# nathanweeks/exonerate

Measured on AMD Instinct MI355X. Metric: DP cells/s (first-pass lattice cells / end-to-end time), est2genome 1kb x 100kb batch, bit-exact vulgar vs reference, higher is better.
Workload: dtype int32 (packed int16 where proven exact)

## Files before the change

exonerate_amd/csrc/c4_ckpt16_kernel.h:

```cpp
#pragma once
#include "c4_viterbi16_kernel.h"

namespace c4k {

__device__ __forceinline__ int bfi32(int mask, int a, int b) {
    return __builtin_amdgcn_bitop3_b32(mask, a, b, 0xCA);
}

template <int R>
struct Prof16 {
    static constexpr int NCODE = 8;
    static constexpr int NP = (R + 1) / 2, EB = NP == 3 ? 12 : 8;
    static constexpr int CODE = 64 * EB;
    static constexpr int INTS = NCODE * CODE / 4;
};

template <int BND>
struct Stage16 {
    static constexpr int COLS = 128, CARRY0 = 6, PLANES = 6 + BND, INTS = COLS * PLANES;
};

template <class M, int R, int ROOT = -1>
struct WaveCK16 {
    using F = Facts<M>;
    static_assert(M::MAXAQ == 1, "the packed forms exchange exactly one query row per step");
    using RT = Roots<M>;
    using W32 = WaveDP<M, R, MODE_CKPT, true, true>;
    static constexpr int NS = M::NS, NCOL = M::MAXAT + 1, W = 64 * R, MAXAT = M::MAXAT;
    static constexpr int CS = W32::CS;
    static constexpr bool live(int s) { return M::NDES > 0 && W32::slot_live(s, 0); }
    static constexpr bool inner(int s) { return RT::member(ROOT, s); }
    static constexpr bool exported(int s) { return inner(s) && F::exported(s); }
    static constexpr int n_live() { int n = 0; for (int s = 0; s < NS; s++) n += (inner(s) && live(s)); return n; }
    static constexpr int n_inner() { int n = 0; for (int s = 0; s < NS; s++) n += inner(s); return n; }
    static constexpr int word_of(int s) { int n = 0; for (int x = 0; x < s; x++) n += inner(x); return n; }
    static constexpr int live_index(int s) { int n = 0; for (int x = 0; x < s; x++) n += (inner(x) && live(x)); return n; }
    static constexpr int CKW = n_inner() + (n_live() + 1) / 2;
    static constexpr int n_exp() { int n = 0; for (int s = 0; s < NS; s++) n += exported(s); return n; }
    static constexpr int n_exp_live() { int n = 0; for (int s = 0; s < NS; s++) n += (exported(s) && live(s)); return n; }
    static constexpr int BND = n_exp() * 2 + n_exp_live();
    static_assert(!F::has_phase(), "split-codon calcs are not packed");
    static_assert(M::NDES <= 1, "one shadow designation");
    static_assert(M::START == 0 && M::END == 1, "state numbering of the closed model");
    static_assert(!F::exported(M::START), "START advances nothing");
    struct C16 { int sc[NS]; int il[NS]; int srp[NS]; };
    typedef __attribute__((address_space(3))) int lds_int;
    __device__ __forceinline__ static lds_int *lds_at(int a) { return (lds_int *)(size_t)(unsigned)a; }
    __device__ __forceinline__ static int lds_addr(const lds_int *p) { return (int)(unsigned)(size_t)p; }
    using P16 = Prof16<R>;
    using ST = Stage16<BND>;

    const KParams *kp;
    int lane;
    const uint8_t *qc[2], *tc[2];
    const uint2 *ss16[2];
    int Q[2], T[2], q0[2], t0[2], tlast[2], cp_count[2], section[2];
    int *ckp[2];
    int cp_next_j[2], cp_next_i[2];
    int cp_phase[2];
    int Qm, Tm, Tmin;
    int open_il_pk, lim_pk, fifteen, at_pk[4], cv_pk[16];
    C16 col[NCOL][R], nbr[NCOL], expo, nx_carry;
    int prof_a[2];
    const uint8_t *tdense;
    int nx_sp4[4], nx_off[2], nx_prof[2 * P16::NP];
    int stage_a, stage_base;
    int carry_a, carry_base;
    bool carry_cols;
    int corner_sc[2], corner_srp[2];
    bool corner_set[2];

    template <class Fn>
    __device__ __forceinline__ static void for_exported(Fn &&fn) {
        int slot = 0;
        static_for<NS>([&](auto S_) __attribute__((always_inline)) { constexpr int S = S_;
            if constexpr (exported(S)) { fn(S_, slot); slot += 2 + (live(S) ? 1 : 0); }
        });
    }
    __device__ __forceinline__ static void write_empty_column(int *colp) {
        for_exported([&](auto S_, int slot) __attribute__((always_inline)) { constexpr int S = S_;
            colp[slot] = NEG16; colp[slot + 1] = 0;
            if constexpr (live(S)) colp[slot + 2] = 0;
        });
    }
    __device__ __forceinline__ void prefetch_carry() {
        const lds_int *p = lds_at(carry_a);
        for_exported([&](auto S_, int slot) __attribute__((always_inline)) { constexpr int S = S_;
            nx_carry.sc[S] = p[slot * ST::COLS];
            nx_carry.srp[S] = p[(slot + 1) * ST::COLS];
            if constexpr (live(S)) nx_carry.il[S] = p[(slot + 2) * ST::COLS];
        });
        carry_a = ((carry_a + 4) & (ST::COLS * 4 - 1)) | carry_base;
    }
    __device__ __forceinline__ void fill_carry(lds_int *stage, int c0, const int *bnd_in) {
        const int c = c0 + lane;
        const int jx = c < 0 ? 0 : (c > Tm ? Tm : c);
        const int jc = carry_cols ? jx : 0;
        const int *g = bnd_in + (long long)jc * BND;
        int v[BND];
        static_for<BND>([&](auto K_) __attribute__((always_inline)) { constexpr int K = K_; v[K] = g[K]; });
        lds_int *p = stage + ST::CARRY0 * ST::COLS + (c & (ST::COLS - 1));
        static_for<BND>([&](auto K_) __attribute__((always_inline)) { constexpr int K = K_; p[K * ST::COLS] = v[K]; });
    }
    template <int H>
    __device__ __forceinline__ void build_profile(int i0) {
        using P16 = Prof16<R>;
        typedef __attribute__((address_space(3))) int lds_int;
        int qr[R];
        static_for<R>([&](auto RR_) __attribute__((always_inline)) { constexpr int RR = RR_;
            const int i = i0 + RR;
            qr[RR] = 24 * ((i >= 1 && i <= Q[H]) ? (int)qc[H][q0[H] + i - 1] : 0);
        });
        for (int d = 0; d < P16::NCODE; d++) {
            const int code = tdense[24 + d];
            int v[R];
            static_for<R>([&](auto RR_) __attribute__((always_inline)) { constexpr int RR = RR_; v[RR] = kp->submat[qr[RR] + code]; });
            lds_int *p = (lds_int *)(size_t)(unsigned)(prof_a[H] + d * P16::CODE);
            static_for<P16::NP>([&](auto K_) __attribute__((always_inline)) { constexpr int K = K_;
                p[K] = pk_pack(v[2 * K], v[2 * K + 1 < R ? 2 * K + 1 : 2 * K]);
            });
        }
    }
    __device__ __forceinline__ void prefetch_column() {
        const lds_int *p = lds_at(stage_a);
        static_for<4>([&](auto K_) __attribute__((always_inline)) { constexpr int K = K_; nx_sp4[K] = p[K * ST::COLS]; });
        nx_off[0] = p[4 * ST::COLS]; nx_off[1] = p[5 * ST::COLS];
        stage_a = ((stage_a + 4) & (ST::COLS * 4 - 1)) | stage_base;
    }
    __device__ __forceinline__ void prefetch_profile() {
        const lds_int *pa = lds_at(prof_a[0] + nx_off[0]), *pb = lds_at(prof_a[1] + nx_off[1]);
        static_for<P16::NP>([&](auto K_) __attribute__((always_inline)) { constexpr int K = K_; nx_prof[K] = pa[K]; nx_prof[P16::NP + K] = pb[K]; });
    }
    __device__ __forceinline__ void fill_stage(lds_int *stage, int c0) {
        constexpr int mat = F::match_at();
        const int c = c0 + lane;
        uint2 sv[2]; int off[2];
        static_for<2>([&](auto H_) __attribute__((always_inline)) { constexpr int H = H_;
            int ti = t0[H] + c - mat;
            ti = ti < 0 ? 0 : (ti > tlast[H] ? tlast[H] : ti);
            off[H] = (int)tc[H][(unsigned)ti] * P16::CODE;
            sv[H] = uint2{0u, 0u};
            if constexpr (F::has_splice()) {
                int tp = t0[H] + c - 2;
                tp = tp < 0 ? 0 : (tp > tlast[H] ? tlast[H] : tp);
                sv[H] = ss16[H][(unsigned)tp];
            }
        });
        lds_int *p = stage + (c & (ST::COLS - 1));
        p[0 * ST::COLS] = (int)__builtin_amdgcn_perm(sv[1].x, sv[0].x, 0x05040100u);
        p[1 * ST::COLS] = (int)__builtin_amdgcn_perm(sv[1].x, sv[0].x, 0x07060302u);
        p[2 * ST::COLS] = (int)__builtin_amdgcn_perm(sv[1].y, sv[0].y, 0x05040100u);
        p[3 * ST::COLS] = (int)__builtin_amdgcn_perm(sv[1].y, sv[0].y, 0x07060302u);
        p[4 * ST::COLS] = off[0]; p[5 * ST::COLS] = off[1];
    }

    template <int RR, int PH, bool JINT>
    __device__ __forceinline__ void eval_cell(int j, bool origin, int ms, const int (&sp)[4]) {
        C16 &c = col[PH][RR];
        static_for<M::NT>([&](auto K_) __attribute__((always_inline)) { constexpr int K = K_;
            constexpr TrDesc t = M::tr[K];
            if constexpr (!inner(t.out)) return;
            if constexpr (t.in == M::START && (RR > 0 || JINT)) return;
            static_assert(!(t.in == M::START && F::code(K) == 1), "a state's first transition is never the one out of START");
            constexpr int PD = (PH - t.at + NCOL) % NCOL;
            const C16 &src = (t.aq == 0) ? col[PD][RR] : (RR > 0 ? col[PD][RR > 0 ? RR - 1 : 0] : nbr[PD]);
            int cand, srpc = 0, ilc = 0;
            if constexpr (t.in == M::START) {
                static_assert(t.in != M::START || (t.aq == 0 && t.at == 0 && t.calc < 0), "START leaves silently");
                cand = origin ? 0 : NEG16;
            } else {
                cand = src.sc[t.in];
                srpc = src.srp[t.in];
                if constexpr (t.calc >= 0) {
                    constexpr CalcDesc cd = M::calc[t.calc];
                    if constexpr (cd.kind == CALC_CONST) cand = pk_add<1>(cand, cv_pk[t.calc]);
                    else if constexpr (cd.kind >= CALC_MATCH_DNA && cd.kind <= CALC_MATCH_P2D) cand = pk_add<1>(cand, ms);
                    else if constexpr (cd.kind == CALC_SPLICE_PRE) cand = pk_add<1>(cand, sp[cd.param]);
                    else if constexpr (cd.kind == CALC_SPLICE_POST) {
                        static_assert(live(t.in), "post-splice calc without a length");
                        const int bad = pk_neg_mask(src.il[t.in], fifteen);
                        const int sv = bfi32(bad, NEG16, sp[cd.param]);
                        cand = pk_add<1>(cand, sv);
                    }
                }
                if constexpr (!JINT && t.at > 0) cand = (j >= t.at) ? cand : NEG16;
                if constexpr (live(t.out)) {
                    if constexpr (F::owns_shadow(t.in, 0)) ilc = open_il_pk;
                    else if constexpr (live(t.in)) ilc = pk_add<1>(src.il[t.in], at_pk[t.at]);
                }
            }
            if constexpr (F::code(K) == 1) {
                c.sc[t.out] = cand;
                c.srp[t.out] = srpc;
                if constexpr (live(t.out)) c.il[t.out] = ilc;
            } else {
                const int win = pk_lt_mask<1>(c.sc[t.out], cand, 0);
                c.srp[t.out] = bfi32(win, srpc, c.srp[t.out]);
                if constexpr (live(t.out)) c.il[t.out] = bfi32(win, ilc, c.il[t.out]);
                c.sc[t.out] = pk_max<1>(c.sc[t.out], cand);
            }
        });
    }

    template <bool JINT, int PH>
    __device__ __forceinline__ void step(int s, int i0, bool first_strip, bool last_strip, const int *bnd_in, int *bnd_out) {
        const int j = s - lane;
        int ms[R];
        static_for<P16::NP>([&](auto K_) __attribute__((always_inline)) { constexpr int K = K_;
            const int ea = nx_prof[K], eb = nx_prof[P16::NP + K];
            ms[2 * K] = (int)__builtin_amdgcn_perm((unsigned)eb, (unsigned)ea, 0x05040100u);
            if constexpr (2 * K + 1 < R) ms[2 * K + 1] = (int)__builtin_amdgcn_perm((unsigned)eb, (unsigned)ea, 0x07060302u);
        });
        int sp[4];
        static_for<4>([&](auto K_) __attribute__((always_inline)) { constexpr int K = K_; sp[K] = nx_sp4[K]; });
        for_exported([&](auto S_, int) __attribute__((always_inline)) { constexpr int S = S_;
            nbr[PH].sc[S] = dpp_shr1(nx_carry.sc[S], expo.sc[S]);
            nbr[PH].srp[S] = dpp_shr1(nx_carry.srp[S], expo.srp[S]);
            if constexpr (live(S)) nbr[PH].il[S] = dpp_shr1(nx_carry.il[S], expo.il[S]);
        });
        prefetch_carry();
        prefetch_column();
        const bool origin = first_strip & (lane == 0) & (s == 0);
        static_for<R>([&](auto RR_) __attribute__((always_inline)) { constexpr int RR = RR_;
            eval_cell<RR, PH, JINT>(j, origin, ms[RR], sp);
            if constexpr (RR == (R + 1) / 2 - 1) prefetch_profile();
        });
        for_exported([&](auto S_, int) __attribute__((always_inline)) { constexpr int S = S_;
            expo.sc[S] = col[PH][R - 1].sc[S];
            expo.srp[S] = col[PH][R - 1].srp[S];
            if constexpr (live(S)) expo.il[S] = col[PH][R - 1].il[S];
        });
        if (!last_strip && lane == 63 && j >= 0 && j <= Tm) {
            for_exported([&](auto S_, int slot) __attribute__((always_inline)) { constexpr int S = S_;
                int *p = bnd_out + (long long)j * BND + slot;
                p[0] = expo.sc[S];
                p[1] = expo.srp[S];
                if constexpr (live(S)) p[2] = expo.il[S];
            });
        }
        if (s >= Tmin) {
            static_for<2>([&](auto H_) __attribute__((always_inline)) { constexpr int H = H_;
                const bool mine = (j == T[H]) & (Q[H] >= i0) & (Q[H] < i0 + R);
                if (__builtin_amdgcn_ballot_w64(mine)) {
                    static_for<R>([&](auto RR_) __attribute__((always_inline)) { constexpr int RR = RR_;
                        if (mine & (i0 + RR == Q[H])) {
                            bool set = false;
                            int e_sc = 0, e_srp = 0;
                            static_for<M::NT>([&](auto K_) __attribute__((always_inline)) { constexpr int K = K_;
                                constexpr TrDesc t = M::tr[K];
                                if constexpr (t.out == M::END && inner(t.in)) {
                                    static_assert(t.out != M::END || (t.aq == 0 && t.at == 0 && t.calc < 0 && t.in != M::START),
                                                  "END is entered silently from an inner state");
                                    const int v = pk_half(col[PH][RR].sc[t.in], H);
                                    const int p = (int)(((unsigned)col[PH][RR].srp[t.in] >> (16 * H)) & 0xffffu);
                                    const bool win = !set | (e_sc < v);
                                    e_sc = win ? v : e_sc;
                                    e_srp = win ? p : e_srp;
                                    set = true;
                                }
                            });
                            corner_sc[H] = e_sc; corner_srp[H] = e_srp; corner_set[H] = set;
                        }
                    });
                }
            });
        }
        const bool cp_near = (section[0] <= 0) | (cp_phase[0] <= 63 + MAXAT - 1) | (section[1] <= 0) | (cp_phase[1] <= 63 + MAXAT - 1);
        static_for<2>([&](auto H_) __attribute__((always_inline)) { constexpr int H = H_;
            const int nx = cp_phase[H] + 1;
            cp_phase[H] = nx >= section[H] ? nx - section[H] : nx;
        });
        if (cp_near) {
            unsigned stamp = 0;
            static_for<2>([&](auto H_) __attribute__((always_inline)) { constexpr int H = H_;
                const bool cp_live = (j >= 0) & (j <= T[H]) & (cp_next_i[H] < cp_count[H]);
                const unsigned ahead = (unsigned)(cp_next_j[H] - j);
                if (__builtin_amdgcn_ballot_w64(cp_live & (ahead < (unsigned)MAXAT))) {
                    if (cp_live & (ahead < (unsigned)MAXAT)) {
                        static_for<R>([&](auto RR_) __attribute__((always_inline)) { constexpr int RR = RR_;
                            const int i = i0 + RR;
                            if (i <= Q[H]) {
                                int *p = ckp[H] + ((((long long)cp_next_i[H] * MAXAT + ahead) * (Q[H] + 1) + i)) * CKW;
                                constexpr unsigned sel = H ? 0x07060302u : 0x05040100u;
                                int lw[(n_live() + 1) / 2 > 0 ? (n_live() + 1) / 2 : 1] = {0};
                                static_for<NS>([&](auto S_) __attribute__((always_inline)) { constexpr int S = S_;
                                    if constexpr (inner(S)) {
                                        p[word_of(S)] = (int)__builtin_amdgcn_perm((unsigned)col[PH][RR].srp[S], (unsigned)col[PH][RR].sc[S], sel);
                                        if constexpr (live(S)) {
                                            constexpr int li = live_index(S);
                                            const unsigned h = ((unsigned)pk_add<1>(col[PH][RR].il[S], lim_pk) >> (16 * H)) & 0xffffu;
                                            lw[li / 2] |= (int)(h << (16 * (li & 1)));
                                        }
                                    }
                                });
                                static_for<(n_live() + 1) / 2>([&](auto L_) __attribute__((always_inline)) { constexpr int L = L_; p[n_inner() + L] = lw[L]; });
                            }
                        });
                    }
                    stamp |= (cp_live & (ahead == 0u)) ? (H ? 0xffff0000u : 0x0000ffffu) : 0u;
                }
            });
            if (__builtin_amdgcn_ballot_w64(stamp != 0u)) {
                int i0v = i0;
                asm volatile("" : "+v"(i0v));
                static_for<MAXAT>([&](auto ROW_) __attribute__((always_inline)) { constexpr int ROW = ROW_;
                    constexpr int PR = (PH - ROW + NCOL) % NCOL;
                    static_for<R>([&](auto RR_) __attribute__((always_inline)) { constexpr int RR = RR_;
                        const int rowid = (i0v + RR) * (NS * MAXAT);
                        static_for<NS>([&](auto S_) __attribute__((always_inline)) { constexpr int S = S_;
                            if constexpr (inner(S)) {
                                const int id = (rowid + S * MAXAT + ROW) & 0xffff;
                                col[PR][RR].srp[S] = bfi32((int)stamp, id | (id << 16), col[PR][RR].srp[S]);
                            }
                        });
                    });
                    const int rowid = (i0v - 1) * (NS * MAXAT);
                    static_for<NS>([&](auto S_) __attribute__((always_inline)) { constexpr int S = S_;
                        if constexpr (exported(S)) {
                            const int id = (rowid + S * MAXAT + ROW) & 0xffff;
                            nbr[PR].srp[S] = bfi32((int)stamp, id | (id << 16), nbr[PR].srp[S]);
                        }
                    });
                });
                static_for<2>([&](auto H_) __attribute__((always_inline)) { constexpr int H = H_;
                    const bool mine = (stamp & (H ? 0xffff0000u : 0x0000ffffu)) != 0u;
                    cp_next_i[H] += mine ? 1 : 0;
                    cp_next_j[H] += mine ? section[H] : 0;
                });
            }
        }
    }

    template <int NW>
    __device__ __forceinline__ void run(const DevJob &ja, const DevJob &jb, const DevSeqs &seqs, int *bnd, int *ckpt_a, int *ckpt_b,
                                        int wid, int *prog, lds_int *stage) {
        const DevJob *jp[2] = {&ja, &jb};
        ckp[0] = ckpt_a; ckp[1] = ckpt_b;
        static_for<2>([&](auto H_) __attribute__((always_inline)) { constexpr int H = H_;
            const DevJob &jx = *jp[H];
            Q[H] = jx.Q; T[H] = jx.T; q0[H] = jx.q0; t0[H] = jx.t0;
            tlast[H] = seqs.tlen[jx.pair] > 0 ? seqs.tlen[jx.pair] - 1 : 0;
            qc[H] = seqs.qcode + seqs.qoff[jx.pair];
            tc[H] = reinterpret_cast<const uint8_t *>(seqs.sub_rows) + seqs.toff[jx.pair];
            ss16[H] = F::has_splice() ? seqs.ss16 + seqs.toff[jx.pair] : nullptr;
            cp_count[H] = jx.cp_count;
            section[H] = jx.T / (jx.cp_count + 1);
            corner_sc[H] = LOW; corner_srp[H] = 0; corner_set[H] = false;
        });
        Qm = Q[0] > Q[1] ? Q[0] : Q[1]; Tm = T[0] > T[1] ? T[0] : T[1]; Tmin = T[0] < T[1] ? T[0] : T[1];
        static_for<M::NC>([&](auto CI_) __attribute__((always_inline)) { constexpr int CI = CI_;
            const int v = clamp16(kp->calc_value[CI]);
            cv_pk[CI] = pk_pack(v, v);
        });
        static_for<4>([&](auto A_) __attribute__((always_inline)) { constexpr int A = A_; at_pk[A] = pk_pack(A, A); });
        {
            const int lim = clamp16(kp->min_intron - 4);
            lim_pk = pk_pack(lim, lim);
            open_il_pk = pk_pack(-lim, -lim);
            fifteen = 0x000f000f;
        }
        const int nstrips = (Qm + 1 + W - 1) / W;
        const int nsteps = Tm + 64;
        const int main_lo = 63 + MAXAT, main_hi = Tm;
        const int nsteps_r = (nsteps + NCOL - 1) / NCOL * NCOL;
        const int main_lo_r = (main_lo + NCOL - 1) / NCOL * NCOL;
        constexpr int CHK = (63 / NCOL) * NCOL;
        const int PS = nsteps_r + 1;
        stage_base = lds_addr(stage);
        carry_base = stage_base + ST::CARRY0 * ST::COLS * 4;
        for (int b = wid; b < nstrips; b += NW) {
            const int i0 = b * W + lane * R;
            stage_a = stage_base + ((0 - lane) & (ST::COLS - 1)) * 4;
            carry_a = carry_base;
            static_for<2>([&](auto H_) __attribute__((always_inline)) { constexpr int H = H_;
                build_profile<H>(i0);
                cp_next_j[H] = section[H] > 0 ? section[H] : 0x7fffffff; cp_next_i[H] = 0;
                cp_phase[H] = section[H] > 0 ? (MAXAT - 1) % section[H] : 0;
            });
            static_for<NS>([&](auto S_) __attribute__((always_inline)) { constexpr int S = S_;
                expo.sc[S] = NEG16; expo.il[S] = 0; expo.srp[S] = 0;
                static_for<NCOL>([&](auto D_) __attribute__((always_inline)) { constexpr int D = D_;
                    nbr[D].sc[S] = NEG16; nbr[D].il[S] = 0; nbr[D].srp[S] = 0;
                    static_for<R>([&](auto RR_) __attribute__((always_inline)) { constexpr int RR = RR_;
                        col[D][RR].sc[S] = NEG16; col[D][RR].il[S] = 0; col[D][RR].srp[S] = 0;
                    });
                });
            });
            __builtin_amdgcn_fence(__ATOMIC_ACQUIRE, "workgroup");
            const bool first = (b == 0), last = (b == nstrips - 1);
            carry_cols = !first;
            const int *bnd_in = first ? bnd : bnd + BND + (long long)((b + 1) & 1) * (Tm + 1) * BND;
            int *bnd_out = bnd + BND + (long long)(b & 1) * (Tm + 1) * BND;
            auto group = [&](auto JI_, int s0) __attribute__((always_inline)) {
                constexpr bool JI = decltype(JI_)::value != 0;
                static_for<NCOL>([&](auto P_) __attribute__((always_inline)) { constexpr int P = P_;
                    step<JI, P>(s0 + P, i0, first, last, bnd_in, bnd_out);
                });
            };
            {
                const int above = (wid + NW - 1) % NW, above_base = ((b - 1) / NW) * PS, my_base = (b / NW) * PS;
                auto wait_above = [&](int c1) __attribute__((always_inline)) {
                    if constexpr (NW == 1) return;
                    if (first) return;
                    const int need = above_base + (c1 + 64 < nsteps_r ? c1 + 64 : nsteps_r);
                    while (__hip_atomic_load(prog + above, __ATOMIC_RELAXED, __HIP_MEMORY_SCOPE_WORKGROUP) < need) __builtin_amdgcn_s_sleep(1);
                    __builtin_amdgcn_fence(__ATOMIC_ACQUIRE, "workgroup");
                };
                fill_stage(stage, -63);
                wait_above(CHK < nsteps_r ? CHK : nsteps_r);
                fill_carry(stage, -63, bnd_in);
                prefetch_column();
                prefetch_profile();
                prefetch_carry();
                for (int c0 = 0; c0 < nsteps_r; c0 += CHK) {
                    const int c1 = c0 + CHK < nsteps_r ? c0 + CHK : nsteps_r;
                    fill_stage(stage, c0 + 1);
                    if (c0) wait_above(c1);
                    fill_carry(stage, c0 + 1, bnd_in);
                    int s = c0;
                    for (; s < main_lo_r && s < c1; s += NCOL) group(IC<0>{}, s);
                    for (; s + NCOL - 1 <= main_hi && s < c1; s += NCOL) group(IC<1>{}, s);
                    for (; s < c1; s += NCOL) group(IC<0>{}, s);
                    if constexpr (NW > 1) {
                        if (!last) {
                            __builtin_amdgcn_fence(__ATOMIC_RELEASE, "workgroup");
                            if (lane == 0) __hip_atomic_store(prog + wid, my_base + c1, __ATOMIC_RELAXED, __HIP_MEMORY_SCOPE_WORKGROUP);
                        }
                    }
                }
            }
            __builtin_amdgcn_fence(__ATOMIC_RELEASE, "workgroup");
        }
    }

    struct Cell3 { int sc, shadow, srp; };
    __device__ static Cell3 cell_at(const int *ck, const DevJob &job, int section_length, int cp, int row, int qpos, int state) {
        const int *p = ck + (((long long)cp * MAXAT + row) * (job.Q + 1) + qpos) * CKW;
        Cell3 c; c.sc = 0; c.shadow = 0; c.srp = 0;
        static_for<NS>([&](auto S_) __attribute__((always_inline)) { constexpr int S = S_;
            if constexpr (inner(S)) {
                if (state == S) {
                    const unsigned w = (unsigned)p[word_of(S)];
                    c.sc = (int)(short)(w & 0xffffu);
                    c.srp = (int)(w >> 16);
                    if constexpr (live(S)) {
                        constexpr int li = live_index(S);
                        const int il = (int)(((unsigned)p[n_inner() + li / 2] >> (16 * (li & 1))) & 0xffffu);
                        c.shadow = job.t0 + (section_length * (cp + 1) - row) - il - 2;
                    }
                }
            }
        });
        return c;
    }
    __device__ __noinline__ static void checkpoint_traceback(const int *ck, const DevJob &job, DevVsa *vsa, DevResult &res) {
        const int q0 = job.q0, t0 = job.t0;
        const int cpn = job.cp_count, section_length = job.T / (cpn + 1);
        auto decode = [&](int srp, int &state, int &row, int &pos) {
            row = srp % MAXAT;
            const int rem = srp / MAXAT;
            state = rem % NS;
            pos = rem / NS;
        };
        int state, row, pos, n = 0;
        decode(res.last_srp, state, row, pos);
        int query_start = q0 + pos, target_start = t0 + section_length * cpn - row;
        DevVsa v;
        v.qs = query_start; v.ts = target_start;
        v.ql = (q0 + job.Q) - query_start; v.tl = (t0 + job.T) - target_start;
        v.first_state = state;
        for (int l = 0; l < CELL_MAX; l++) v.final_cell[l] = l < CS ? res.final_cell[l] : 0;
        vsa[n++] = v;
        for (int c = cpn - 1; c >= 1; c--) {
            const DevVsa p = v;
            const int prev_row = row;
            const Cell3 cell = cell_at(ck, job, section_length, c, prev_row, p.qs - q0, p.first_state);
            decode(cell.srp, state, row, pos);
            query_start = q0 + pos;
            target_start = p.ts - section_length - row + prev_row;
            v.qs = query_start; v.ts = target_start; v.ql = p.qs - query_start; v.tl = p.ts - target_start;
            v.first_state = state;
            for (int l = 0; l < CELL_MAX; l++) v.final_cell[l] = 0;
            v.final_cell[0] = cell.sc; v.final_cell[1] = cell.shadow; v.final_cell[CS - 1] = cell.srp;
            vsa[n++] = v;
        }
        {
            const DevVsa p = v;
            const Cell3 cell = cell_at(ck, job, section_length, 0, row, p.qs - q0, p.first_state);
            v.qs = q0; v.ts = t0; v.ql = query_start - q0; v.tl = target_start - t0;
            v.first_state = job.first_state;
            for (int l = 0; l < CELL_MAX; l++) v.final_cell[l] = 0;
            v.final_cell[0] = cell.sc; v.final_cell[1] = cell.shadow; v.final_cell[CS - 1] = cell.srp;
            vsa[n++] = v;
        }
        res.n_vsa = n;
    }
};

template <class M, int R, int ROOT, int NW>
__device__ __forceinline__ void ckpt16_pair(const KParams *kp_lds, const DevSeqs &seqs, const DevJob *jobs, int ia, int ib,
                                            DevResult *results, DevVsa *vsas, int *bnd, int *ck_a, int *ck_b, int *prog,
                                            int (*corner_lds)[4], int *prof_mem, const uint8_t *tdense, int *stage_mem) {
    using DP = WaveCK16<M, R, ROOT>;
    if (threadIdx.x == 0) DP::write_empty_column(bnd);
    if constexpr (NW > 1) {
        if (threadIdx.x < NW) prog[threadIdx.x] = 0;
        if (threadIdx.x < 2) corner_lds[threadIdx.x][3] = 0;
    }
    __builtin_amdgcn_fence(__ATOMIC_RELEASE, "workgroup");
    __syncthreads();
    DP dp{};
    dp.kp = kp_lds;
    dp.lane = threadIdx.x & 63;
    dp.tdense = tdense;
    {
        typedef __attribute__((address_space(3))) int lds_int;
        const int w = __builtin_amdgcn_readfirstlane((int)(threadIdx.x >> 6));
        for (int h = 0; h < 2; h++)
            dp.prof_a[h] = (int)(unsigned)(size_t)((lds_int *)prof_mem + (w * 2 + h) * Prof16<R>::INTS) + dp.lane * Prof16<R>::EB;
    }
    {
        const int w = __builtin_amdgcn_readfirstlane((int)(threadIdx.x >> 6));
        dp.template run<NW>(jobs[ia], jobs[ib], seqs, bnd, ck_a, ck_b, w, prog, (typename DP::lds_int *)stage_mem + w * DP::ST::INTS);
    }
    int sc[2], srp[2];
    bool set[2];
    if constexpr (NW == 1) {
        for (int h = 0; h < 2; h++) {
            const unsigned long long owners = __ballot(dp.corner_set[h]);
            const int owner = owners ? __ffsll((long long)owners) - 1 : 0;
            sc[h] = __shfl(dp.corner_sc[h], owner); srp[h] = __shfl(dp.corner_srp[h], owner);
            set[h] = owners != 0;
        }
        __builtin_amdgcn_fence(__ATOMIC_ACQ_REL, "workgroup");
        __syncthreads();
    } else {
        for (int h = 0; h < 2; h++)
            if (dp.corner_set[h]) { corner_lds[h][0] = dp.corner_sc[h]; corner_lds[h][1] = dp.corner_srp[h]; corner_lds[h][3] = 1; }
        __builtin_amdgcn_fence(__ATOMIC_ACQ_REL, "workgroup");
        __syncthreads();
        for (int h = 0; h < 2; h++) { sc[h] = corner_lds[h][0]; srp[h] = corner_lds[h][1]; set[h] = corner_lds[h][3] != 0; }
    }
    if (threadIdx.x < 2 && (threadIdx.x == 0 || ib != ia)) {
        const int h = threadIdx.x;
        const DevJob &job = jobs[h ? ib : ia];
        DevResult res;
        res.flags = set[h] ? 0 : FLAG_NO_END; res.n_ops = 0; res.n_vsa = 0; res.pad = 0; res.qs = res.ts = 0;
        res.cell_size = DP::CS; res.ops_off = 0;
        for (int l = 0; l < CELL_MAX; l++) res.final_cell[l] = 0;
        res.final_cell[0] = sc[h]; res.final_cell[DP::CS - 1] = srp[h];
        res.score = sc[h]; res.end_set = set[h]; res.qe = job.Q; res.te = job.T; res.last_srp = srp[h];
        if (set[h]) DP::checkpoint_traceback(h ? ck_b : ck_a, job, vsas + job.vsa_off, res);
        results[h ? ib : ia] = res;
    }
    __syncthreads();
}

template <class M, int R, int WPE, bool ROOTED, int NW = 1>
__global__ __launch_bounds__(64 * NW) __attribute__((amdgpu_waves_per_eu(WPE, 8)))
void ckpt16_kernel(const KParams *kparams, DevSeqs seqs, const DevJob *jobs, const int *pairs, int n_pairs, DevResult *results,
                   DevVsa *vsas, DevScratch scratch, int *queue) {
    using RT = Roots<M>;
    static_assert(!ROOTED || RT::disjoint(), "a rooted pass needs components to choose from");
    __shared__ __attribute__((aligned(512))) int stage_mem[NW * Stage16<WaveCK16<M, R, ROOTED ? Roots<M>::root(0) : -1>::BND>::INTS];
    static_assert(!ROOTED || WaveCK16<M, R, Roots<M>::root(0)>::BND == WaveCK16<M, R, Roots<M>::root(Roots<M>::count() - 1)>::BND, "one stage layout for every root");
    __shared__ int next_job;
    __shared__ int prog[NW];
    __shared__ int corner_lds[2][4];
    __shared__ __attribute__((aligned(16))) int prof_mem[NW * 2 * Prof16<R>::INTS];
    __shared__ uint8_t tdense_lds[32];
    if (threadIdx.x < 32) tdense_lds[threadIdx.x] = reinterpret_cast<const uint8_t *>(seqs.sub_colptr)[threadIdx.x];
    __syncthreads();
    const KParams *kp_lds = kparams;
    int *bnd = scratch.bnd + (long long)blockIdx.x * scratch.bnd_stride;
    int *ck_a = scratch.ckpt + (long long)blockIdx.x * 2 * scratch.ckpt_stride, *ck_b = ck_a + scratch.ckpt_stride;
    for (;;) {
        if (threadIdx.x == 0) next_job = atomicAdd(queue, 1);
        __syncthreads();
        const int pid = __builtin_amdgcn_readfirstlane(next_job);
        __syncthreads();
        if (pid >= n_pairs) break;
        const int ia = pairs[2 * pid], ib = pairs[2 * pid + 1] >= 0 ? pairs[2 * pid + 1] : ia;
        if constexpr (ROOTED) {
            const int root = jobs[ia].root;
            bool ran = false;
            static_for<RT::count()>([&](auto X_) __attribute__((always_inline)) { constexpr int X = X_;
                constexpr int ROOT = RT::root(X);
                if (!ran && root == ROOT) {
                    ckpt16_pair<M, R, ROOT, NW>(kp_lds, seqs, jobs, ia, ib, results, vsas, bnd, ck_a, ck_b, prog, corner_lds, prof_mem, tdense_lds, stage_mem);
                    ran = true;
                }
            });
            if (!ran && threadIdx.x < 2 && (threadIdx.x == 0 || ib != ia)) {
                DevResult res;
                res.flags = FLAG_NO_END; res.n_ops = 0; res.n_vsa = 0; res.pad = 0; res.qs = res.ts = res.qe = res.te = 0;
                res.cell_size = 0; res.ops_off = 0; res.score = LOW; res.end_set = 0; res.last_srp = 0;
                for (int l = 0; l < CELL_MAX; l++) res.final_cell[l] = 0;
                results[threadIdx.x ? ib : ia] = res;
            }
        } else {
            ckpt16_pair<M, R, -1, NW>(kp_lds, seqs, jobs, ia, ib, results, vsas, bnd, ck_a, ck_b, prog, corner_lds, prof_mem, tdense_lds, stage_mem);
        }
    }
}

}
```

exonerate_amd/csrc/c4_config.h:

```cpp
#pragma once
#include <cstdlib>
#include <mutex>

namespace c4cfg {

#define C4CFG_KEYS(X) \
    X(TRACE) X(PK16) X(WPE) X(WIN16) X(PACK) X(SEED_KSHIFT) X(WIN_NW) X(WINDOW_HOPS) X(WINDOWED) X(STRICT) X(SPLICE_TILE) \
    X(SDP_ARENA_MB) X(REPAIR_REJOIN) X(PK16_R6) X(PK16_NW8) X(PK16_LONG) X(PK16_IO) X(PK16_C8) X(PIN_XFER) X(NESTED_REDO) X(MW) \
    X(LOOP_SHORTCUT) X(LOCAL_EXACT) X(LANES) X(FUSED) X(FREE_NOW) X(FORCE_CORNER_MISMATCH) X(DL_SYNC_FIRST) X(CONT_FREE) \
    X(CK16_TMAX) X(CK16_ROOT) X(CK16) X(CELL_STRICT) X(BYROOT) X(SS16_CHECK) X(SCORE_FIRST) X(HOST_THREADS) X(FORCE_SEQUENTIAL) \
    X(FILL_ALLOC)

enum Key {
#define X(name) name,
    C4CFG_KEYS(X)
#undef X
    N_KEYS
};

struct Entry { bool set; int value; double real; };
struct Table { Entry e[N_KEYS]; };

inline Table &table() { static Table t{}; return t; }
inline std::once_flag &loaded_flag() { static std::once_flag f; return f; }

inline void load_from_environment() {
    static const char *const names[N_KEYS] = {
#define X(name) "C4GPU_" #name,
        C4CFG_KEYS(X)
#undef X
    };
    Table &t = table();
    for (int k = 0; k < N_KEYS; k++) {
        const char *v = getenv(names[k]);
        t.e[k].set = v != nullptr;
        t.e[k].value = v ? atoi(v) : 0;
        t.e[k].real = v ? atof(v) : 0.0;
    }
}
inline const Table &get() {
    std::call_once(loaded_flag(), load_from_environment);
    return table();
}
inline bool has(Key k) { return get().e[k].set; }
inline int num(Key k, int dflt) { const Entry &x = get().e[k]; return x.set ? x.value : dflt; }
inline double real(Key k, double dflt) { const Entry &x = get().e[k]; return x.set ? x.real : dflt; }
inline bool is(Key k, int v) { const Entry &x = get().e[k]; return x.set && x.value == v; }
inline bool nonzero(Key k) { const Entry &x = get().e[k]; return x.set && x.value != 0; }

}
```

exonerate_amd/csrc/c4_engine_find_path.inc:

```
int find_path_batch(Engine &eng, const ResidentSeqs &seqs, int dpmemory_mb, c4gpu_score threshold,
                    c4gpu_alignment *alignments, const std::vector<const c4gpu_subopt *> *subs = nullptr,
                    const uint8_t *active = nullptr, const std::vector<c4gpu_score> *pair_thresholds = nullptr,
                    const c4gpu_region *initial = nullptr, bool own_all = true) {
    const c4gpu_model *m = eng.model;
    const int n = seqs.n_pairs;
    const c4gpu_score base_threshold = threshold;
    auto thr = [&](int pair) {
        return (pair_thresholds && (*pair_thresholds)[pair] > base_threshold) ? (*pair_thresholds)[pair] : base_threshold;
    };
    struct SubScope {
        Engine &e;
        SubScope(Engine &e_, const std::vector<const c4gpu_subopt *> *s) : e(e_) { e.pair_sub = s; }
        ~SubScope() { e.pair_sub = nullptr; }
    } sub_scope(eng, subs);
    const bool trace = c4cfg::has(c4cfg::TRACE);
    const auto t_begin = std::chrono::steady_clock::now();
    auto lap = [&](const char *what) {
        if (trace) fprintf(stderr, "c4gpu trace: find_path_batch: %-28s at %.3f ms\n", what,
                           std::chrono::duration<double, std::milli>(std::chrono::steady_clock::now() - t_begin).count());
    };
    const bool strict_cells = cell_strict();
    std::vector<PairPlan> plan(n);
    std::vector<JobSpec> &specs = eng.fp_specs;
    std::vector<JobOut> &outs = eng.fp_outs;
    specs.clear();
    std::vector<int> owner;
    if (own_all) for (int i = 0; i < n; i++) memset(&alignments[i], 0, sizeof(c4gpu_alignment));
    std::vector<int> region_pairs;
    for (int i = 0; i < n; i++) {
        plan[i].ar = initial ? initial[i] : c4gpu_region{0, 0, seqs.qlen[i], seqs.tlen[i]};
        plan[i].active = !active || active[i];
        if (!plan[i].active) continue;
        if (c4h::use_reduced_space(m, &plan[i].ar, dpmemory_mb)) {
            plan[i].reduced = true;
            if (!model_is_global(m)) region_pairs.push_back(i);
        }
    }
    const size_t step1_total = region_pairs.size();
    double &hit_rate = eng.ctx->hit_rate[subs ? 1 : 0];
    std::vector<std::pair<int, DevResult>> region_done;
    {
        bool pk16_serves = eng.family == FAM_EST2GENOME && eng.pk16_params_ok && region_pairs.size() >= 2 &&
                           !(c4cfg::is(c4cfg::PK16, 0)) && get_kernel_pk16(eng.family, 1) != nullptr;
        for (size_t x = 0; x < region_pairs.size() && pk16_serves; x++)
            pk16_serves = eng.pk16_fits(plan[region_pairs[x]].ar.query_length, plan[region_pairs[x]].ar.target_length);
        int kshift_env = pk16_serves ? 12 : 13;
        for (int i : region_pairs)
            if (plan[i].ar.target_length < (4 << 13) && plan[i].ar.target_length >= (4 << 12)) kshift_env = 12;
        kshift_env = c4cfg::num(c4cfg::SEED_KSHIFT, kshift_env);
        const int kshift = std::max(2, std::min(kshift_env, 20));
        const bool off = c4cfg::is(c4cfg::WINDOWED, 0);
        const KernelInfo *k1 = get_kernel_mw(eng.family, MODE_SCORE, true, false, 4, false, 1);
        const KernelInfo *k2 = get_kernel_mw(eng.family, MODE_REGION, true, true, 4, false, 2);
        const bool pays = eng.ctx->window_rate < 0 || eng.ctx->window_rate >= 0.5 || c4cfg::has(c4cfg::SEED_KSHIFT);
        if (!off && pays && !subs && eng.local && eng.local_exact && k1 && k2 && !(c4cfg::is(c4cfg::PACK, 0))) {
            std::vector<int> win_pairs, rest;
            for (int i : region_pairs) {
                const c4gpu_region &ar = plan[i].ar;
                const bool rows_ok = ar.query_length + 1 > 2 * 64 * k2->R;
                if (rows_ok && ar.target_length >= (4 << kshift) && ar.query_length < (1 << 20)) win_pairs.push_back(i);
                else rest.push_back(i);
            }
            if (!win_pairs.empty()) {
                std::vector<DevResult> wres;
                if (windowed_region_pass(eng, seqs, win_pairs, plan, thr, kshift, wres)) return -1;
                for (size_t x = 0; x < win_pairs.size(); x++) region_done.emplace_back(win_pairs[x], wres[x]);
                region_pairs.swap(rest);
            }
        }
    }
    {
        const bool sf_env = c4cfg::has(c4cfg::SCORE_FIRST);
        const bool can = threshold > C4GPU_IMPOSSIBLY_LOW_SCORE && region_pairs.size() >= 512;
        const size_t total = region_pairs.size();
        auto score_filter = [&](size_t first, size_t count, size_t *kept) -> int {
            specs.clear();
            for (size_t x = first; x < first + count; x++) { JobSpec s; s.pair = region_pairs[x]; s.region = plan[region_pairs[x]].ar; specs.push_back(s); }
            if (eng.run(seqs, MODE_SCORE, false, specs, outs)) return -1;
            *kept = 0;
            for (size_t x = 0; x < count; x++) {
                if (outs[x].res.score < thr(region_pairs[first + x])) plan[region_pairs[first + x]].active = false;
                else (*kept)++;
            }
            return 0;
        };
        bool score_first = false;
        size_t sampled = 0, kept = 0, all_kept = 0;
        if (can && sf_env) score_first = c4cfg::num(c4cfg::SCORE_FIRST, 0) != 0;
        else if (can && hit_rate >= 0) score_first = hit_rate < 0.3;
        else if (can) {
            sampled = std::min<size_t>(8 * (size_t)eng.ctx->prop.multiProcessorCount, total);
            if (score_filter(0, sampled, &kept)) return -1;
            all_kept = kept;
            score_first = (double)kept / (double)sampled < 0.3;
        }
        if (score_first && sampled < total) {
            if (score_filter(sampled, total - sampled, &kept)) return -1;
            all_kept += kept;
        }
        if (score_first || sampled) {
            std::vector<int> survivors;
            for (int i : region_pairs) if (plan[i].active) survivors.push_back(i);
            region_pairs.swap(survivors);
        }
        (void)all_kept;
    }
    specs.clear();
    for (int i : region_pairs) { JobSpec s; s.pair = i; s.region = plan[i].ar; specs.push_back(s); }
    if (eng.run(seqs, MODE_REGION, false, specs, outs)) return -1;
    for (size_t x = 0; x < region_pairs.size(); x++) region_done.emplace_back(region_pairs[x], outs[x].res);
    for (const auto &pr : region_done) {
        PairPlan &p = plan[pr.first];
        const DevResult &r = pr.second;
        if (r.score < thr(pr.first)) { p.active = false; continue; }
        p.region_score = r.score;
        p.end_from = r.last_srp;
        if (m->start_scope != C4GPU_SCOPE_QUERY) p.ar.query_start += r.qs;
        if (m->start_scope != C4GPU_SCOPE_TARGET) p.ar.target_start += r.ts;
        p.ar.query_length = r.qe - (m->start_scope != C4GPU_SCOPE_QUERY ? r.qs : 0);
        p.ar.target_length = r.te - (m->start_scope != C4GPU_SCOPE_TARGET ? r.ts : 0);
    }
    if (step1_total >= 64 && threshold > C4GPU_IMPOSSIBLY_LOW_SCORE) {
        size_t hits = 0;
        for (const auto &pr : region_done) hits += plan[pr.first].active ? 1 : 0;
        const double rate = (double)hits / (double)step1_total;
        hit_rate = hit_rate < 0 ? rate : 0.5 * hit_rate + 0.5 * rate;
    }
    lap("region pass done");
    specs.clear(); owner.clear();
    for (int i = 0; i < n; i++) {
        PairPlan &p = plan[i];
        if (!p.active) continue;
        if (p.reduced && c4h::use_reduced_space(m, &p.ar, dpmemory_mb)) continue;
        p.reduced = false;
        JobSpec s; s.pair = i; s.region = p.ar;
        specs.push_back(s); owner.push_back(i);
    }
    if (eng.run(seqs, MODE_PATH, false, specs, outs)) return -1;
    for (size_t x = 0; x < owner.size(); x++) {
        const int i = owner[x];
        const DevResult &r = outs[x].res;
        c4gpu_alignment &a = alignments[i];
        a.score = r.score;
        a.region.query_start = plan[i].ar.query_start + r.qs;
        a.region.target_start = plan[i].ar.target_start + r.ts;
        a.region.query_length = r.qe - r.qs;
        a.region.target_length = r.te - r.ts;
        int cap = 0;
        for (uint32_t r : outs[x].runs) c4h::alignment_add(&a, &cap, (int)(r >> 24), (int)(r & 0xffffff));
        a.valid = 1;
    }
    lap("quadratic paths done");
    std::vector<int> red;
    for (int i = 0; i < n; i++)
        if (plan[i].active && plan[i].reduced) {
            Segment s;
            memset(&s, 0, sizeof s);
            s.region = plan[i].ar; s.first_state = m->start_state; s.needs_checkpoints = true;
            plan[i].segs.assign(1, s);
            red.push_back(i);
        }
    std::map<int, JobOut> ckpt_done;
    if (!red.empty() && !subs) {
        std::vector<char> done(n, 0);
        if (fused_reduced_paths(eng, seqs, red, plan, dpmemory_mb, alignments, done, ckpt_done)) return -1;
        std::vector<int> rest;
        for (int i : red) if (!done[i]) rest.push_back(i);
        red.swap(rest);
        lap("device route done");
    }
    std::vector<c4gpu_score> red_score(n, 0);
    std::vector<char> redo(n, 0), packed_pair(n, 0);
    for (const auto &kv : ckpt_done) packed_pair[kv.first] = kv.second.packed ? 1 : 0;
    bool first_round = true;
    for (;;) {
        struct Ref { int pair, seg; };
        std::vector<Ref> refs;
        specs.clear();
        for (int i : red) {
            std::vector<Segment> &sg = plan[i].segs;
            for (size_t k = 0; k < sg.size(); k++) {
                if (!sg[k].needs_checkpoints) continue;
                JobSpec s; s.pair = i; s.region = sg[k].region;
                s.first_state = sg[k].first_state;
                if (k > 0) memcpy(s.first_cell, sg[k - 1].final_cell, sizeof s.first_cell);
                s.final_state = (k + 1 < sg.size()) ? sg[k + 1].first_state : m->end_state;
                s.cp_count = c4h::checkpoint_rows(m, &s.region, dpmemory_mb);
                specs.push_back(s);
                refs.push_back(Ref{i, (int)k});
            }
        }
        if (specs.empty()) break;
        lap("checkpoint jobs listed");
        bool have_all = first_round && !ckpt_done.empty();
        for (size_t x = 0; x < refs.size() && have_all; x++) have_all = ckpt_done.count(refs[x].pair) != 0;
        if (have_all) {
            if (outs.size() < refs.size()) outs.resize(refs.size());
            for (size_t x = 0; x < refs.size(); x++) outs[x] = ckpt_done[refs[x].pair];
        } else if (eng.run(seqs, MODE_CKPT, true, specs, outs)) return -1;
        lap("checkpoint pass done");
        std::vector<int> group;
        for (size_t x = 0; x < refs.size(); x++)
            if (!x || refs[x].pair != refs[x - 1].pair) group.push_back((int)x);
        group.push_back((int)refs.size());
        parallel_for((long long)group.size() - 1, 256, [&](long long g0, long long g1) {
          for (long long g = g0; g < g1; g++)
            for (int x = group[g + 1] - 1; x >= group[g]; x--) {
            std::vector<Segment> &sg = plan[refs[x].pair].segs;
            const int k = refs[x].seg;
            if (first_round) red_score[refs[x].pair] = outs[x].res.score;
            std::vector<Segment> children;
            children.reserve(outs[x].vsa.size());
            for (int v = (int)outs[x].vsa.size() - 1; v >= 0; v--) {
                const DevVsa &dv = outs[x].vsa[v];
                Segment c;
                c.region = c4gpu_region{dv.qs, dv.ts, dv.ql, dv.tl};
                c.first_state = dv.first_state;
                memcpy(c.final_cell, dv.final_cell, sizeof c.final_cell);
                c.needs_checkpoints = c4h::use_reduced_space(m, &c.region, dpmemory_mb);
                children.push_back(c);
            }
            if (!first_round && !children.empty() &&
                !final_cell_equiv(children.back().final_cell, sg[k].final_cell, 1 + m->total_shadow_designations,
                                  sg[k].region.target_start + sg[k].region.target_length, packed_pair[refs[x].pair] != 0, strict_cells)) {
                const bool next_in_round = x + 1 < group[g + 1] && refs[x + 1].seg == k + 1;
                if (c4cfg::has(c4cfg::TRACE))
                    fprintf(stderr, "c4gpu trace: pair %d nested segment %d: final cell %d/%d after the nested pass, %d/%d predicted%s\n",
                            refs[x].pair, k, children.back().final_cell[0], children.back().final_cell[1], sg[k].final_cell[0], sg[k].final_cell[1],
                            next_in_round ? ": the next segment's nested pass used the old cell, sequential route" : "");
                if (next_in_round || c4cfg::nonzero(c4cfg::NESTED_REDO)) redo[refs[x].pair] = 1;
            }
            sg.erase(sg.begin() + k);
            sg.insert(sg.begin() + k, children.begin(), children.end());
            }
        });
        first_round = false;
    }
    lap("segments expanded");
    specs.clear();
    struct Ref2 { int pair, seg; };
    std::vector<Ref2> refs2;
    std::vector<size_t> seg_first(red.size() + 1, 0);
    for (size_t r = 0; r < red.size(); r++) seg_first[r + 1] = seg_first[r] + plan[red[r]].segs.size();
    std::vector<JobSpec> &sub_specs = eng.fp_sub_specs;
    if (sub_specs.size() != seg_first[red.size()]) sub_specs.resize(seg_first[red.size()]);
    refs2.resize(seg_first[red.size()]);
    parallel_for((long long)red.size(), 256, [&](long long r0, long long r1) {
        for (long long r = r0; r < r1; r++) {
            const int i = red[r];
            const std::vector<Segment> &sg = plan[i].segs;
            for (size_t k = 0; k < sg.size(); k++) {
                JobSpec s; s.pair = i; s.region = sg[k].region;
                s.first_state = sg[k].first_state;
                if (k > 0) memcpy(s.first_cell, sg[k - 1].final_cell, sizeof s.first_cell);
                s.final_state = (k + 1 < sg.size()) ? sg[k + 1].first_state : m->end_state;
                sub_specs[seg_first[r] + k] = s;
                refs2[seg_first[r] + k] = Ref2{i, (int)k};
            }
        }
    });
    lap("sub-alignment jobs listed");
    if (eng.run(seqs, MODE_PATH, true, sub_specs, outs)) return -1;
    lap("sub-alignment pass done");
    {
        std::vector<int> cap(n, 0);
        const int path_cs = 1 + m->total_shadow_designations;
        const bool force_seq = c4cfg::has(c4cfg::FORCE_SEQUENTIAL);
        if (force_seq) for (int i : red) redo[i] = 1;
        struct Repair { int pair, next_seg; int seed[CELL_MAX]; };
        std::vector<Repair> repairs;
        std::vector<int> repairing(n, -1);
        std::mutex repairs_lock;
        parallel_for((long long)red.size(), 256, [&](long long r0, long long r1) {
          for (long long r = r0; r < r1; r++)
            for (size_t x = seg_first[r]; x < seg_first[r + 1]; x++) {
            const int i = refs2[x].pair, k = refs2[x].seg;
            c4gpu_alignment &a = alignments[i];
            std::vector<Segment> &sg = plan[i].segs;
            if (k == 0) {
                a.score = red_score[i];
                a.region = plan[i].ar;
                a.valid = 1;
            }
            if (redo[i] || repairing[i] >= 0) continue;
            for (uint32_t r : outs[x].runs) c4h::alignment_add(&a, &cap[i], (int)(r >> 24), (int)(r & 0xffffff));
            if (!final_cell_equiv(outs[x].res.final_cell, sg[k].final_cell, path_cs,
                                  sg[k].region.target_start + sg[k].region.target_length, packed_pair[i] != 0, strict_cells)) {
                if (c4cfg::has(c4cfg::TRACE))
                    fprintf(stderr, "c4gpu trace: pair %d sub-alignment %d: final cell %d/%d computed, %d/%d predicted\n", i,
                            k, outs[x].res.final_cell[0], outs[x].res.final_cell[1], sg[k].final_cell[0], sg[k].final_cell[1]);
                if (k + 1 < (int)sg.size()) {
                    Repair rp; rp.pair = i; rp.next_seg = k + 1;
                    memcpy(rp.seed, outs[x].res.final_cell, sizeof rp.seed);
                    std::lock_guard<std::mutex> hold(repairs_lock);
                    repairs.push_back(rp);
                    repairing[i] = k + 1;
                }
            }
            }
        });
        std::sort(repairs.begin(), repairs.end(), [](const Repair &x, const Repair &y) { return x.pair < y.pair; });
        const bool rejoin = !(c4cfg::is(c4cfg::REPAIR_REJOIN, 0));
        std::vector<size_t> first_of(n, 0);
        for (size_t r = 0; r < red.size(); r++) first_of[red[r]] = seg_first[r];
        std::vector<JobOut> routs;
        long long repair_launches = 0, repaired = 0, rejoined = 0;
        while (!repairs.empty()) {
            specs.clear();
            for (const Repair &rp : repairs) {
                const std::vector<Segment> &sg = plan[rp.pair].segs;
                JobSpec s; s.pair = rp.pair; s.region = sg[rp.next_seg].region;
                s.first_state = sg[rp.next_seg].first_state;
                memcpy(s.first_cell, rp.seed, sizeof s.first_cell);
                s.final_state = (rp.next_seg + 1 < (int)sg.size()) ? sg[rp.next_seg + 1].first_state : m->end_state;
                specs.push_back(s);
            }
            if (eng.run(seqs, MODE_PATH, true, specs, routs)) return -1;
            repair_launches++; repaired += (long long)repairs.size();
            std::vector<Repair> next;
            for (size_t x = 0; x < repairs.size(); x++) {
                Repair rp = repairs[x];
                c4gpu_alignment &a = alignments[rp.pair];
                const std::vector<Segment> &sg = plan[rp.pair].segs;
                const int nseg = (int)sg.size();
                for (uint32_t r : routs[x].runs) c4h::alignment_add(&a, &cap[rp.pair], (int)(r >> 24), (int)(r & 0xffffff));
                memcpy(rp.seed, routs[x].res.final_cell, sizeof rp.seed);
                const int j = rp.next_seg;
                if (j + 1 >= nseg) continue;
                const bool joined = rejoin && final_cell_equiv(rp.seed, sg[j].final_cell, path_cs,
                                                               sg[j].region.target_start + sg[j].region.target_length, packed_pair[rp.pair] != 0, strict_cells);
                if (!joined) { rp.next_seg = j + 1; next.push_back(rp); continue; }
                rejoined++;
                for (int k = j + 1; k < nseg; k++) {
                    const JobOut &bo = outs[first_of[rp.pair] + k];
                    for (uint32_t r : bo.runs) c4h::alignment_add(&a, &cap[rp.pair], (int)(r >> 24), (int)(r & 0xffffff));
                    if (k + 1 < nseg && !final_cell_equiv(bo.res.final_cell, sg[k].final_cell, path_cs,
                                                          sg[k].region.target_start + sg[k].region.target_length, packed_pair[rp.pair] != 0, strict_cells)) {
                        rp.next_seg = k + 1;
                        memcpy(rp.seed, bo.res.final_cell, sizeof rp.seed);
                        next.push_back(rp);
                        break;
                    }
                }
            }
            repairs.swap(next);
        }
        if (repair_launches && c4cfg::has(c4cfg::TRACE))
            fprintf(stderr, "c4gpu trace: stale tails: %lld sub-alignments recomputed in %lld launches, %lld re-joined the batch\n",
                    repaired, repair_launches, rejoined);
    }
    lap("alignments assembled");
    for (int i : red)
        if (redo[i] && sequential_reduced_path(eng, seqs, i, dpmemory_mb, plan[i].ar, &alignments[i])) return -1;
    for (int i = 0; i < n; i++) {
        if (active && !active[i]) continue;
        c4gpu_alignment &a = alignments[i];
        if (a.valid && a.score < thr(i)) c4gpu_alignment_clear(&a);
    }
    return 0;
}

struct SideLane {
    c4gpu_ctx ctx;
    Engine eng;
    ~SideLane() {
        if (ctx.stream) (void)hipStreamDestroy(ctx.stream);
        if (ctx.ev0) (void)hipEventDestroy(ctx.ev0);
        if (ctx.ev1) (void)hipEventDestroy(ctx.ev1);
    }
// ... 62 lines not shown
```

exonerate_amd/csrc/c4_engine_launch.inc:

```
struct JobSpec {
    int pair;
    c4gpu_region region;
    int first_state = 0, final_state = 1, cp_count = 0;
    int root = 0;
    int first_cell[CELL_MAX] = {0};
    bool dump_checkpoints = false;
    const c4gpu_subopt *sub = nullptr;
    const int32_t *span_in = nullptr;
    int32_t *span_out = nullptr;
};
typedef std::vector<std::pair<int32_t, int32_t>> RegionPoints;
struct RunList {
    static constexpr int INLINE = 6;
    int n = 0;
    uint32_t small[INLINE];
    std::vector<uint32_t> big;
    const uint32_t *begin() const { return n <= INLINE ? small : big.data(); }
    const uint32_t *end() const { return begin() + n; }
    void assign_reversed(const uint32_t *first, int count) {
        n = count;
        uint32_t *dst = small;
        if (count > INLINE) { big.resize(count); dst = big.data(); }
        for (int k = 0; k < count; k++) dst[k] = first[count - 1 - k];
    }
};
struct JobOut {
    DevResult res;
    RunList runs;
    std::vector<DevVsa> vsa;
    std::vector<int> checkpoints;
    bool packed = false;
};

struct SeedPlan {
    int mode = 0;
    int kshift = 11;
    bool fmt16 = false;
    int seedw = 0, dc = 0;
    std::vector<long long> off;
    std::vector<int> rows;
    std::vector<long long> base;
    std::vector<int> d, t0w, t0_base;
    int hops = 0;
};

int window_waves(int family) {
    int nw = c4cfg::num(c4cfg::WIN_NW, 2);
    if (nw != 2) nw = 4;
    return get_kernel_mw(family, MODE_REGION, true, true, nw, false, 2) ? nw : 4;
}

struct Engine {
    c4gpu_ctx *ctx;
    const c4gpu_model *model;
    int family;
    bool local;
    bool local_exact = true;
    bool pk16_params_ok = false;
    double calc_bound = 0;
    int pk16_match_max = 1, pk16_max_intron = 0;
    int pk16_intron_gain = 0, pk16_intron_cols = 4;
    int loop_tr_host[16] = {-1, -1, -1, -1, -1, -1, -1, -1, -1, -1, -1, -1, -1, -1, -1, -1};
    DevBuf<KParams> kparams;
    DevBuf<DevJob> d_jobs;
    DevBuf<DevResult> d_results;
    DevBuf<DevVsa> d_vsa;
    DevBuf<uint32_t> d_runs, d_runs_out;
    DevBuf<unsigned long long> d_runs_used;
    DevBuf<uint8_t> d_ops;
    DevBuf<int> d_bnd, d_ckpt, d_ckpt_dump, d_queue;
    DevBuf<uint32_t> d_tb;
    DevBuf<int> d_sub_t, d_sub_q, d_sub_colptr, d_span, d_seed, d_pairs;
    DevBuf<DevJob> d_fjobs, d_fsub_jobs;
    DevBuf<DevResult> d_fres, d_fsub_res;
    DevBuf<DevVsa> d_fvsa;
    DevBuf<int> d_ffirst, d_fflags, d_fout;
    DevBuf<unsigned long long> d_fstats;
    DevBuf<FusePair> d_fpairs;
    std::vector<DevJob> hf_jobs;
    std::vector<DevResult> hf_res;
    std::vector<int> hf_first, hf_flags, hf_out;
    std::vector<FusePair> hf_pairs;
    std::vector<int> h_order;
    std::vector<long long> h_key;
    std::vector<DevJob> h_jobs;
    std::vector<DevResult> h_res;
    std::vector<uint32_t> h_runs;
    std::vector<DevVsa> h_vsa;
    std::vector<int> h_dump;
    std::vector<JobSpec> fp_specs;
    std::vector<JobSpec> fp_sub_specs;
    std::vector<JobOut> fp_outs;
    const std::vector<const c4gpu_subopt *> *pair_sub = nullptr;

    bool annotated = false;
    int init(c4gpu_ctx *c, const c4gpu_model *m, const c4gpu_params *params) {
        KParams kp;
        if (init_host(c, m, params, kp)) return -1;
        return kparams.upload(&kp, 1, ctx->stream);
    }
    int init_host(c4gpu_ctx *c, const c4gpu_model *m, const c4gpu_params *params, KParams &kp) {
        ctx = c; model = m;
        family = model_family(*m);
        if (family < 0) {
            c4h::set_error(std::string("model [") + m->name + "] is not one of the device-accelerated families");
            return -1;
        }
        local = m->start_scope == C4GPU_SCOPE_ANYWHERE && m->end_scope == C4GPU_SCOPE_ANYWHERE;
        memset(&kp, 0, sizeof kp);
        for (int i = 0; i < 16; i++) loop_tr_host[i] = -1;
        for (int i = 0; i < m->n_calcs; i++) kp.calc_value[i] = m->calcs[i].value;
        kp.min_intron = params->min_intron; kp.max_intron = params->max_intron;
        if (params->max_intron < params->min_intron) {
            kp.min_intron = kp.max_intron = 0x7fffffff;
        }
        kp.start_scope = m->start_scope; kp.end_scope = m->end_scope;
        bool protein = false;
        for (int i = 0; i < m->n_calcs; i++)
            if (m->calcs[i].kind == C4GPU_CALC_MATCH_PROTEIN || m->calcs[i].kind == C4GPU_CALC_MATCH_P2D ||
                m->calcs[i].kind == C4GPU_CALC_MATCH_CODON) protein = true;
        memcpy(kp.submat, protein ? &params->protein_submat[0][0] : &params->dna_submat[0][0], sizeof(int) * 24 * 24);
        bool dna_match = false;
        for (int i = 0; i < m->n_calcs; i++) dna_match |= m->calcs[i].kind == C4GPU_CALC_MATCH_DNA;
        const bool veto = annotated && dna_match && !protein;
        for (int c = 0; c < 24; c++) kp.submat[24 * 24 + c] = veto ? C4GPU_IMPOSSIBLY_LOW_SCORE : 0;
        {
            double pmax = 0;
            for (int i = 0; i < m->n_calcs; i++) pmax = std::max(pmax, std::fabs((double)m->calcs[i].value));
            for (int i = 0; i < 24 * 24; i++) pmax = std::max(pmax, std::fabs((double)kp.submat[i]));
            double smax = 0;
            if (family_has_splice(family))
                for (int k = 0; k < 4; k++) {
                    const c4gpu_splice_model &sp = params->splice[k];
                    double sum = 0;
                    for (int r = 0; r < sp.model_length && r < C4GPU_SPLICE_MAX_LEN; r++) {
                        double mx = 0;
                        for (int c = 0; c < 5; c++) mx = std::max(mx, std::fabs((double)sp.data[r][c]));
                        sum += mx;
                    }
                    smax = std::max(smax, sum + 1.0);
                }
            local_exact = (pmax + smax) * (m->n_states + 4) < 4.0e8;
            calc_bound = pmax + smax;
            double mmax = 0;
            for (int i = 0; i < 24 * 24; i++) mmax = std::max(mmax, (double)kp.submat[i]);
            pk16_match_max = (int)std::max(1.0, mmax);
            pk16_params_ok = pmax <= 16000.0 && smax <= 16000.0 && params->min_intron >= 0 && params->min_intron <= 30000 &&
                             params->max_intron >= params->min_intron;
            pk16_max_intron = params->max_intron;
            if (veto) {
                local_exact = false;
                pk16_params_ok = false;
                calc_bound = std::max(calc_bound, 987654321.0);
            }
            if (family_has_splice(family)) {
                int best[4] = {0, 0, 0, 0};
                for (int k = 0; k < 4; k++) {
                    const c4gpu_splice_model &sp = params->splice[k];
                    double sum = 0;
                    for (int r = 0; r < sp.model_length && r < C4GPU_SPLICE_MAX_LEN; r++) {
                        double mx = 0;
                        for (int c = 0; c < 5; c++) mx = std::max(mx, (double)sp.data[r][c]);
                        sum += mx;
                    }
                    best[k] = (int)std::floor(sum + 0.5) + 1;
                }
                long long gain = -0x40000000LL;
                for (int st = 0; st < m->n_states; st++) {
                    long long pre = -0x40000000LL, post = -0x40000000LL;
                    for (int k = 0; k < m->n_transitions; k++) {
                        const c4gpu_transition &t = m->transitions[k];
                        if (t.calc < 0) continue;
                        const c4gpu_calc &cc = m->calcs[t.calc];
                        const int prm = cc.param & 3;
                        if (cc.kind == C4GPU_CALC_SPLICE_PRE && t.output == st) pre = std::max<long long>(pre, (long long)cc.value + best[prm]);
                        if (cc.kind == C4GPU_CALC_SPLICE_POST && t.input == st) post = std::max<long long>(post, (long long)cc.value + best[prm]);
                    }
                    if (pre > -0x40000000LL && post > -0x40000000LL) gain = std::max(gain, pre + post);
                }
                pk16_intron_gain = (int)std::max<long long>(0, std::min<long long>(gain, 1 << 20));
                pk16_intron_cols = std::max(4, params->min_intron);
                const bool loop_on = !(c4cfg::is(c4cfg::LOOP_SHORTCUT, 0));
                bool others_cost = true;
                for (int k = 0; k < m->n_transitions; k++) {
                    const c4gpu_transition &t = m->transitions[k];
                    if (t.advance_query != 0 || t.calc < 0) continue;
                    const c4gpu_calc &cc = m->calcs[t.calc];
                    if (cc.kind == C4GPU_CALC_SPLICE_PRE || cc.kind == C4GPU_CALC_SPLICE_POST) continue;
                    if (cc.kind != C4GPU_CALC_CONST || cc.value > 0) others_cost = false;
                }
                if (loop_on && family == FAM_EST2GENOME && others_cost && m->n_states <= 16) {
                    int tight[4];
                    for (int k = 0; k < 4; k++) {
                        const c4gpu_splice_model &sp = params->splice[k];
                        double sum = 0;
                        for (int r = 0; r < sp.model_length && r < C4GPU_SPLICE_MAX_LEN; r++) {
                            double mx = 0;
                            for (int c = 0; c < 5; c++) mx = std::max(mx, (double)sp.data[r][c]);
                            sum += mx;
                        }
                        tight[k] = (int)std::floor(sum + 0.5 + 1e-3);
                    }
                    for (int st = 0; st < m->n_states; st++) {
                        long long pre = -0x40000000LL, post = -0x40000000LL;
                        int loop = -1;
                        bool clean = true;
                        for (int k = 0; k < m->n_transitions; k++) {
                            const c4gpu_transition &t = m->transitions[k];
                            const c4gpu_calc *cc = t.calc >= 0 ? &m->calcs[t.calc] : nullptr;
                            if (t.input == st && t.output == st) {
                                if (t.advance_query == 0 && t.advance_target == 1 && !cc && loop < 0) loop = k; else clean = false;
                            } else if (t.output == st) {
                                if (cc && cc->kind == C4GPU_CALC_SPLICE_PRE) pre = std::max<long long>(pre, (long long)cc->value + tight[cc->param & 3]);
                                else clean = false;
                            } else if (t.input == st) {
                                if (cc && cc->kind == C4GPU_CALC_SPLICE_POST) post = std::max<long long>(post, (long long)cc->value + tight[cc->param & 3]);
                                else clean = false;
                            }
                        }
                        loop_tr_host[st] = (clean && loop >= 0 && pre > -0x40000000LL && post > -0x40000000LL && pre + post < 0) ? loop : -1;
                    }
                }
            }
            if (c4cfg::is(c4cfg::LOCAL_EXACT, 0)) local_exact = false;
        }
        for (int i = 0; i < 16; i++) kp.loop_tr[i] = loop_tr_host[i];
        if (c4cfg::has(c4cfg::TRACE) && family == FAM_EST2GENOME) {
            std::string which;
            for (int i = 0; i < 16; i++) if (loop_tr_host[i] >= 0) which += " " + std::to_string(i) + ":" + std::to_string(loop_tr_host[i]);
            fprintf(stderr, "c4gpu trace: one-row sections answered without a DP for states (state:loop transition)%s\n",
                    which.empty() ? " none" : which.c_str());
        }
        for (int c = 0; c < 4096; c++) {
            const uint8_t row = params->submat_index[params->aa[params->trans[c]]];
            kp.codon_row[c] = row < 24 ? row : 0;
        }
        return 0;
    }

    bool cont_free_ok(long long q_plus_t) const {
        if (c4cfg::is(c4cfg::CONT_FREE, 0)) return false;
        return (double)(q_plus_t + 2) * std::max(calc_bound, 1.0) < 4.0e8;
    }

    bool pk16_fits(int query_length, int target_length) const {
        const double gain = (double)(query_length + 1) * pk16_match_max +
                            (double)(target_length / pk16_intron_cols + 1) * pk16_intron_gain;
        return gain <= 16000.0 && (!family_has_splice(family) || (long long)target_length + 4 <= (long long)pk16_max_intron);
    }
    int ensure_ss16(const ResidentSeqs &seqs) {
        if (!family_has_splice(family)) return 0;
        std::lock_guard<std::mutex> hold(seqs.ss16_lock);
        if (!seqs.ss16_built) {
            if (seqs.ss16.alloc((size_t)seqs.ss_len)) return -1;
            HIP_OK(pk16_build_splice(family, kparams.p, seqs.dev.ss, seqs.dev.ss_stride, seqs.ss_len, seqs.ss16.p, ctx->stream));
            HIP_OK(c4_stream_sync(ctx->stream));
            seqs.ss16_built = true;
        }
        return 0;
    }

    int run(const ResidentSeqs &seqs, int mode, bool cont, const std::vector<JobSpec> &specs, std::vector<JobOut> &out,
            SeedPlan *seed = nullptr) {
        const int n = (int)specs.size();
        if (seed) return run_impl(seqs, mode, cont, specs, out, nullptr, seed);
        for (int i = 0; i < n; i++)
            if (specs[i].span_in || specs[i].span_out) return run_impl(seqs, mode, cont, specs, out, nullptr);
        std::vector<int> plain, blocked;
        std::vector<RegionPoints> pts;
        for (int i = 0; i < n; i++) {
            const c4gpu_subopt *so = specs[i].sub ? specs[i].sub : (pair_sub ? (*pair_sub)[specs[i].pair] : nullptr);
            RegionPoints rp;
            if (so && !so->points.empty()) c4h::subopt_region_points(so, specs[i].region, rp);
            if (rp.empty()) plain.push_back(i);
            else { blocked.push_back(i); pts.push_back(std::move(rp)); }
        }
        if (blocked.empty()) return run_impl(seqs, mode, cont, specs, out, nullptr);
        if (plain.size() * 4 < blocked.size()) {
            std::vector<RegionPoints> all(n);
            for (size_t x = 0; x < blocked.size(); x++) all[blocked[x]] = std::move(pts[x]);
            return run_impl(seqs, mode, cont, specs, out, &all);
        }
        out.assign(n, JobOut());
        std::vector<JobSpec> part;
        std::vector<JobOut> part_out;
        for (int i : plain) part.push_back(specs[i]);
        if (run_impl(seqs, mode, cont, part, part_out, nullptr)) return -1;
        for (size_t x = 0; x < plain.size(); x++) out[plain[x]] = std::move(part_out[x]);
        part.clear();
        for (int i : blocked) part.push_back(specs[i]);
        if (run_impl(seqs, mode, cont, part, part_out, &pts)) return -1;
        for (size_t x = 0; x < blocked.size(); x++) out[blocked[x]] = std::move(part_out[x]);
        return 0;
    }

    int run_impl(const ResidentSeqs &seqs, int mode, bool cont, const std::vector<JobSpec> &specs,
                 std::vector<JobOut> &out, const std::vector<RegionPoints> *pts, SeedPlan *seed = nullptr) {
        const bool trace = c4cfg::has(c4cfg::TRACE);
        const auto t_begin = std::chrono::steady_clock::now();
        struct Trace {
            bool on; std::chrono::steady_clock::time_point t0; int mode, n;
            ~Trace() {
                if (on) fprintf(stderr, "c4gpu trace: run mode %d jobs %d host+device %.3f ms\n", mode, n,
                                std::chrono::duration<double, std::milli>(std::chrono::steady_clock::now() - t0).count());
            }
        } tr{trace, t_begin, mode, (int)specs.size()};
        auto lap = [&](const char *what) {
            if (trace) fprintf(stderr, "c4gpu trace:   %-18s at %.3f ms\n", what,
                               std::chrono::duration<double, std::milli>(std::chrono::steady_clock::now() - t_begin).count());
        };
        const int n = (int)specs.size();
        if ((int)out.size() < n) out.resize(n);
        if (!n) return 0;
        const bool use_local = local && local_exact && !cont && (mode == MODE_SCORE || mode == MODE_REGION);
        auto nbits = [](int v) { int b = 0; while ((1LL << b) <= v) b++; return b; };
        bool pack = (mode == MODE_REGION) && !(c4cfg::is(c4cfg::PACK, 0));
        for (int i = 0; i < n && pack; i++)
            pack = nbits(specs[i].region.query_length) + nbits(specs[i].region.target_length) <= 31;
        const int wpe_env = c4cfg::num(c4cfg::WPE, 0);
        int span = 0;
        for (int i = 0; i < n; i++) {
            const int sp = specs[i].span_in ? 1 : (specs[i].span_out ? 2 : 0);
            if (i && sp != span) { c4h::set_error("jobs with and without span matrices in one call"); return -1; }
            span = sp;
        }
        bool cont_free = false;
        if (cont && (mode == MODE_PATH || mode == MODE_CKPT) && !pts && !span) {
            long long worst = 0;
            bool cells_leave = false;
            for (int i = 0; i < n; i++) {
                worst = std::max(worst, (long long)specs[i].region.query_length + specs[i].region.target_length);
                cells_leave |= specs[i].dump_checkpoints;
            }
            cont_free = !cells_leave && cont_free_ok(worst);
        }
        const uint8_t *staged_codes = nullptr;
        const KernelInfo *ki = get_kernel(family, mode, cont, cont ? cont_free : use_local, pack, pts ? 0 : wpe_env, pts != nullptr, span);
        if (!ki && cont_free) ki = get_kernel(family, mode, cont, false, pack, pts ? 0 : wpe_env, pts != nullptr, span);
        if (!ki) { c4h::set_error("no compiled kernel for this model/mode"); return -1; }
        const int span_cs = 1 + model->total_shadow_designations;
        const int mw_env = c4cfg::num(c4cfg::MW, 1);
        if (seed) {
            int win_nw = seed->mode == 2 ? window_waves(family) : 4;
            if (seed->mode == 1 && mw_env != 4 && (long long)n * 8 <= 2LL * 4 * ctx->prop.multiProcessorCount &&
                get_kernel_mw(family, mode, true, false, 8, false, 1))
                win_nw = 8;
            ki = get_kernel_mw(family, mode, true, mode == MODE_REGION, win_nw, false, seed->mode);
            if (!ki || !use_local || (mode == MODE_REGION && !pack)) { c4h::set_error("no seeded kernel for this launch"); return -1; }
            const int pk_env = c4cfg::num(c4cfg::PK16, 1);
            const KernelInfo *kpk = (seed->mode == 1 && pk_env && pk16_params_ok && n >= 2) ? get_kernel_pk16(family, pk_env == 3 ? 0 : pk_env == 4 ? 2 : 1) : nullptr;
            if (kpk) {
                bool fits = true;
                for (int i = 0; i < n && fits; i++) fits = pk16_fits(specs[i].region.query_length, specs[i].region.target_length);
                if (fits && pk_env != 3 && ensure_ss16(seqs)) return -1;
                if (fits) ki = kpk;
                const int w16_env = c4cfg::num(c4cfg::WIN16, 1);
                const KernelInfo *kd = (fits && pk_env == 1 && w16_env) ? get_kernel_pk16(family, 3) : nullptr;
                if (kd && get_kernel_win16(family, 0) && seed->kshift <= 15 && seqs.tdense_n > 0) {
                    bool rows_ok = true;
                    for (int i = 0; i < n && rows_ok; i++) rows_ok = specs[i].region.query_length < 32000;
                    if (rows_ok) { ki = kd; seed->fmt16 = true; }
                    const int io_env = c4cfg::num(c4cfg::PK16_IO, 2);
                    const KernelInfo *ke = (rows_ok && io_env) ? get_kernel_pk16(family, io_env == 2 ? 5 : 4) : nullptr;
                    if (ke && seqs.tdense_n > pk16_staged_codes() && seqs.tdense_n <= 8 && io_env == 2 &&
                        !(c4cfg::is(c4cfg::PK16_C8, 0)) && get_kernel_pk16(family, 8)) {
                        bool strips_ok = true;
                        for (int i = 0; i < n && strips_ok; i++) strips_ok = specs[i].region.query_length + 1 <= pk16_staged_rows();
                        if (strips_ok) { ki = get_kernel_pk16(family, 8); staged_codes = seqs.tdense.p; }
                    }
                    if (ke && seqs.tdense_n > 0 && seqs.tdense_n <= pk16_staged_codes()) {
                        bool strips_ok = true;
                        for (int i = 0; i < n && strips_ok; i++) strips_ok = specs[i].region.query_length + 1 <= pk16_staged_rows();
                        if (strips_ok) { ki = ke; staged_codes = seqs.tdense.p; }
                        else if (io_env == 2 && !(c4cfg::is(c4cfg::PK16_R6, 0))) {
                            const KernelInfo *kh = get_kernel_pk16(family, 7);
                            bool six_ok = kh != nullptr;
                            for (int i = 0; i < n && six_ok; i++) six_ok = specs[i].region.query_length + 1 <= pk16_staged_rows6();
                            if (six_ok) { ki = kh; staged_codes = seqs.tdense.p; }
                            else if (get_kernel_pk16(family, 9) && !(c4cfg::is(c4cfg::PK16_LONG, 0))) {
                                ki = get_kernel_pk16(family, 9); staged_codes = seqs.tdense.p;
                            }
                        }
                        const int nw8_env = c4cfg::num(c4cfg::PK16_NW8, -1);
                        const KernelInfo *kg = (strips_ok && io_env == 2 && nw8_env != 0) ? get_kernel_pk16(family, 6) : nullptr;
                        if (kg && (nw8_env == 1 || (n + 1) / 2 <= ctx->prop.multiProcessorCount)) ki = kg;
                    }
                }
            }
            if (seed->mode == 1) { seed->seedw = ki->seedw; seed->dc = ki->max_at; }
            if (seed->mode == 2 && seed->fmt16) {
                const int w16_env = c4cfg::num(c4cfg::WIN16, 1);
                int shape = w16_env == 9 ? 0 : w16_env - 1;
                if (w16_env <= 1) {
                    long long strips = 0;
                    for (int i = 0; i < n; i++) strips += (specs[i].region.query_length + 1 + 255) / 256;
                    shape = strips >= 2LL * n ? ((n + 1) / 2 <= ctx->prop.multiProcessorCount ? 4 : 7) : 0;
                }
                ki = get_kernel_win16(family, shape);
                if (!ki || !seqs.ss16_built) { c4h::set_error("no packed window kernel for this launch"); return -1; }
            }
        } else if (mw_env && !cont && (mode == MODE_SCORE || mode == MODE_REGION)) {
            const KernelInfo *kmw = get_kernel_mw(family, mode, use_local, pack, 4, pts != nullptr);
            if (kmw) {
                long long strips = 0;
                for (int i = 0; i < n; i++) strips += (specs[i].region.query_length + 1 + 64 * kmw->R - 1) / (64 * kmw->R);
                if (strips >= 3LL * n) ki = kmw;
            }
            const KernelInfo *kmw8 = (ki == kmw && mw_env != 4 && !pts) ? get_kernel_mw(family, mode, use_local, pack, 8) : nullptr;
            if (kmw8 && (long long)n * 8 <= 2LL * 4 * ctx->prop.multiProcessorCount) ki = kmw8;
        }
        if (seed && c4cfg::has(c4cfg::TRACE)) fprintf(stderr, "c4gpu trace:   seeded pass %d with kernel %s\n", seed->mode, ki->name);
        std::vector<int> &order = h_order;
        order.resize(n);
        std::iota(order.begin(), order.end(), 0);
        auto cells = [&](int i) { return (long long)(specs[i].region.query_length + 1) * (specs[i].region.target_length + 1); };
        {
            std::vector<long long> &key = h_key;
            key.resize(n);
            long long biggest = 0;
            for (int i = 0; i < n; i++) { key[i] = cells(i); biggest = std::max(biggest, key[i]); }
            if (ki->pairs)
                std::stable_sort(order.begin(), order.end(), [&](int a, int b) {
                    return specs[a].root != specs[b].root ? specs[a].root < specs[b].root : key[a] > key[b];
                });
            else if (!(n > 32768 && biggest < (1 << 20)))
                std::stable_sort(order.begin(), order.end(), [&](int a, int b) { return key[a] > key[b]; });
        }
        std::vector<DevJob> &jobs = h_jobs;
        jobs.resize(n);
        long long ops_total = 0, vsa_total = 0, dump_total = 0, max_T = 0, max_tb = 0, max_ckpt = 0, total_cells = 0;
        long long max_runs = 0, sub_cols = 0, span_total = 0, seed_total = 0;
        if (seed && seed->mode == 1) seed->off.assign(n, -1);
        std::vector<int> sub_t, sub_q;
        parallel_for(n, 32768, [&](long long first, long long last) {
            for (long long x = first; x < last; x++) {
                const JobSpec &s = specs[order[x]];
                DevJob &j = jobs[x];
                memset(&j, 0, sizeof j);
                j.seed_off = -1;
                if (seed) j.seed_kshift = seed->kshift;
                j.pair = s.pair; j.q0 = s.region.query_start; j.t0 = s.region.target_start;
                j.Q = s.region.query_length; j.T = s.region.target_length;
                j.first_state = s.first_state; j.final_state = s.final_state; j.cp_count = s.cp_count;
                j.root = s.root;
                j.tshift = nbits(j.T);
                memcpy(j.first_cell, s.first_cell, sizeof j.first_cell);
                j.ckpt_off = -1;
            }
        });
        for (int x = 0; x < n; x++) {
            const JobSpec &s = specs[order[x]];
            DevJob &j = jobs[x];
            if (span) {
                j.span_off = span_total;
                span_total += (long long)(s.region.query_length + 1) * (s.region.target_length + 1) * span_cs;
            }
            if (pts) {
                const RegionPoints &rp = (*pts)[order[x]];
                j.sub_off = sub_cols; j.sub_pt_off = (int)sub_t.size(); j.sub_pt_n = (int)rp.size();
                sub_cols += s.region.target_length + 2;
                for (const auto &p : rp) { sub_t.push_back(p.first); sub_q.push_back(p.second); }
            }
            if (seed) {
                if (seed->mode == 1) {
                    j.seed_off = seed_total; j.seed_rows = s.region.query_length + 1;
                    seed->off[order[x]] = seed_total;
                    seed_total += (long long)(s.region.target_length >> seed->kshift) * ki->max_at * (s.region.query_length + 1) *
                                  ki->seedw;
                } else {
                    j.seed_off = seed->off[order[x]]; j.seed_rows = seed->rows[order[x]];
                    if (seed->hops) {
                        j.seed_base = seed->base[order[x]]; j.win_d = seed->d[order[x]]; j.win_t0w = seed->t0w[order[x]];
                        j.win_t0_base = seed->t0_base[order[x]]; j.win_hops = seed->hops;
                    }
                }
            }
            j.ops_off = ops_total; j.ops_cap = 0; j.vsa_off = (int)vsa_total;
            total_cells += (long long)(j.Q + 1) * (j.T + 1);
            max_T = std::max<long long>(max_T, j.T);
            if (mode == MODE_PATH) {
                const long long strips = (j.Q + 1 + 64 * ki->R - 1) / (64 * ki->R);
                j.ops_cap = 3 * (j.Q + j.T) + 16;
                max_runs = std::max<long long>(max_runs, j.ops_cap);
                ops_total += j.ops_cap;
                max_tb = std::max(max_tb, strips * (long long)(j.T + 64) * 64 * ki->R);
            }
            if (mode == MODE_CKPT) {
                const long long ck = (long long)j.cp_count * ki->max_at * (j.Q + 1) * ki->n_states * ki->cs;
                max_ckpt = std::max(max_ckpt, ck);
                vsa_total += j.cp_count + 1;
                if (s.dump_checkpoints) { j.ckpt_off = dump_total; dump_total += ck; }
            }
        }
        if (seed && seed->mode == 2 && seed->hops)
            max_T = std::max<long long>(max_T, (1LL << seed->kshift) + 2LL * ki->max_at);
        lap("jobs built");
        int blocks_per_cu = 0;
        HIP_OK(hipOccupancyMaxActiveBlocksPerMultiprocessor(&blocks_per_cu, ki->func, 64 * ki->waves, 0));
        if (blocks_per_cu < 1) blocks_per_cu = 1;
        if (trace) fprintf(stderr, "c4gpu trace:   kernel %s: %d workgroups per CU\n", ki->name, blocks_per_cu);
        std::vector<int> pair_list;
        if (ki->pairs)
            for (int x = 0; x < n;) {
                const bool two = x + 1 < n && jobs[x + 1].root == jobs[x].root;
                pair_list.push_back(x); pair_list.push_back(two ? x + 1 : -1);
                x += two ? 2 : 1;
            }
        long long grid = std::min<long long>(ki->pairs ? (long long)pair_list.size() / 2 : n, (long long)blocks_per_cu * ctx->prop.multiProcessorCount);
        long long carry_T = 0;
        for (int x = 0; x < n; x++)
            if ((jobs[x].Q + 1 + 64 * ki->R - 1) / (64 * ki->R) > (ki->hbm_carry ? 1 : ki->waves)) carry_T = max_T;
        const long long bnd_per_wave = (2 * ((carry_T ? carry_T : 0) + 1) + 1) * (long long)std::max(ki->bnd, 1);
        const long long bytes_per_wave = bnd_per_wave * 4 + max_tb * 4 + max_ckpt * 4 + max_runs * 4;
        long long runs_capacity = std::min<long long>(ops_total, std::max<long long>(1 << 20, (long long)n * 256));
        const long long budget = (long long)(ctx->prop.totalGlobalMem / 4);
        if (bytes_per_wave * grid > budget) grid = std::max<long long>(1, budget / std::max<long long>(1, bytes_per_wave));
        hipStream_t s = ctx->stream;
        std::vector<DevResult> &res = h_res;
        res.resize(n);
        std::vector<uint32_t> &runs = h_runs;
        runs.clear();
        std::vector<DevVsa> &vsa = h_vsa;
        std::vector<int> &dump = h_dump;
        vsa.resize(vsa_total);
        dump.resize(dump_total);
        for (int attempt = 0; attempt < 2; attempt++) {
            int zero = 0;
            unsigned long long zero64 = 0;
            if (d_jobs.upload(jobs.data(), n, s) || d_results.alloc(n) || d_queue.upload(&zero, 1, s) ||
                d_runs_used.upload(&zero64, 1, s) || d_bnd.alloc(bnd_per_wave * grid) || d_vsa.alloc(vsa_total) ||
                d_runs.alloc(max_runs * grid) || d_runs_out.alloc(runs_capacity) ||
                d_tb.alloc(max_tb * grid) || d_ckpt.alloc(max_ckpt * grid) || d_ckpt_dump.alloc(dump_total))
                return -1;
            LaunchArgs a;
            a.kp = kparams.p; a.seqs = seqs.dev; a.jobs = d_jobs.p; a.n_jobs = n; a.results = d_results.p;
            a.seqs.sub_colptr = nullptr; a.seqs.sub_rows = nullptr;
            a.seqs.span_in = nullptr; a.seqs.span_out = nullptr;
            if (span) {
                std::vector<int> host(span_total);
                for (int x = 0; x < n; x++) {
                    const JobSpec &sp = specs[order[x]];
                    const int32_t *src = span == 1 ? sp.span_in : sp.span_out;
                    const long long cnt = (long long)(jobs[x].Q + 1) * (jobs[x].T + 1) * span_cs;
                    memcpy(host.data() + jobs[x].span_off, src, sizeof(int) * cnt);
                }
                if (d_span.upload(host.data(), span_total, s)) return -1;
                a.seqs.span_in = d_span.p; a.seqs.span_out = d_span.p;
            }
            if (pts) {
                sub_q.push_back(0);
                if (d_sub_t.upload(sub_t.data(), sub_t.size(), s) || d_sub_q.upload(sub_q.data(), sub_q.size(), s) ||
                    d_sub_colptr.alloc(2 * sub_cols)) return -1;
                hipLaunchKernelGGL(subopt_colptr_kernel, dim3(std::min(n, 65535)), dim3(256), 0, s, d_jobs.p, n,
                                   d_sub_t.p, d_sub_q.p, d_sub_colptr.p);
                HIP_OK(hipGetLastError());
                a.seqs.sub_colptr = d_sub_colptr.p; a.seqs.sub_rows = d_sub_q.p;
            }
            a.seqs.ss16 = seqs.ss16_built ? seqs.ss16.p : nullptr;
            if (seed && seed->mode == 2 && seed->fmt16) {
                if (seqs.tdense_n <= 0) { c4h::set_error("packed region windows without a residue-code table"); return -1; }
                a.seqs.sub_rows = reinterpret_cast<const int *>(seqs.tcode_dense.p);
                a.seqs.sub_colptr = reinterpret_cast<const int *>(seqs.tdense.p);
            }
            a.seqs.seed = nullptr;
            if (seed) {
                if (seed->mode == 1 && d_seed.alloc((size_t)std::max<long long>(seed_total, 1))) return -1;
                a.seqs.seed = d_seed.p;
            }
            a.vsas = d_vsa.p; a.ops = nullptr; a.queue = d_queue.p; a.grid = (int)grid; a.stream = s;
            if (ki->pairs) {
                if (d_pairs.upload(pair_list.data(), pair_list.size(), s)) return -1;
                a.aux = d_pairs.p; a.n_aux = (int)(pair_list.size() / 2);
            }
            if (staged_codes) a.aux = reinterpret_cast<const int *>(staged_codes);
            a.scratch.bnd = d_bnd.p; a.scratch.bnd_stride = bnd_per_wave; a.scratch.carry = carry_T ? 1 : 0;
            a.scratch.tb = max_tb ? d_tb.p : nullptr; a.scratch.tb_stride = max_tb;
            a.scratch.ckpt = max_ckpt ? d_ckpt.p : nullptr; a.scratch.ckpt_stride = max_ckpt;
            a.scratch.ckpt_dump = d_ckpt_dump.p;
            a.scratch.runs = d_runs.p; a.scratch.runs_stride = max_runs;
            a.scratch.runs_out = d_runs_out.p; a.scratch.runs_capacity = runs_capacity;
            a.scratch.runs_used = d_runs_used.p;
            lap("uploaded");
            if (ctx->timing) HIP_OK(hipEventRecord(ctx->ev0, s));
            HIP_OK(ki->launch(a));
            if (ctx->timing) HIP_OK(hipEventRecord(ctx->ev1, s));
            unsigned long long used = 0;
            if (d_results.download(res.data(), n, s) || d_runs_used.download(&used, 1, s) ||
                d_vsa.download(vsa.data(), vsa_total, s) || d_ckpt_dump.download(dump.data(), dump_total, s))
                return -1;
            HIP_OK(c4_stream_sync(s));
            lap("kernel + results");
            if (ctx->timing) {
                float ms = 0;
                HIP_OK(hipEventElapsedTime(&ms, ctx->ev0, ctx->ev1));
                ctx->kernel_ms[mode] += ms; ctx->kernel_launches[mode]++; ctx->kernel_cells[mode] += total_cells;
            }
            if ((long long)used > runs_capacity) {
                if (attempt == 1) { c4h::set_error("traceback runs exceed their worst-case buffer"); return -1; }
                runs_capacity = ops_total;
                continue;
            }
            runs.resize(used);
            if (d_runs_out.download(runs.data(), used, s)) return -1;
            HIP_OK(c4_stream_sync(s));
            if (span == 2) {
                std::vector<int> host(span_total);
                if (d_span.download(host.data(), span_total, s)) return -1;
                HIP_OK(c4_stream_sync(s));
                for (int x = 0; x < n; x++) {
                    const long long cnt = (long long)(jobs[x].Q + 1) * (jobs[x].T + 1) * span_cs;
                    memcpy(specs[order[x]].span_out, host.data() + jobs[x].span_off, sizeof(int) * cnt);
                }
            }
            break;
        }
        lap("runs downloaded");
        std::atomic<int> overflow{0};
        parallel_for(n, 32768, [&](long long first, long long last) {
            for (long long x = first; x < last; x++) {
                JobOut &o = out[order[x]];
                o.res = res[x];
                if (res[x].flags & FLAG_OPS_OVERFLOW) { overflow = 1; continue; }
                if (mode == MODE_PATH) o.runs.assign_reversed(runs.data() + res[x].ops_off, res[x].n_ops);
                else o.runs.n = 0;
                if (mode == MODE_CKPT) o.vsa.assign(vsa.begin() + jobs[x].vsa_off, vsa.begin() + jobs[x].vsa_off + res[x].n_vsa);
                else o.vsa.clear();
                if (mode == MODE_CKPT && jobs[x].ckpt_off >= 0) {
                    const long long ck = (long long)jobs[x].cp_count * ki->max_at * (jobs[x].Q + 1) * ki->n_states * ki->cs;
                    o.checkpoints.assign(dump.begin() + jobs[x].ckpt_off, dump.begin() + jobs[x].ckpt_off + ck);
                } else {
                    o.checkpoints.clear();
                }
            }
        });
        if (overflow) { c4h::set_error("traceback path longer than its buffer"); return -1; }
        return 0;
    }
};
```

exonerate_amd/csrc/c4_engine_passes.inc:

```
struct Segment {
    c4gpu_region region;
    int first_state;
    int final_cell[CELL_MAX];
    bool needs_checkpoints;
};

struct PairPlan {
    bool active = false, reduced = false;
    c4gpu_score region_score = 0;
    c4gpu_region ar;
    int end_from = 0;
    std::vector<Segment> segs;
};

bool model_is_global(const c4gpu_model *m) {
    return m->start_scope == C4GPU_SCOPE_CORNER && m->end_scope == C4GPU_SCOPE_CORNER;
}

struct SeqVsa { c4gpu_region region; int first_state; int final_cell[CELL_MAX]; };

int sequential_recur(Engine &eng, const ResidentSeqs &seqs, int pair, int dpmemory_mb, const c4gpu_region &region,
                     int first_state, const int *first_cell, int final_state, int *final_cell_out,
                     c4gpu_score *score_out, std::vector<SeqVsa> &leaves) {
    const c4gpu_model *m = eng.model;
    JobSpec js;
    js.pair = pair; js.region = region; js.first_state = first_state; js.final_state = final_state;
    memcpy(js.first_cell, first_cell, sizeof js.first_cell);
    js.cp_count = c4h::checkpoint_rows(m, &region, dpmemory_mb);
    std::vector<JobOut> outs;
    if (eng.run(seqs, MODE_CKPT, true, std::vector<JobSpec>(1, js), outs)) return -1;
    *score_out = outs[0].res.score;
    memcpy(final_cell_out, outs[0].res.final_cell, sizeof(int) * CELL_MAX);
    std::vector<SeqVsa> sub;
    for (int v = (int)outs[0].vsa.size() - 1; v >= 0; v--) {
        const DevVsa &dv = outs[0].vsa[v];
        SeqVsa sv;
        sv.region = c4gpu_region{dv.qs, dv.ts, dv.ql, dv.tl};
        sv.first_state = dv.first_state;
        memcpy(sv.final_cell, dv.final_cell, sizeof sv.final_cell);
        sub.push_back(sv);
    }
    for (size_t k = 0; k < sub.size(); k++) {
        if (c4h::use_reduced_space(m, &sub[k].region, dpmemory_mb)) {
            const int *sub_first = k ? sub[k - 1].final_cell : first_cell;
            const int sub_final_state = (k + 1 < sub.size()) ? sub[k + 1].first_state : final_state;
            c4gpu_score dummy;
            if (sequential_recur(eng, seqs, pair, dpmemory_mb, sub[k].region, sub[k].first_state, sub_first,
                                 sub_final_state, sub[k].final_cell, &dummy, leaves)) return -1;
        } else {
            leaves.push_back(sub[k]);
        }
    }
    return 0;
}

int sequential_reduced_path(Engine &eng, const ResidentSeqs &seqs, int pair, int dpmemory_mb,
                            const c4gpu_region &ar, c4gpu_alignment *a) {
    const c4gpu_model *m = eng.model;
    int zero[CELL_MAX] = {0}, final_cell[CELL_MAX];
    std::vector<SeqVsa> leaves;
    c4gpu_score score = 0;
    if (sequential_recur(eng, seqs, pair, dpmemory_mb, ar, m->start_state, zero, m->end_state, final_cell, &score,
                         leaves)) return -1;
    c4gpu_alignment_clear(a);
    a->score = score; a->region = ar; a->valid = 1;
    int cap = 0;
    for (size_t k = 0; k < leaves.size(); k++) {
        JobSpec js;
        js.pair = pair; js.region = leaves[k].region; js.first_state = leaves[k].first_state;
        memcpy(js.first_cell, k ? leaves[k - 1].final_cell : zero, sizeof js.first_cell);
        js.final_state = (k + 1 < leaves.size()) ? leaves[k + 1].first_state : m->end_state;
        std::vector<JobOut> outs;
        if (eng.run(seqs, MODE_PATH, true, std::vector<JobSpec>(1, js), outs)) return -1;
        memcpy(leaves[k].final_cell, outs[0].res.final_cell, sizeof(int) * CELL_MAX);
        for (uint32_t r : outs[0].runs) c4h::alignment_add(a, &cap, (int)(r >> 24), (int)(r & 0xffffff));
    }
    return 0;
}

int fused_reduced_paths(Engine &eng, const ResidentSeqs &seqs, const std::vector<int> &red, const std::vector<PairPlan> &plan,
                        int dpmemory_mb, c4gpu_alignment *alignments, std::vector<char> &done, std::map<int, JobOut> &unfinished) {
    const bool trace = c4cfg::has(c4cfg::TRACE);
    const auto t_begin = std::chrono::steady_clock::now();
    auto lap = [&](const char *what) {
        if (trace) fprintf(stderr, "c4gpu trace:   fused: %-22s at %.3f ms\n", what,
                           std::chrono::duration<double, std::milli>(std::chrono::steady_clock::now() - t_begin).count());
    };
    const c4gpu_model *m = eng.model;
    c4gpu_ctx *ctx = eng.ctx;
    const int n = (int)red.size();
    if (!n || eng.pair_sub) return 0;
    if (c4cfg::is(c4cfg::FUSED, 0)) return 0;
    const int wpe_env = c4cfg::num(c4cfg::WPE, 0);
    long long worst = 0;
    for (int i : red) worst = std::max(worst, (long long)plan[i].ar.query_length + plan[i].ar.target_length);
    const bool cont_free = eng.cont_free_ok(worst);
    const KernelInfo *kc = get_kernel(eng.family, MODE_CKPT, true, cont_free, false, wpe_env, false, 0);
    const KernelInfo *kp = get_kernel(eng.family, MODE_PATH, true, cont_free, false, wpe_env, false, 0);
    if (!kc) kc = get_kernel(eng.family, MODE_CKPT, true, false, false, wpe_env, false, 0);
    if (!kp) kp = get_kernel(eng.family, MODE_PATH, true, false, false, wpe_env, false, 0);
    if (!kc || !kp) return 0;
    const int ck_env = c4cfg::num(c4cfg::CK16, 1);
    const bool ck_root_env = !(c4cfg::is(c4cfg::CK16_ROOT, 0));
    const bool ck16_on = ck_env > 0 && cont_free && eng.pk16_params_ok && seqs.tdense_n > 0;
    const KernelInfo *kc16 = ck16_on ? get_kernel_ck16(eng.family, 0, false) : nullptr;
    const KernelInfo *kc16r = (ck16_on && ck_root_env) ? get_kernel_ck16(eng.family, ck_env == 8 ? 0 : ck_env - 1, true) : nullptr;
    const int ck16_tmax = c4cfg::num(c4cfg::CK16_TMAX, 0x7fffffff);
    hipStream_t s = ctx->stream;
    const c4h::MemRule rule{m->max_query_advance, m->max_target_advance, m->n_states, m->total_shadow_designations};
    std::vector<int> order(n), cpn(n);
    std::vector<char> group(n, 0);
    std::iota(order.begin(), order.end(), 0);
    auto cells = [&](int x) { const c4gpu_region &r = plan[red[x]].ar; return (long long)(r.query_length + 1) * (r.target_length + 1); };
    auto root_of = [&](int x) { return plan[red[x]].end_from; };
    int count_g[3] = {0, 0, 0};
    for (int x = 0; x < n; x++) {
        const c4gpu_region &r = plan[red[x]].ar;
        cpn[x] = c4h::checkpoint_rows(m, &r, dpmemory_mb);
        if (!kc16) continue;
        const bool ok = eng.pk16_fits(r.query_length, r.target_length) && r.target_length <= ck16_tmax &&
                        ((long long)r.query_length + 2) * kc16->n_states * kc16->max_at <= 65535 && cpn[x] >= 1 &&
                        r.target_length / (cpn[x] + 1) >= kc16->max_at;
        group[x] = !ok ? 0 : (kc16r && root_of(x) > 1) ? 2 : 1;
        count_g[(int)group[x]]++;
    }
    for (int g = 2; g >= 1; g--)
        if (count_g[g] == 1) {
            for (int x = 0; x < n; x++) if (group[x] == g) group[x] = (char)(g - 1);
            count_g[g - 1]++; count_g[g] = 0;
        }
    if (!count_g[1] && !count_g[2]) { kc16 = nullptr; kc16r = nullptr; }
    const int n16r = count_g[2], n16a = count_g[1], n16 = n16r + n16a;
    if (kc16r && n16r && ck_env == 1) {
        long long strips = 0;
        int rows_max = 0;
        for (int x = 0; x < n; x++)
            if (group[x] == 2) {
                strips += (plan[red[x]].ar.query_length + 1 + 255) / 256;
                rows_max = std::max(rows_max, plan[red[x]].ar.query_length + 1);
            }
        kc16r = get_kernel_ck16(eng.family, strips >= 3LL * n16r ? 8 : strips >= 2LL * n16r ? 5 : 0, true);
        if (rows_max > 1024 && rows_max <= 3 * 384 && strips >= 4LL * n16r && get_kernel_ck16(eng.family, 6, true))
            kc16r = get_kernel_ck16(eng.family, 6, true);
    }
    if (n16 && eng.ensure_ss16(seqs)) return -1;
    std::stable_sort(order.begin(), order.end(), [&](int a, int b) {
        if (group[a] != group[b]) return group[a] > group[b];
        if (group[a] == 2 && root_of(a) != root_of(b)) return root_of(a) < root_of(b);
        return cells(a) > cells(b);
    });
    if (c4cfg::has(c4cfg::TRACE))
        fprintf(stderr, "c4gpu trace:   fused: kernels %s, %s\nc4gpu trace:   fused: packed checkpoint kernels %s for %d, %s for %d of %d jobs\n",
                kc->name, kp->name, (kc16r && n16r) ? kc16r->name : "-", n16r, (kc16 && n16a) ? kc16->name : "-", n16a, n);
    std::vector<DevJob> &jobs = eng.hf_jobs;
    jobs.resize(n);
    long long vsa_total = 0, max_ckpt = 0, max_T = 0, ckpt_cells = 0, max_ckpt16 = 0, max_T16 = 0;
    bool carry = false, carry16 = false;
    int bnd16 = 0;
    for (int x = 0; x < n; x++) {
        const c4gpu_region &r = plan[red[order[x]]].ar;
        DevJob &j = jobs[x];
        memset(&j, 0, sizeof j);
        j.pair = red[order[x]]; j.q0 = r.query_start; j.t0 = r.target_start; j.Q = r.query_length; j.T = r.target_length;
        j.first_state = m->start_state; j.final_state = m->end_state;
        j.cp_count = cpn[order[x]];
        j.root = x < n16r ? root_of(order[x]) : 0;
        int tb = 0;
        while ((1LL << tb) <= j.T) tb++;
        j.tshift = tb;
        j.ckpt_off = -1; j.seed_off = -1;
        j.vsa_off = (int)vsa_total;
        vsa_total += j.cp_count + 1;
        ckpt_cells += (long long)(j.Q + 1) * (j.T + 1);
        if (x < n16) {
            const KernelInfo *k16 = x < n16r ? kc16r : kc16;
            max_ckpt16 = std::max(max_ckpt16, (long long)j.cp_count * k16->max_at * (j.Q + 1) * (x < n16r ? k16->ckw_root : k16->ckw));
            max_T16 = std::max<long long>(max_T16, j.T);
            bnd16 = std::max(bnd16, k16->bnd);
            if ((j.Q + 1 + 64 * k16->R - 1) / (64 * k16->R) > 1) carry16 = true;
        } else {
            max_ckpt = std::max(max_ckpt, (long long)j.cp_count * kc->max_at * (j.Q + 1) * kc->n_states * kc->cs);
            max_T = std::max<long long>(max_T, j.T);
            if ((j.Q + 1 + 64 * kc->R - 1) / (64 * kc->R) > kc->waves) carry = true;
        }
    }
    if (vsa_total > 0x7fffffffLL) return 0;
    std::vector<int> pair_list;
    int pairs_r = 0, pairs_a = 0;
    for (int x = 0; x < n16;) {
        const int lim = x < n16r ? n16r : n16;
        const bool two = x + 1 < lim && jobs[x + 1].root == jobs[x].root;
        pair_list.push_back(x); pair_list.push_back(two ? x + 1 : -1);
        (x < n16r ? pairs_r : pairs_a)++;
        x += two ? 2 : 1;
    }
    auto grid_for = [&](const KernelInfo *ki, long long jobs_n, long long bytes_per_wave) -> long long {
        int blocks_per_cu = 0;
        if (hipOccupancyMaxActiveBlocksPerMultiprocessor(&blocks_per_cu, ki->func, 64 * ki->waves, 0) != hipSuccess || blocks_per_cu < 1)
            blocks_per_cu = 1;
        long long grid = std::min<long long>(jobs_n, (long long)blocks_per_cu * ctx->prop.multiProcessorCount);
        const long long budget = (long long)(ctx->prop.totalGlobalMem / 4);
        if (bytes_per_wave * grid > budget) grid = std::max<long long>(1, budget / std::max<long long>(1, bytes_per_wave));
        return grid;
    };
    int zero = 0;
    unsigned long long zero64 = 0;
    {
        const int zeros[3] = {0, 0, 0};
        const int n32 = n - n16;
        const long long bnd_per_wave = (2 * ((carry ? max_T : 0) + 1) + 1) * (long long)std::max(kc->bnd, 1);
        const long long grid = n32 ? grid_for(kc, n32, bnd_per_wave * 4 + max_ckpt * 4) : 0;
        const long long bnd16_per_wave = n16 ? (2 * ((carry16 ? max_T16 : 0) + 1) + 1) * (long long)std::max(bnd16, 1) : 0;
        const long long grid16r = pairs_r ? grid_for(kc16r, pairs_r, bnd16_per_wave * 4 + 2 * max_ckpt16 * 4) : 0;
        const long long grid16a = pairs_a ? grid_for(kc16, pairs_a, bnd16_per_wave * 4 + 2 * max_ckpt16 * 4) : 0;
        const long long grid16 = std::max(grid16r, grid16a);
        if (eng.d_fjobs.upload(jobs.data(), n, s) || eng.d_fres.alloc(n) || eng.d_queue.upload(zeros, 3, s) ||
            eng.d_pairs.upload(pair_list.data(), pair_list.size(), s) ||
            eng.d_bnd.alloc(std::max(bnd_per_wave * grid, bnd16_per_wave * grid16)) || eng.d_fvsa.alloc(vsa_total) ||
            eng.d_ckpt.alloc(std::max(max_ckpt * grid, 2 * max_ckpt16 * grid16)) || eng.d_ckpt_dump.alloc(1))
            return -1;
        LaunchArgs a;
        memset(&a.scratch, 0, sizeof a.scratch);
        a.kp = eng.kparams.p; a.seqs = seqs.dev;
        a.seqs.sub_colptr = nullptr; a.seqs.sub_rows = nullptr; a.seqs.span_in = nullptr; a.seqs.span_out = nullptr;
        a.seqs.seed = nullptr;
        a.seqs.ss16 = seqs.ss16_built ? seqs.ss16.p : nullptr;
        a.vsas = eng.d_fvsa.p; a.ops = nullptr; a.stream = s;
        a.scratch.bnd = eng.d_bnd.p;
        a.scratch.ckpt_dump = eng.d_ckpt_dump.p;
        if (ctx->timing) HIP_OK(hipEventRecord(ctx->ev0, s));
        a.jobs = eng.d_fjobs.p; a.n_jobs = n16; a.results = eng.d_fres.p;
        a.scratch.bnd_stride = bnd16_per_wave; a.scratch.carry = carry16 ? 1 : 0;
        a.scratch.ckpt = eng.d_ckpt.p; a.scratch.ckpt_stride = max_ckpt16;
        if (pairs_r || pairs_a) {
            a.seqs.sub_rows = reinterpret_cast<const int *>(seqs.tcode_dense.p);
            a.seqs.sub_colptr = reinterpret_cast<const int *>(seqs.tdense.p);
        }
        if (pairs_r) {
            a.queue = eng.d_queue.p; a.grid = (int)grid16r; a.aux = eng.d_pairs.p; a.n_aux = pairs_r;
            HIP_OK(kc16r->launch(a));
        }
        if (pairs_a) {
            a.queue = eng.d_queue.p + 1; a.grid = (int)grid16a; a.aux = eng.d_pairs.p + 2 * pairs_r; a.n_aux = pairs_a;
            HIP_OK(kc16->launch(a));
        }
        a.seqs.sub_rows = nullptr; a.seqs.sub_colptr = nullptr;
        if (n32) {
            a.jobs = eng.d_fjobs.p + n16; a.n_jobs = n32; a.results = eng.d_fres.p + n16; a.queue = eng.d_queue.p + 2; a.grid = (int)grid;
            a.aux = nullptr; a.n_aux = 0;
            a.scratch.bnd_stride = bnd_per_wave; a.scratch.carry = carry ? 1 : 0;
            a.scratch.ckpt = max_ckpt ? eng.d_ckpt.p : nullptr; a.scratch.ckpt_stride = max_ckpt;
            HIP_OK(kc->launch(a));
        }
        if (ctx->timing) HIP_OK(hipEventRecord(ctx->ev1, s));
    }
    std::vector<DevResult> &res = eng.hf_res;
    res.resize(n);
    if (eng.d_fres.download(res.data(), n, s)) return -1;
    HIP_OK(c4_stream_sync(s));
    if (ctx->timing) {
        float ms = 0;
        HIP_OK(hipEventElapsedTime(&ms, ctx->ev0, ctx->ev1));
        ctx->kernel_ms[MODE_CKPT] += ms; ctx->kernel_launches[MODE_CKPT]++; ctx->kernel_cells[MODE_CKPT] += ckpt_cells;
    }
    lap("checkpoint pass");
    std::vector<int> &first = eng.hf_first;
    first.assign(n + 1, 0);
    for (int x = 0; x < n; x++) first[x + 1] = first[x] + ((res[x].flags & FLAG_NO_END) ? 0 : res[x].n_vsa);
    const long long n_sub = first[n];
    if (!n_sub) return 0;
    std::vector<unsigned long long> stats(FUSE_STATS, 0);
    if (eng.d_ffirst.upload(first.data(), n + 1, s) || eng.d_fsub_jobs.alloc(n_sub) || eng.d_fflags.alloc(n) ||
        eng.d_fstats.upload(stats.data(), FUSE_STATS, s))
        return -1;
    if (eng.d_fflags.zero(n, s)) return -1;
    hipLaunchKernelGGL(fuse_expand_kernel, dim3(n), dim3(64), 0, s, eng.d_fjobs.p, eng.d_fvsa.p, eng.d_ffirst.p, n,
                       eng.d_fsub_jobs.p, rule, dpmemory_mb, kp->R, eng.d_fflags.p, eng.d_fstats.p,
                       (c4cfg::is(c4cfg::BYROOT, 0)) ? 0 : 1);
    HIP_OK(hipGetLastError());
    if (eng.d_fstats.download(stats.data(), FUSE_STATS, s)) return -1;
    HIP_OK(c4_stream_sync(s));
    lap("jobs listed");
    const long long max_runs = (long long)stats[FUSE_MAX_OPS_CAP], max_tb = (long long)stats[FUSE_MAX_TB];
    const long long sub_T = (long long)stats[FUSE_MAX_T], ops_total = (long long)stats[FUSE_OPS_TOTAL];
    const bool sub_carry = (long long)stats[FUSE_MAX_STRIPS] > kp->waves;
    const long long bnd_per_wave = (2 * ((sub_carry ? sub_T : 0) + 1) + 1) * (long long)std::max(kp->bnd, 1);
    const long long grid = grid_for(kp, n_sub, bnd_per_wave * 4 + max_tb * 4 + max_runs * 4);
    long long runs_capacity = std::min<long long>(ops_total, std::max<long long>(1 << 20, n_sub * 256));
    unsigned long long used = 0;
    for (int attempt = 0; attempt < 2; attempt++) {
        if (eng.d_fsub_res.alloc(n_sub) || eng.d_queue.upload(&zero, 1, s) || eng.d_runs_used.upload(&zero64, 1, s) ||
            eng.d_bnd.alloc(bnd_per_wave * grid) || eng.d_runs.alloc(max_runs * grid) || eng.d_runs_out.alloc(runs_capacity) ||
            eng.d_tb.alloc(max_tb * grid))
            return -1;
        LaunchArgs a;
        memset(&a.scratch, 0, sizeof a.scratch);
        a.kp = eng.kparams.p; a.seqs = seqs.dev; a.jobs = eng.d_fsub_jobs.p; a.n_jobs = (int)n_sub; a.results = eng.d_fsub_res.p;
        a.seqs.sub_colptr = nullptr; a.seqs.sub_rows = nullptr; a.seqs.span_in = nullptr; a.seqs.span_out = nullptr;
        a.seqs.seed = nullptr;
        a.vsas = nullptr; a.ops = nullptr; a.queue = eng.d_queue.p; a.grid = (int)grid; a.stream = s;
        a.scratch.bnd = eng.d_bnd.p; a.scratch.bnd_stride = bnd_per_wave; a.scratch.carry = sub_carry ? 1 : 0;
        a.scratch.tb = max_tb ? eng.d_tb.p : nullptr; a.scratch.tb_stride = max_tb;
        a.scratch.runs = eng.d_runs.p; a.scratch.runs_stride = max_runs;
        a.scratch.runs_out = eng.d_runs_out.p; a.scratch.runs_capacity = runs_capacity;
        a.scratch.runs_used = eng.d_runs_used.p;
        if (ctx->timing) HIP_OK(hipEventRecord(ctx->ev0, s));
        HIP_OK(kp->launch(a));
        if (ctx->timing) HIP_OK(hipEventRecord(ctx->ev1, s));
        if (eng.d_runs_used.download(&used, 1, s)) return -1;
        HIP_OK(c4_stream_sync(s));
        if (ctx->timing) {
            float ms = 0;
            HIP_OK(hipEventElapsedTime(&ms, ctx->ev0, ctx->ev1));
            ctx->kernel_ms[MODE_PATH] += ms; ctx->kernel_launches[MODE_PATH]++;
        }
        if ((long long)used <= runs_capacity) break;
        if (attempt == 1) { c4h::set_error("traceback runs exceed their worst-case buffer"); return -1; }
        runs_capacity = ops_total;
    }
    lap("sub-alignment pass");
    if (eng.d_fout.alloc(2 * (size_t)std::max<unsigned long long>(used, 1)) || eng.d_fpairs.alloc(n) ||
        eng.d_runs_used.upload(&zero64, 1, s))
        return -1;
    hipLaunchKernelGGL(fuse_stitch_kernel, dim3((n + 63) / 64), dim3(64), 0, s, eng.d_fjobs.p, eng.d_fvsa.p, eng.d_ffirst.p, n,
                       eng.d_fsub_res.p, eng.d_runs_out.p, 1 + m->total_shadow_designations, eng.d_fflags.p, eng.d_runs_used.p,
                       eng.d_fout.p, eng.d_fpairs.p, n16, cell_strict() ? 1 : 0);
    HIP_OK(hipGetLastError());
    std::vector<FusePair> &fps = eng.hf_pairs;
    fps.resize(n);
    unsigned long long out_used = 0;
    if (eng.d_fpairs.download(fps.data(), n, s) || eng.d_runs_used.download(&out_used, 1, s)) return -1;
    HIP_OK(c4_stream_sync(s));
    std::vector<int> &out = eng.hf_out;
    out.resize(2 * (size_t)out_used);
    if (out_used) {
        if (eng.d_fout.download(out.data(), 2 * (size_t)out_used, s)) return -1;
        HIP_OK(c4_stream_sync(s));
    }
    lap("stitched + downloaded");
    int n_done = 0;
    for (int x = 0; x < n; x++) {
        if (fps[x].status & 1) continue;
        const int i = red[order[x]];
        c4gpu_alignment &a = alignments[i];
        a.score = res[x].score;
        a.region = plan[i].ar;
        a.valid = 1;
        a.n_ops = fps[x].count;
        if (a.n_ops) {
            a.op_transition = (int32_t *)malloc(sizeof(int32_t) * a.n_ops);
            a.op_length = (int32_t *)malloc(sizeof(int32_t) * a.n_ops);
            const int *src = out.data() + 2 * fps[x].off;
            for (int k = 0; k < a.n_ops; k++) { a.op_transition[k] = src[2 * k]; a.op_length[k] = src[2 * k + 1]; }
        }
        done[i] = 1;
        n_done++;
    }
    if (n_done < n) {
        std::vector<DevVsa> vsa((size_t)vsa_total);
        if (eng.d_fvsa.download(vsa.data(), vsa_total, s)) return -1;
        HIP_OK(c4_stream_sync(s));
        for (int x = 0; x < n; x++) {
            if (!(fps[x].status & 1)) continue;
            JobOut o;
            o.res = res[x];
            o.runs.n = 0;
            o.packed = x < n16;
            if (!(res[x].flags & FLAG_NO_END)) o.vsa.assign(vsa.begin() + jobs[x].vsa_off, vsa.begin() + jobs[x].vsa_off + res[x].n_vsa);
            unfinished[red[order[x]]] = std::move(o);
        }
    }
    if (c4cfg::has(c4cfg::TRACE))
    {
        long long score_only = 0;
        for (int x = 0; x < n; x++) score_only += fps[x].status >> 8;
        fprintf(stderr, "c4gpu trace:   fused: %d of %d pairs finished on the device route, %lld sub-alignments, %lld final cells that "
                "differ from their prediction in the score only\n", n_done, n, n_sub, score_only);
    }
    lap("alignments built");
    return 0;
}

template <class Thr>
int windowed_region_pass(Engine &eng, const ResidentSeqs &seqs, const std::vector<int> &pairs,
                         const std::vector<PairPlan> &plan, Thr thr, int kshift, std::vector<DevResult> &out) {
    const int n = (int)pairs.size();
    auto nbits = [](int v) { int b = 0; while ((1LL << b) <= v) b++; return b; };
    std::vector<JobSpec> specs(n);
    std::vector<JobOut> outs;
    for (int x = 0; x < n; x++) { specs[x].pair = pairs[x]; specs[x].region = plan[pairs[x]].ar; }
    SeedPlan sp1;
    sp1.mode = 1; sp1.kshift = kshift;
    if (eng.run(seqs, MODE_SCORE, false, specs, outs, &sp1)) return -1;
    const long long seedw = sp1.seedw;
    const int dc = sp1.dc;
    out.assign(n, DevResult());
    std::vector<int> want;
    for (int x = 0; x < n; x++) {
        out[x] = outs[x].res;
        out[x].qs = out[x].ts = 0;
        if (!outs[x].res.end_set || outs[x].res.score < thr(pairs[x])) continue;
        want.push_back(x);
    }
    const size_t wanted = want.size();
    int need_hops = 12;
    for (int x : want) need_hops = std::max(need_hops, ((outs[x].res.te - 1) >> kshift) + 2);
    const int max_hops = c4cfg::num(c4cfg::WINDOW_HOPS, std::min(need_hops, 64));
    std::vector<int> open;
    std::vector<char> demoted(n, 0);
    long long windows = 0;
    const bool strict = c4cfg::nonzero(c4cfg::STRICT);
    const int force_miss = c4cfg::num(c4cfg::FORCE_CORNER_MISMATCH, 0);
    if (sp1.fmt16) {
        std::vector<int> keep;
        for (int x : want) {
            if (outs[x].res.last_srp > 1) { keep.push_back(x); continue; }
            if (strict) { c4h::set_error("windowed region pass: the score pass did not say where END was entered from"); return -1; }
            if (c4cfg::has(c4cfg::TRACE)) fprintf(stderr, "c4gpu trace:   pair %d: no root from the packed score pass, one-pass kernel\n", pairs[x]);
            open.push_back(x); demoted[x] = 1;
        }
        want.swap(keep);
    }
    if (!want.empty()) {
        std::vector<JobSpec> hs(want.size());
        SeedPlan sp2;
        sp2.mode = 2; sp2.kshift = kshift; sp2.hops = std::max(1, max_hops); sp2.fmt16 = sp1.fmt16;
        sp2.off.resize(want.size()); sp2.rows.resize(want.size()); sp2.base.resize(want.size());
        sp2.d.resize(want.size()); sp2.t0w.resize(want.size()); sp2.t0_base.resize(want.size());
        for (size_t h = 0; h < want.size(); h++) {
            const int x = want[h];
            const c4gpu_region &ar = plan[pairs[x]].ar;
            const int d = (outs[x].res.te - 1) >> kshift;
            const int t0w = d >= 1 ? (d << kshift) - (dc - 1) : 0;
            hs[h].pair = pairs[x];
            hs[h].region = c4gpu_region{ar.query_start, ar.target_start + t0w, outs[x].res.qe, outs[x].res.te - t0w};
            hs[h].final_state = eng.model->end_state;
            if (sp1.fmt16) {
                hs[h].final_state = hs[h].root = outs[x].res.last_srp;
            }
            sp2.rows[h] = ar.query_length + 1;
            sp2.base[h] = sp1.off[x];
            sp2.off[h] = d >= 1 ? sp1.off[x] + (long long)(d - 1) * dc * (ar.query_length + 1) * seedw : -1;
            sp2.d[h] = d; sp2.t0w[h] = t0w; sp2.t0_base[h] = ar.target_start;
        }
        std::vector<JobOut> wouts;
        if (eng.run(seqs, MODE_REGION, false, hs, wouts, &sp2)) return -1;
        for (size_t h = 0; h < want.size(); h++) {
            const DevResult &r = wouts[h].res;
            DevResult &o = out[want[h]];
            if (!r.end_set || r.score != o.score || (force_miss > 0 && h % (size_t)force_miss == 0)) {
                if (c4cfg::has(c4cfg::TRACE))
                    fprintf(stderr, "c4gpu trace:   pair %d: score pass %d at (%d, %d), window corner %d (set %d): one-pass kernel\n", pairs[want[h]],
                            o.score, o.qe, o.te, r.score, (int)r.end_set);
                if (strict) { c4h::set_error("windowed region pass: a window's corner cell differs from the score pass"); return -1; }
                open.push_back(want[h]); demoted[want[h]] = 1;
                continue;
            }
            windows += r.n_vsa;
            if (r.pad >= 0) { o.qs = r.qs; o.ts = r.ts; }
            else open.push_back(want[h]);
        }
    }
    if (!open.empty()) {
        std::vector<JobSpec> fs(open.size());
        for (size_t h = 0; h < open.size(); h++) { fs[h].pair = pairs[open[h]]; fs[h].region = plan[pairs[open[h]]].ar; }
        if (eng.run(seqs, MODE_REGION, false, fs, outs)) return -1;
        for (size_t h = 0; h < open.size(); h++) {
            const DevResult &r = outs[h].res;
            DevResult &o = out[open[h]];
            if (r.score != o.score || r.qe != o.qe || r.te != o.te) {
                if (c4cfg::has(c4cfg::TRACE))
                    fprintf(stderr, "c4gpu trace:   pair %d: score pass %d at (%d, %d), one-pass kernel %d at (%d, %d)\n", pairs[open[h]],
                            o.score, o.qe, o.te, r.score, r.qe, r.te);
                if (strict || !demoted[open[h]]) {
                    c4h::set_error("windowed region pass: the one-pass kernel disagrees with the score pass");
                    return -1;
                }
                o = r;
            }
            o.qs = r.qs; o.ts = r.ts;
            if (demoted[open[h]]) o.last_srp = 0;
        }
    }
    const std::vector<int> &hops = open;
    const long long round = windows;
    if (wanted >= 64 && !force_miss) {
        const double rate = 1.0 - (double)hops.size() / (double)wanted;
        eng.ctx->window_rate = eng.ctx->window_rate < 0 ? rate : 0.5 * eng.ctx->window_rate + 0.5 * rate;
    }
    if (c4cfg::has(c4cfg::TRACE))
        fprintf(stderr, "c4gpu trace: windowed region pass: %d pairs, dumps every %d columns, %lld windows in one launch, %zu of %zu "
                "paths left to the one-pass kernel\n", n, 1 << kshift, round, hops.size(), wanted);
    return 0;
}
```

exonerate_amd/csrc/c4_engine_staging.inc:

```
template <class M>
bool model_matches(const c4gpu_model &m) {
    if (m.n_states != M::NS || m.n_transitions != M::NT || m.n_calcs != M::NC || m.n_shadows != M::NSH) return false;
    if (m.start_state != M::START || m.end_state != M::END || m.total_shadow_designations != M::NDES) return false;
    for (int k = 0; k < M::NT; k++) {
        const c4gpu_transition &t = m.transitions[k];
        const TrDesc &d = M::tr[k];
        if (t.input != d.in || t.output != d.out || t.advance_query != d.aq || t.advance_target != d.at ||
            t.calc != d.calc || t.label != d.label || t.dst_shadow_mask != d.dst_shadow_mask) return false;
    }
    for (int c = 0; c < M::NC; c++) {
        const int kind = m.calcs[c].kind, dk = M::calc[c].kind;
        const bool both_11 = (kind == C4GPU_CALC_MATCH_DNA || kind == C4GPU_CALC_MATCH_PROTEIN) &&
                             (dk == C4GPU_CALC_MATCH_DNA || dk == C4GPU_CALC_MATCH_PROTEIN);
        if (!both_11 && kind != dk) return false;
        if (kind >= C4GPU_CALC_SPLICE_PRE && m.calcs[c].param != M::calc[c].param) return false;
        if (m.calcs[c].protect != M::calc[c].protect) return false;
    }
    for (int s = 0; s < M::NSH; s++) {
        if (m.shadows[s].designation != M::sh[s].designation || m.shadows[s].on_target != M::sh[s].on_target ||
            m.shadows[s].src_state_mask != M::sh[s].src_state_mask ||
            m.shadows[s].dst_transition_mask != M::sh[s].dst_transition_mask) return false;
    }
    return true;
}
// ... 116 lines not shown
    }
  }
}

__global__ void splice_kernel(const uint8_t *__restrict__ seq, const long long *off, const int *len, int n_seqs,
                              const c4gpu_splice_model *__restrict__ models, int *__restrict__ out,
                              long long stride) {
  const int type = blockIdx.z;
  const c4gpu_splice_model *sp = &models[type];
  for (int pair = blockIdx.y; pair < n_seqs; pair += gridDim.y) {
    const uint8_t *s = seq + off[pair];
    const int n = len[pair];
    int *o = out + (long long)type * stride + off[pair];
    for (int pos = blockIdx.x * blockDim.x + threadIdx.x; pos < n; pos += gridDim.x * blockDim.x) {
        int seq_start = pos - sp->splice_after, model_start = 0, calc_length = sp->model_length;
        if (seq_start < 0) { model_start = -seq_start; seq_start = 0; calc_length -= model_start; }
        if (seq_start + calc_length > n) calc_length = n - seq_start;
        float score = 0.0f;
        for (int i = 0; i < calc_length; i++) score = score + sp->data[model_start + i][sp->index[s[seq_start + i]]];
        if (sp->gtag_only) {
            const int b1 = s[pos], b2 = pos + 1 < n ? s[pos + 1] : 0;
            const int u1 = (b1 >= 'a' && b1 <= 'z') ? b1 - 32 : b1, u2 = (b2 >= 'a' && b2 <= 'z') ? b2 - 32 : b2;
            if (u1 != sp->expect_one || u2 != sp->expect_two) score = -987654321.0f;
        }
        const double r = score < 0 ? (double)score - 0.5 : (double)score + 0.5;
        o[pos] = (int)r;
    }
  }
}

struct SpliceFold { int add[4]; };
constexpr int SPLICE_TILE = 1024, SPLICE_HALO = C4GPU_SPLICE_MAX_LEN;
__global__ __launch_bounds__(256) void splice_tile_kernel(const uint8_t *__restrict__ seq, const long long *off, const int *len, int n_seqs,
                                                          const c4gpu_splice_model *__restrict__ models, int *__restrict__ out,
                                                          long long stride, SpliceFold fold, uint2 *__restrict__ out16) {
    __shared__ float sdata[4][C4GPU_SPLICE_MAX_LEN * 5];
    __shared__ uint8_t sindex[4][256];
    __shared__ __attribute__((aligned(16))) uint8_t scol[4][SPLICE_TILE + 2 * SPLICE_HALO + 16];
    __shared__ __attribute__((aligned(16))) uint8_t sraw[SPLICE_TILE + 16];
    __shared__ int s_mlen[4], s_after[4], s_gtag[4], s_e1[4], s_e2[4];
    const int tid = threadIdx.x;
    for (int x = tid; x < 4 * C4GPU_SPLICE_MAX_LEN * 5; x += 256) sdata[x / (C4GPU_SPLICE_MAX_LEN * 5)][x % (C4GPU_SPLICE_MAX_LEN * 5)] =
        models[x / (C4GPU_SPLICE_MAX_LEN * 5)].data[(x % (C4GPU_SPLICE_MAX_LEN * 5)) / 5][x % 5];
    for (int x = tid; x < 4 * 256; x += 256) sindex[x >> 8][x & 255] = models[x >> 8].index[x & 255];
    if (tid < 4) {
        s_mlen[tid] = models[tid].model_length; s_after[tid] = models[tid].splice_after; s_gtag[tid] = models[tid].gtag_only;
        s_e1[tid] = models[tid].expect_one; s_e2[tid] = models[tid].expect_two;
    }
    __syncthreads();
    for (int pair = blockIdx.y; pair < n_seqs; pair += gridDim.y) {
        const uint8_t *s = seq + off[pair];
        const int n = len[pair];
        for (int tile = blockIdx.x * SPLICE_TILE; tile < n; tile += gridDim.x * SPLICE_TILE) {
            __syncthreads();
            const int lo = tile - SPLICE_HALO;
            for (int x = tid; x < SPLICE_TILE + 2 * SPLICE_HALO; x += 256) {
                const int p = lo + x;
                const uint8_t b = (p >= 0 && p < n) ? s[p] : 0;
                for (int k = 0; k < 4; k++) scol[k][x] = sindex[k][b];
            }
            for (int x = tid; x < SPLICE_TILE + 2; x += 256) sraw[x] = (tile + x < n) ? s[tile + x] : 0;
            __syncthreads();
            const int p0 = tile + 4 * tid;
            if (p0 >= n) continue;
            int v[4][4];
            for (int k = 0; k < 4; k++) {
                const int mlen = s_mlen[k], after = s_after[k];
                const float *d = sdata[k];
                const uint8_t *c = scol[k] + (p0 - after - lo);
                float sc[4] = {0.0f, 0.0f, 0.0f, 0.0f};
                if (p0 - after >= 0 && p0 + 3 - after + mlen <= n) {
                    unsigned w = (unsigned)c[0] | ((unsigned)c[1] << 8) | ((unsigned)c[2] << 16);
                    for (int i = 0; i < mlen; i++) {
                        w |= (unsigned)c[i + 3] << 24;
                        const float *row = d + 5 * i;
                        sc[0] = sc[0] + row[w & 0xff];
                        sc[1] = sc[1] + row[(w >> 8) & 0xff];
                        sc[2] = sc[2] + row[(w >> 16) & 0xff];
                        sc[3] = sc[3] + row[w >> 24];
                        w >>= 8;
                    }
                } else {
                    for (int q = 0; q < 4; q++) {
                        const int pos = p0 + q;
                        if (pos >= n) break;
                        int seq_start = pos - after, model_start = 0, calc_length = mlen;
                        if (seq_start < 0) { model_start = -seq_start; seq_start = 0; calc_length -= model_start; }
                        if (seq_start + calc_length > n) calc_length = n - seq_start;
                        float score = 0.0f;
                        for (int i = 0; i < calc_length; i++) score = score + d[5 * (model_start + i) + scol[k][seq_start + i - lo]];
                        sc[q] = score;
                    }
                }
                for (int q = 0; q < 4; q++) {
                    float score = sc[q];
                    if (s_gtag[k]) {
                        const int pos = p0 + q;
                        const int b1 = sraw[4 * tid + q], b2 = pos + 1 < n ? sraw[4 * tid + q + 1] : 0;
                        const int u1 = (b1 >= 'a' && b1 <= 'z') ? b1 - 32 : b1, u2 = (b2 >= 'a' && b2 <= 'z') ? b2 - 32 : b2;
                        if (u1 != s_e1[k] || u2 != s_e2[k]) score = -987654321.0f;
                    }
                    const double r = score < 0 ? (double)score - 0.5 : (double)score + 0.5;
                    v[k][q] = (int)r;
                }
            }
            const long long base = off[pair] + p0;
            if (p0 + 3 < n) {
                for (int k = 0; k < 4; k++)
                    *reinterpret_cast<int4 *>(out + (long long)k * stride + base) = make_int4(v[k][0], v[k][1], v[k][2], v[k][3]);
            } else {
                for (int k = 0; k < 4; k++)
                    for (int q = 0; q < 4 && p0 + q < n; q++) out[(long long)k * stride + base + q] = v[k][q];
            }
            if (out16) {
                auto c16 = [](int x) { return x < -32768 ? -32768 : (x > 32767 ? 32767 : x); };
                for (int q = 0; q < 4 && p0 + q < n; q++) {
                    uint2 o;
                    o.x = ((unsigned)c16(fold.add[0] + v[0][q]) & 0xffffu) | ((unsigned)c16(fold.add[1] + v[1][q]) << 16);
                    o.y = ((unsigned)c16(fold.add[2] + v[2][q]) & 0xffffu) | ((unsigned)c16(fold.add[3] + v[3][q]) << 16);
                    out16[base + q] = o;
                }
            }
        }
    }
}

struct HspJob { long long qoff, toff; int qlen, tlen; };
__device__ __forceinline__ c4gpu_hsp hsp_extend_one(const uint8_t *__restrict__ qcode, const uint8_t *__restrict__ tcode, const HspJob jb,
                                                     const c4gpu_hsp_seed sd, const int *sm, int aq, int at, int seedlen, int dropoff) {
        const uint8_t *q = qcode + jb.qoff, *t = tcode + jb.toff;
        auto sc = [&](int qp, int tp) { return sm[q[qp] * 24 + t[tp]]; };
        int qs = sd.query_start, ts = sd.target_start, length = seedlen, i;
        for (i = 0; i < length; i++) {
            if (sc(qs, ts) > 0) break;
            qs += aq; ts += at;
        }
        length -= i;
        int qp = qs + length * aq - aq, tp = ts + length * at - at;
        while (length > 0) {
            if (sc(qp, tp) > 0) break;
            length--; qp -= aq; tp -= at;
        }
        int score = 0;
        for (i = 0, qp = qs, tp = ts; i < length; i++, qp += aq, tp += at) score += sc(qp, tp);
        int maxscore = score, extend, maxext;
        qp = qs - aq; tp = ts - at;
        for (extend = 1, maxext = 0; qp >= 0 && tp >= 0; extend++) {
            score += sc(qp, tp);
            if (maxscore <= score) { maxscore = score; maxext = extend; }
            else { if (score < 0) break; if (maxscore - score >= dropoff) break; }
            qp -= aq; tp -= at;
        }
        qp = qs + length * aq; tp = ts + length * at;
        qs -= maxext * aq; ts -= maxext * at; length += maxext;
        score = maxscore;
        for (extend = 1, maxext = 0; qp + aq <= jb.qlen && tp + at <= jb.tlen; extend++) {
            score += sc(qp, tp);
            if (maxscore <= score) { maxscore = score; maxext = extend; }
            else { if (score < 0) break; if (maxscore - score >= dropoff) break; }
            qp += aq; tp += at;
        }
        length += maxext;
        score = 0;
        for (i = 0, qp = qs, tp = ts; i < length; i++, qp += aq, tp += at) {
            score += sc(qp, tp);
            if (score >= (maxscore >> 1)) break;
        }
        return c4gpu_hsp{qs, ts, length, maxscore, i};
}

__global__ void hsp_extend_kernel(const uint8_t *__restrict__ qcode, const uint8_t *__restrict__ tcode,
                                  const HspJob *__restrict__ jobs, const c4gpu_hsp_seed *__restrict__ seeds, int n_seeds,
                                  const int *__restrict__ submat, int aq, int at, int seedlen, int dropoff,
                                  c4gpu_hsp *__restrict__ out) {
    __shared__ int sm[24 * 24];
    for (int x = threadIdx.x; x < 24 * 24; x += blockDim.x) sm[x] = submat[x];
    __syncthreads();
    for (int k = blockIdx.x * blockDim.x + threadIdx.x; k < n_seeds; k += gridDim.x * blockDim.x)
        out[k] = hsp_extend_one(qcode, tcode, jobs[seeds[k].pair], seeds[k], sm, aq, at, seedlen, dropoff);
}

__global__ void hsp_chain_kernel(const uint8_t *__restrict__ qcode, const uint8_t *__restrict__ tcode,
                                 const HspJob *__restrict__ jobs, const c4gpu_hsp_seed *__restrict__ seeds,
                                 const int *__restrict__ order, const int *__restrict__ chain_first, int n_chains,
                                 const int *__restrict__ horizon0, const int *__restrict__ submat, int aq, int at, int seedlen,
                                 int dropoff, c4gpu_hsp *__restrict__ out) {
    __shared__ int sm[24 * 24];
    for (int x = threadIdx.x; x < 24 * 24; x += blockDim.x) sm[x] = submat[x];
    __syncthreads();
    for (int c = blockIdx.x * blockDim.x + threadIdx.x; c < n_chains; c += gridDim.x * blockDim.x) {
        int horizon = horizon0[c];
        for (int x = chain_first[c]; x < chain_first[c + 1]; x++) {
            const int k = order[x];
            if (seeds[k].target_start < horizon) { out[k] = c4gpu_hsp{0, 0, -1, 0, 0}; continue; }
            const c4gpu_hsp h = hsp_extend_one(qcode, tcode, jobs[seeds[k].pair], seeds[k], sm, aq, at, seedlen, dropoff);
            out[k] = h;
            horizon = h.target_start + h.length * at;
        }
    }
}

__global__ void subopt_colptr_kernel(const DevJob *jobs, int n_jobs, const int *pts_t, const int *pts_q, int *colent) {
    constexpr int SUB_NONE = -0x40000000;
    for (int x = blockIdx.x; x < n_jobs; x += gridDim.x) {
        const DevJob &j = jobs[x];
        const int *pt = pts_t + j.sub_pt_off;
        const int *pq = pts_q + j.sub_pt_off;
        const int n = j.sub_pt_n;
        for (int k = threadIdx.x; k <= n; k += blockDim.x) {
            const int first = k == 0 ? 0 : pt[k - 1] + 1;
            const int last = k == n ? j.T + 1 : pt[k];
            const int idx2 = 2 * (j.sub_pt_off + k);
            for (int c = first; c <= last; c++) {
                const bool own = k < n && c == last;
                const bool more = own && k + 1 < n && pt[k + 1] == c;
                int *e = colent + 2 * (j.sub_off + c);
                e[0] = own ? pq[k] : SUB_NONE;
                e[1] = idx2 | (more ? 1 : 0);
            }
        }
    }
}

enum { FUSE_MAX_OPS_CAP = 0, FUSE_MAX_TB, FUSE_MAX_T, FUSE_MAX_STRIPS, FUSE_OPS_TOTAL, FUSE_STATS };

__device__ __forceinline__ unsigned long long wave_max_u64(unsigned long long v) {
    for (int off = 32; off > 0; off >>= 1) { const unsigned long long o = __shfl_xor(v, off); v = o > v ? o : v; }
    return v;
}
__device__ __forceinline__ unsigned long long wave_sum_u64(unsigned long long v) {
    for (int off = 32; off > 0; off >>= 1) v += __shfl_xor(v, off);
    return v;
}

__global__ __launch_bounds__(64) void fuse_expand_kernel(const DevJob *parents, const DevVsa *vsa, const int *first, int n_parents,
                                                         DevJob *out, c4h::MemRule rule, int dpmemory_mb, int path_R,
                                                         int *flags, unsigned long long *stats, int keep_root) {
    const int x = blockIdx.x;
    if (x >= n_parents) return;
    const DevJob &pj = parents[x];
    const int base = first[x], cnt = first[x + 1] - base;
    unsigned long long m_cap = 0, m_tb = 0, m_T = 0, m_strips = 0, ops = 0;
    bool nested = false;
    for (int k = threadIdx.x; k < cnt; k += 64) {
        const DevVsa &dv = vsa[pj.vsa_off + (cnt - 1 - k)];
        DevJob j;
        memset(&j, 0, sizeof j);
        j.pair = pj.pair; j.q0 = dv.qs; j.t0 = dv.ts; j.Q = dv.ql; j.T = dv.tl;
        j.root = keep_root ? pj.root : 0;
        j.first_state = dv.first_state;
        j.final_state = (k + 1 < cnt) ? vsa[pj.vsa_off + (cnt - 2 - k)].first_state : pj.final_state;
        const int *fc = k > 0 ? vsa[pj.vsa_off + (cnt - k)].final_cell : pj.first_cell;
        for (int l = 0; l < CELL_MAX; l++) j.first_cell[l] = fc[l];
        int tb = 0;
        while ((1LL << tb) <= j.T) tb++;
        j.tshift = tb;
        j.ckpt_off = -1; j.seed_off = -1;
        j.ops_cap = 3 * (j.Q + j.T) + 16;
        out[base + k] = j;
        nested |= c4h::use_reduced_space(rule, dv.ql, dv.tl, dpmemory_mb);
        const unsigned long long strips = (unsigned long long)(j.Q + 1 + 64 * path_R - 1) / (unsigned long long)(64 * path_R);
        const unsigned long long tbw = strips * (unsigned long long)(j.T + 64) * 64ull * (unsigned long long)path_R;
        m_cap = m_cap > (unsigned long long)j.ops_cap ? m_cap : (unsigned long long)j.ops_cap;
        m_tb = m_tb > tbw ? m_tb : tbw;
        m_T = m_T > (unsigned long long)j.T ? m_T : (unsigned long long)j.T;
        m_strips = m_strips > strips ? m_strips : strips;
        ops += (unsigned long long)j.ops_cap;
    }
    m_cap = wave_max_u64(m_cap); m_tb = wave_max_u64(m_tb); m_T = wave_max_u64(m_T); m_strips = wave_max_u64(m_strips);
    ops = wave_sum_u64(ops);
    const bool any_nested = __builtin_amdgcn_ballot_w64(nested) != 0;
    if (threadIdx.x == 0) {
        if (any_nested) flags[x] = 1;
        atomicMax(&stats[FUSE_MAX_OPS_CAP], m_cap); atomicMax(&stats[FUSE_MAX_TB], m_tb); atomicMax(&stats[FUSE_MAX_T], m_T);
        atomicMax(&stats[FUSE_MAX_STRIPS], m_strips); atomicAdd(&stats[FUSE_OPS_TOTAL], ops);
    }
}

__global__ void memrule_probe_kernel(c4h::MemRule rule, int dpmemory_mb, const int *ql, const int *tl, int n, int *reduced, int *rows) {
    const int x = blockIdx.x * blockDim.x + threadIdx.x;
    if (x >= n) return;
    reduced[x] = c4h::use_reduced_space(rule, ql[x], tl[x], dpmemory_mb) ? 1 : 0;
    rows[x] = c4h::viterbi_row_bytes(rule, ql[x], 1 + rule.total_shadow_designations + 1) ? c4h::checkpoint_rows(rule, ql[x], tl[x], dpmemory_mb) : -1;
}

struct FusePair { long long off; int count, status; };

__host__ __device__ inline bool final_cell_equiv(const int *computed, const int *predicted, int n_slots, int target_end, bool packed,
                                                 bool strict_score = false) {
    if (strict_score && computed[0] != predicted[0]) return false;
    const long long shift = (long long)computed[0] - (long long)predicted[0];
    if (shift > 4096 || shift < -4096) return false;
    for (int l = 1; l < n_slots; l++) {
        if (computed[l] == predicted[l]) continue;
        if (!(packed && (long long)target_end - predicted[l] - 2 >= 32767 && (long long)target_end - computed[l] - 2 >= 32767)) return false;
    }
    return true;
}

inline bool cell_strict() { return c4cfg::nonzero(c4cfg::CELL_STRICT); }

__global__ void fuse_stitch_kernel(const DevJob *parents, const DevVsa *vsa, const int *first, int n_parents,
                                   const DevResult *sub, const uint32_t *runs, int path_cs, const int *flags,
                                   unsigned long long *out_used, int *out, FusePair *pairs, int n_packed, int strict_score) {
    const int x = blockIdx.x * blockDim.x + threadIdx.x;
    if (x >= n_parents) return;
    FusePair fp; fp.off = 0; fp.count = 0; fp.status = 1;
    const int base = first[x], cnt = first[x + 1] - base;
    if (flags[x] || cnt == 0) { pairs[x] = fp; return; }
    const DevJob &pj = parents[x];
    long long total = 0;
    bool bad = false;
    int score_only = 0;
    for (int k = 0; k < cnt; k++) {
        const DevResult &r = sub[base + k];
        if (r.flags & (FLAG_OPS_OVERFLOW | FLAG_NO_END)) { bad = true; break; }
        total += r.n_ops;
        if (k + 1 < cnt) {
            const DevVsa &dv = vsa[pj.vsa_off + (cnt - 1 - k)];
            bad |= !final_cell_equiv(r.final_cell, dv.final_cell, path_cs, dv.ts + dv.tl, x < n_packed, strict_score != 0);
            if (bad) break;
            score_only += r.final_cell[0] != dv.final_cell[0];
        }
    }
    if (bad) { pairs[x] = fp; return; }
    const long long off = (long long)atomicAdd(out_used, (unsigned long long)total);
    int *o = out + 2 * off;
    int n = 0;
    for (int k = 0; k < cnt; k++) {
        const DevResult &r = sub[base + k];
        const uint32_t *w = runs + r.ops_off;
        for (int q = r.n_ops - 1; q >= 0; q--) {
            const int tr = (int)(w[q] >> 24), len = (int)(w[q] & 0xffffff);
            if (n && o[2 * (n - 1)] == tr) {
                o[2 * (n - 1) + 1] += len;
                if (o[2 * (n - 1) + 1] == 0) n--;
            } else {
                o[2 * n] = tr; o[2 * n + 1] = len; n++;
            }
        }
    }
    fp.off = off; fp.count = n; fp.status = score_only << 8;
    pairs[x] = fp;
}

__global__ void annotate_qcode_kernel(uint8_t *qcode, const long long *qoff, const int *cds, int n_pairs) {
    const int p = blockIdx.x;
    if (p >= n_pairs) return;
    const int start = cds[3 * p], length = cds[3 * p + 1], qlen = cds[3 * p + 2];
    if (length <= 0) return;
    const int a = start < 0 ? 0 : start;
    const long long e = (long long)start + length;
    const int b = e > qlen ? qlen : (int)e;
    for (int i = a + (int)threadIdx.x; i < b; i += (int)blockDim.x) qcode[qoff[p] + i] = 24;
}

struct ResidentSeqs {
    int n_pairs = 0;
    std::vector<long long> qoff, toff;
    std::vector<int> qlen, tlen;
    long long total_q = 0, total_t = 0;
    DevBuf<uint8_t> qraw, traw, qcode, tcode;
    DevBuf<long long> d_qoff, d_toff;
    DevBuf<int> d_qlen, d_tlen, ss;
    DevBuf<uint16_t> tn4;
    mutable DevBuf<uint2> ss16;
    mutable bool ss16_built = false;
    mutable std::mutex ss16_lock;
    DevBuf<uint8_t> tdense;
    int tdense_n = 0;
    DevBuf<uint8_t> tcode_dense;
    long long ss_len = 0;
    DevBuf<PrepTables> tables;
    DevBuf<c4gpu_splice_model> splice_models;
    DevBuf<int> bad;
    DevSeqs dev;

    int n_utargets = 0;
    DevBuf<long long> d_utoff;
    DevBuf<int> d_utlen;
    DevBuf<long long> d_uqoff;
    DevBuf<int> d_uqlen;

    PinBuf pin_q, pin_t;

    int build(c4gpu_ctx *ctx, int family, const c4gpu_params *params, const c4gpu_pair *pairs, int n, bool pin = false,
              const SpliceFold *fold16 = nullptr) {
        const bool trace = c4cfg::has(c4cfg::TRACE);
        const auto t_begin = std::chrono::steady_clock::now();
        auto lap = [&](const char *what) {
            if (trace) fprintf(stderr, "c4gpu trace: staging: %-24s at %.3f ms\n", what,
                               std::chrono::duration<double, std::milli>(std::chrono::steady_clock::now() - t_begin).count());
        };
        n_pairs = n;
        qoff.resize(n); toff.resize(n); qlen.resize(n); tlen.resize(n);
        total_q = total_t = 0;
        std::map<std::pair<const uint8_t *, int>, long long> qseen, tseen;
        std::vector<int> uq, ut;
        std::vector<long long> utoff, uqoff;
        std::vector<int> utlen, uqlen;
        for (int i = 0; i < n; i++) {
            qlen[i] = pairs[i].query_len; tlen[i] = pairs[i].target_len;
            if (qlen[i] < 0 || tlen[i] < 0 || tlen[i] >= (1 << 30) || qlen[i] >= (1 << 30)) {
                c4h::set_error("sequence length outside [0, 2^30): the kernels address a sequence with 32-bit byte offsets");
                return -1;
            }
            auto qk = std::make_pair(pairs[i].query, qlen[i]);
            auto qi = qseen.find(qk);
            if (qi == qseen.end()) {
                qseen[qk] = total_q; qoff[i] = total_q; uq.push_back(i);
                total_q += (qlen[i] + 3) & ~3LL;
            } else qoff[i] = qi->second;
            auto tk = std::make_pair(pairs[i].target, tlen[i]);
            auto ti = tseen.find(tk);
            if (ti == tseen.end()) {
                tseen[tk] = total_t; toff[i] = total_t; ut.push_back(i);
                utoff.push_back(total_t); utlen.push_back(tlen[i]);
                total_t += (tlen[i] + 3) & ~3LL;
            } else toff[i] = ti->second;
        }
        n_utargets = (int)ut.size();
        const size_t hq_n = (size_t)total_q + 64, ht_n = (size_t)total_t + 64;
        std::unique_ptr<uint8_t[]> own_q, own_t;
        uint8_t *hq = nullptr, *ht = nullptr;
        if (pin) {
            if (pin_q.reserve(hq_n) || pin_t.reserve(ht_n)) return -1;
            hq = pin_q.p; ht = pin_t.p;
        } else {
            own_q.reset(new uint8_t[hq_n]); own_t.reset(new uint8_t[ht_n]);
            hq = own_q.get(); ht = own_t.get();
        }
        hipStream_t s = ctx->stream;
        if (qraw.alloc(hq_n) || traw.alloc(ht_n)) return -1;
        auto gather = [&](uint8_t *dst, const std::vector<int> &uniq, bool query, size_t ua, size_t ub) {
            parallel_for((long long)(ub - ua), 16, [&](long long first, long long last) {
                for (long long x = (long long)ua + first; x < (long long)ua + last; x++) {
                    const int i = uniq[x];
                    const int len = query ? qlen[i] : tlen[i];
                    uint8_t *d = dst + (query ? qoff[i] : toff[i]);
                    if (len) memcpy(d, query ? pairs[i].query : pairs[i].target, len);
                    for (int k = len; k < ((len + 3) & ~3); k++) d[k] = 'A';
                }
            });
        };
        auto side = [&](uint8_t *host, uint8_t *devp, const std::vector<int> &uniq, bool query, long long total, size_t host_n) -> int {
            const size_t slice = pin ? (size_t)32 << 20 : ~(size_t)0;
            size_t ua = 0;
            long long sent = 0;
            while (ua < uniq.size()) {
                size_t ub = ua;
                long long end = sent;
                while (ub < uniq.size() && (size_t)(end - sent) < slice) {
                    const int i = uniq[ub++];
                    end = (query ? qoff[i] : toff[i]) + (((query ? qlen[i] : tlen[i]) + 3) & ~3LL);
                }
                gather(host, uniq, query, ua, ub);
                if (pin && end > sent) HIP_OK(hipMemcpyAsync(devp + sent, host + sent, (size_t)(end - sent), hipMemcpyHostToDevice, s));
                sent = end; ua = ub;
            }
            memset(host + total, 'A', 64);
            if (pin) HIP_OK(hipMemcpyAsync(devp + total, host + total, 64, hipMemcpyHostToDevice, s));
            else HIP_OK(hipMemcpyAsync(devp, host, host_n, hipMemcpyHostToDevice, s));
            return 0;
        };
        if (side(hq, qraw.p, uq, true, total_q, hq_n) || side(ht, traw.p, ut, false, total_t, ht_n)) return -1;
        lap("sequences gathered");
        PrepTables pt;
        memcpy(pt.submat_index, params->submat_index, 256);
        memcpy(pt.nt2d, params->nt2d, 256);
        memcpy(pt.trans, params->trans, 4096);
        memcpy(pt.aa, params->aa, 40);
        if (tables.upload(&pt, 1, s) ||
            qcode.alloc(hq_n) || tcode.alloc(ht_n) || d_qoff.upload(qoff.data(), n, s) ||
            d_toff.upload(toff.data(), n, s) || d_qlen.upload(qlen.data(), n, s) || d_tlen.upload(tlen.data(), n, s) ||
            d_utoff.upload(utoff.data(), n_utargets, s) || d_utlen.upload(utlen.data(), n_utargets, s))
            return -1;
        if (trace) { HIP_OK(c4_stream_sync(s)); lap("uploaded"); }
        int zero[2] = {0, 0};
        if (bad.upload(zero, 2, s)) return -1;
        const int blocks = 1024;
        int max_t = 1, max_q = 1;
        for (int i = 0; i < n; i++) { max_t = std::max(max_t, tlen[i]); max_q = std::max(max_q, qlen[i]); }
        if (family_is_codon(family)) {
            uqoff.resize(uq.size()); uqlen.resize(uq.size());
            for (size_t x = 0; x < uq.size(); x++) { uqoff[x] = qoff[uq[x]]; uqlen[x] = qlen[uq[x]]; }
            const int nuq = (int)uq.size();
            if (d_uqoff.upload(uqoff.data(), nuq, s) || d_uqlen.upload(uqlen.data(), nuq, s)) return -1;
            hipLaunchKernelGGL(codon_kernel, dim3(std::min(256, (max_q + 255) / 256), std::max(1, std::min(nuq, 32768))), dim3(256), 0, s,
                               qraw.p, qcode.p, d_uqoff.p, d_uqlen.p, nuq, tables.p, bad.p);
        } else {
            hipLaunchKernelGGL(encode_kernel, dim3(blocks), dim3(256), 0, s, qraw.p, qcode.p, (long long)hq_n, tables.p, bad.p);
        }
        const int xb = std::min(256, (max_t + 255) / 256), yb = std::max(1, std::min(n_utargets, 32768));
        if (family_is_p2d(family)) {
            hipLaunchKernelGGL(codon_kernel, dim3(xb, yb), dim3(256), 0, s, traw.p, tcode.p, d_utoff.p, d_utlen.p, n_utargets, tables.p, bad.p);
        } else {
            hipLaunchKernelGGL(encode_kernel, dim3(blocks), dim3(256), 0, s, traw.p, tcode.p, (long long)ht_n, tables.p, bad.p, bad.p + 1);
        }
        dev.ss = nullptr;
        dev.ss16 = nullptr;
        dev.ss_stride = 0;
        ss16_built = false;
        if (family_has_splice(family)) {
            if (splice_models.upload(params->splice, 4, s) || ss.alloc((size_t)4 * ht_n)) return -1;
            bool tiled = !(c4cfg::is(c4cfg::SPLICE_TILE, 0));
            for (int k = 0; k < 4; k++)
                tiled = tiled && params->splice[k].splice_after >= 0 && params->splice[k].splice_after <= SPLICE_HALO &&
                        params->splice[k].model_length >= 0 && params->splice[k].model_length <= C4GPU_SPLICE_MAX_LEN;
            if (tiled) {
                if (fold16 && ss16.alloc(ht_n)) return -1;
                const int tiles = std::max(1, std::min(4096, (max_t + SPLICE_TILE - 1) / SPLICE_TILE));
                hipLaunchKernelGGL(splice_tile_kernel, dim3(tiles, yb), dim3(256), 0, s, traw.p, d_utoff.p, d_utlen.p, n_utargets,
                                   splice_models.p, ss.p, (long long)ht_n, fold16 ? *fold16 : SpliceFold{{0, 0, 0, 0}},
                                   fold16 ? ss16.p : (uint2 *)nullptr);
                if (fold16) { ss16_built = true; dev.ss16 = nullptr; }
            } else
            hipLaunchKernelGGL(splice_kernel, dim3(xb, yb, 4), dim3(256), 0, s, traw.p, d_utoff.p, d_utlen.p, n_utargets,
                               splice_models.p, ss.p, (long long)ht_n);
            dev.ss = ss.p;
            dev.ss_stride = (long long)ht_n;
            ss_len = (long long)ht_n;
        }
        dev.tn4 = nullptr;
        if (family_has_phase(family)) {
            if (tn4.alloc(ht_n)) return -1;
            hipLaunchKernelGGL(tn4_kernel, dim3(xb, yb), dim3(256), 0, s, traw.p, tn4.p, d_utoff.p, d_utlen.p, n_utargets, tables.p);
            dev.tn4 = tn4.p;
        }
        HIP_OK(hipGetLastError());
        lap("kernels queued");
        int hbad2[2] = {0, 0};
        if (bad.download(hbad2, 2, s)) return -1;
        HIP_OK(c4_stream_sync(s));
        const int hbad = hbad2[0];
        tdense_n = 0;
        if (!family_is_p2d(family) && hbad2[1]) {
            uint8_t tab[32];
            memset(tab, 0xff, 24);
            memset(tab + 24, 0, 8);
            int nd = 0;
            for (int c = 0; c < 24; c++)
                if (hbad2[1] >> c & 1) { if (nd < 8) { tab[c] = (uint8_t)nd; tab[24 + nd] = (uint8_t)c; } nd++; }
            if (nd <= 8) {
                if (tdense.upload(tab, 32, s) || tcode_dense.alloc(ht_n)) return -1;
                hipLaunchKernelGGL(dense_kernel, dim3(blocks), dim3(256), 0, s, tcode.p, tcode_dense.p, (long long)ht_n, tdense.p);
                HIP_OK(hipGetLastError());
                HIP_OK(c4_stream_sync(s));
                tdense_n = nd;
            }
        }
        lap("coded, splice arrays built");
        if (hbad) {
            c4h::set_error(hbad == 2 ? "a target codon translates outside the substitution matrix alphabet (non-IUPAC base?)"
                                     : "a residue is outside the 24-letter substitution matrix alphabet "
                                       "(exonerate's Submat index would read out of bounds, submat.c:27-61)");
            return -1;
        }
        dev.qcode = qcode.p; dev.tcode = tcode.p; dev.qoff = d_qoff.p; dev.toff = d_toff.p; dev.tlen = d_tlen.p;
        return 0;
    }

    void swap_with(ResidentSeqs &o) {
        std::swap(n_pairs, o.n_pairs);
        qoff.swap(o.qoff); toff.swap(o.toff); qlen.swap(o.qlen); tlen.swap(o.tlen);
        std::swap(total_q, o.total_q); std::swap(total_t, o.total_t);
        qraw.swap(o.qraw); traw.swap(o.traw); qcode.swap(o.qcode); tcode.swap(o.tcode);
        d_qoff.swap(o.d_qoff); d_toff.swap(o.d_toff); d_qlen.swap(o.d_qlen); d_tlen.swap(o.d_tlen); ss.swap(o.ss);
        tn4.swap(o.tn4); ss16.swap(o.ss16); std::swap(ss16_built, o.ss16_built);
        tdense.swap(o.tdense); std::swap(tdense_n, o.tdense_n); std::swap(ss_len, o.ss_len); tcode_dense.swap(o.tcode_dense);
        tables.swap(o.tables); splice_models.swap(o.splice_models); bad.swap(o.bad);
        std::swap(dev, o.dev);
        std::swap(n_utargets, o.n_utargets); d_utoff.swap(o.d_utoff); d_utlen.swap(o.d_utlen);
        d_uqoff.swap(o.d_uqoff); d_uqlen.swap(o.d_uqlen);
        std::swap(pin_q.p, o.pin_q.p); std::swap(pin_q.n, o.pin_q.n); std::swap(pin_t.p, o.pin_t.p); std::swap(pin_t.n, o.pin_t.n);
    }
};
```

exonerate_amd/csrc/c4_win16_kernel.h:

```cpp
#pragma once
#include "c4_ckpt16_kernel.h"

namespace c4k {

template <class M, int R, int ROOT>
struct WaveWin16 {
    using F = Facts<M>;
    static_assert(M::MAXAQ == 1, "the packed forms exchange exactly one query row per step");
    using D16 = Dump16<M>;
    using RT = Roots<M>;
    static constexpr int NS = M::NS, NCOL = M::MAXAT + 1, W = 64 * R, MAXAT = M::MAXAT, DC = M::MAXAT;
    static constexpr int SEEDW = D16::SEEDW16;
    static constexpr bool live(int s) { return D16::live(s); }
    static constexpr bool inner(int s) { return RT::member(ROOT, s); }
    static constexpr bool exported(int s) { return inner(s) && F::exported(s); }
    static constexpr int n_exp() { int n = 0; for (int s = 0; s < NS; s++) n += exported(s); return n; }
    static constexpr int n_exp_live() { int n = 0; for (int s = 0; s < NS; s++) n += (exported(s) && live(s)); return n; }
    static constexpr int n_exp_live_all() { int n = 0; for (int s = 0; s < NS; s++) n += (F::exported(s) && live(s)); return n; }
    static constexpr int BND_ALL = F::n_exported() * 3 + n_exp_live_all();
    static constexpr int BND = n_exp() * 3 + n_exp_live();
    static constexpr int CS = 1 + M::NDES + 2;
    static_assert(!F::has_phase(), "split-codon calcs are not packed");
    static_assert(M::NDES <= 1, "one shadow designation");
    static_assert(M::START == 0 && M::END == 1, "state numbering of the closed model");
    static_assert(!F::exported(M::START), "START advances nothing");
    static_assert(NS * DC < 0x8000, "entry-cell identity in 16 bits");
    struct C16 { int sc[NS]; int il[NS]; int rq[NS]; int rt[NS]; };
    typedef __attribute__((address_space(3))) int lds_int;
    __device__ __forceinline__ static lds_int *lds_at(int a) { return (lds_int *)(size_t)(unsigned)a; }
    __device__ __forceinline__ static int lds_addr(const lds_int *p) { return (int)(unsigned)(size_t)p; }
    using P16 = Prof16<R>;
    using ST = Stage16<BND>;

    const KParams *kp;
    int lane;
    const uint8_t *qc[2], *tc[2];
    const uint2 *ss16[2];
    const int *seed_rd[2];
    int Q[2], T[2], q0[2], t0[2], tlast[2], seed_rows[2], final_state[2];
    bool seeded[2];
    int Qm, Tm;
    int open_il_pk, lim_pk, fifteen, at_pk[4], cv_pk[16];
    C16 col[NCOL][R], nbr[NCOL], expo, nx_carry;
    int prof_a[2];
    const uint8_t *tdense;
    int nx_sp4[4], nx_off[2], nx_prof[2 * P16::NP];
    int stage_a, stage_base, carry_a, carry_base;
    bool carry_cols;
    int corner_sc[2], corner_rq[2], corner_rt[2];
    bool corner_set[2];

    template <class Fn>
    __device__ __forceinline__ static void for_exported(Fn &&fn) {
        int slot = 0;
        static_for<NS>([&](auto S_) __attribute__((always_inline)) { constexpr int S = S_;
            if constexpr (exported(S)) { fn(S_, slot); slot += 3 + (live(S) ? 1 : 0); }
        });
    }
    __device__ __forceinline__ static void write_empty_column(int *colp) {
        for_exported([&](auto S_, int slot) __attribute__((always_inline)) { constexpr int S = S_;
            colp[slot] = NEG16; colp[slot + 1] = 0; colp[slot + 2] = 0;
            if constexpr (live(S)) colp[slot + 3] = 0;
        });
    }
    __device__ __forceinline__ void prefetch_carry() {
        const lds_int *p = lds_at(carry_a);
        for_exported([&](auto S_, int slot) __attribute__((always_inline)) { constexpr int S = S_;
            nx_carry.sc[S] = p[slot * ST::COLS];
            nx_carry.rq[S] = p[(slot + 1) * ST::COLS];
            nx_carry.rt[S] = p[(slot + 2) * ST::COLS];
            if constexpr (live(S)) nx_carry.il[S] = p[(slot + 3) * ST::COLS];
        });
        carry_a = ((carry_a + 4) & (ST::COLS * 4 - 1)) | carry_base;
    }
    __device__ __forceinline__ void fill_carry(lds_int *stage, int c0, const int *bnd_in) {
        const int c = c0 + lane;
        const int jx = c < 0 ? 0 : (c > Tm ? Tm : c);
        const int jc = carry_cols ? jx : 0;
        const int *g = bnd_in + (long long)jc * BND;
        int v[BND];
        static_for<BND>([&](auto K_) __attribute__((always_inline)) { constexpr int K = K_; v[K] = g[K]; });
        lds_int *p = stage + ST::CARRY0 * ST::COLS + (c & (ST::COLS - 1));
        static_for<BND>([&](auto K_) __attribute__((always_inline)) { constexpr int K = K_; p[K * ST::COLS] = v[K]; });
    }
    template <int H>
    __device__ __forceinline__ void build_profile(int i0) {
        using P16 = Prof16<R>;
        typedef __attribute__((address_space(3))) int lds_int;
        int qr[R];
        static_for<R>([&](auto RR_) __attribute__((always_inline)) { constexpr int RR = RR_;
            const int i = i0 + RR;
            qr[RR] = 24 * ((i >= 1 && i <= Q[H]) ? (int)qc[H][q0[H] + i - 1] : 0);
        });
        for (int d = 0; d < P16::NCODE; d++) {
            const int code = tdense[24 + d];
            int v[R];
            static_for<R>([&](auto RR_) __attribute__((always_inline)) { constexpr int RR = RR_; v[RR] = kp->submat[qr[RR] + code]; });
            lds_int *p = (lds_int *)(size_t)(unsigned)(prof_a[H] + d * P16::CODE);
            static_for<P16::NP>([&](auto K_) __attribute__((always_inline)) { constexpr int K = K_;
                p[K] = pk_pack(v[2 * K], v[2 * K + 1 < R ? 2 * K + 1 : 2 * K]);
            });
        }
    }
    __device__ __forceinline__ void prefetch_column() {
        const lds_int *p = lds_at(stage_a);
        static_for<4>([&](auto K_) __attribute__((always_inline)) { constexpr int K = K_; nx_sp4[K] = p[K * ST::COLS]; });
        nx_off[0] = p[4 * ST::COLS]; nx_off[1] = p[5 * ST::COLS];
        stage_a = ((stage_a + 4) & (ST::COLS * 4 - 1)) | stage_base;
    }
    __device__ __forceinline__ void prefetch_profile() {
        const lds_int *pa = lds_at(prof_a[0] + nx_off[0]), *pb = lds_at(prof_a[1] + nx_off[1]);
        static_for<P16::NP>([&](auto K_) __attribute__((always_inline)) { constexpr int K = K_; nx_prof[K] = pa[K]; nx_prof[P16::NP + K] = pb[K]; });
    }
    __device__ __forceinline__ void fill_stage(lds_int *stage, int c0) {
        constexpr int mat = F::match_at();
        const int c = c0 + lane;
        uint2 sv[2]; int off[2];
        static_for<2>([&](auto H_) __attribute__((always_inline)) { constexpr int H = H_;
            int ti = t0[H] + c - mat;
            ti = ti < 0 ? 0 : (ti > tlast[H] ? tlast[H] : ti);
            off[H] = (int)tc[H][(unsigned)ti] * P16::CODE;
            sv[H] = uint2{0u, 0u};
            if constexpr (F::has_splice()) {
                int tp = t0[H] + c - 2;
                tp = tp < 0 ? 0 : (tp > tlast[H] ? tlast[H] : tp);
                sv[H] = ss16[H][(unsigned)tp];
            }
        });
        lds_int *p = stage + (c & (ST::COLS - 1));
        p[0 * ST::COLS] = (int)__builtin_amdgcn_perm(sv[1].x, sv[0].x, 0x05040100u);
        p[1 * ST::COLS] = (int)__builtin_amdgcn_perm(sv[1].x, sv[0].x, 0x07060302u);
        p[2 * ST::COLS] = (int)__builtin_amdgcn_perm(sv[1].y, sv[0].y, 0x05040100u);
        p[3 * ST::COLS] = (int)__builtin_amdgcn_perm(sv[1].y, sv[0].y, 0x07060302u);
        p[4 * ST::COLS] = off[0]; p[5 * ST::COLS] = off[1];
    }

    template <int RR, int PH, bool JINT>
    __device__ __forceinline__ void eval_cell(int j, int ms, const int (&sp)[4], int ipk, int jpk) {
        C16 &c = col[PH][RR];
        static_for<M::NT>([&](auto K_) __attribute__((always_inline)) { constexpr int K = K_;
            constexpr TrDesc t = M::tr[K];
            if constexpr (!inner(t.out)) return;
            static_assert(!(t.in == M::START && F::code(K) == 1), "a state's first transition is never the one out of START");
            constexpr int PD = (PH - t.at + NCOL) % NCOL;
            const C16 &src = (t.aq == 0) ? col[PD][RR] : (RR > 0 ? col[PD][RR > 0 ? RR - 1 : 0] : nbr[PD]);
            int cand, rqc, rtc, ilc = 0;
            if constexpr (t.in == M::START) {
                static_assert(t.in != M::START || (t.aq == 0 && t.at == 0 && t.calc < 0), "START leaves silently");
                cand = 0; rqc = ipk; rtc = jpk;
            } else {
                cand = src.sc[t.in];
                rqc = src.rq[t.in];
                rtc = src.rt[t.in];
                if constexpr (t.calc >= 0) {
                    constexpr CalcDesc cd = M::calc[t.calc];
                    if constexpr (cd.kind == CALC_CONST) cand = pk_add<1>(cand, cv_pk[t.calc]);
                    else if constexpr (cd.kind >= CALC_MATCH_DNA && cd.kind <= CALC_MATCH_P2D) cand = pk_add<1>(cand, ms);
                    else if constexpr (cd.kind == CALC_SPLICE_PRE) cand = pk_add<1>(cand, sp[cd.param]);
                    else if constexpr (cd.kind == CALC_SPLICE_POST) {
                        static_assert(live(t.in), "post-splice calc without a length");
                        const int bad = pk_neg_mask(src.il[t.in], fifteen);
                        const int sv = bfi32(bad, NEG16, sp[cd.param]);
                        cand = pk_add<1>(cand, sv);
                    }
                }
                if constexpr (!JINT && t.at > 0) cand = (j >= t.at) ? cand : NEG16;
                if constexpr (live(t.out)) {
                    if constexpr (F::owns_shadow(t.in, 0)) ilc = open_il_pk;
                    else if constexpr (live(t.in)) ilc = pk_add<1>(src.il[t.in], at_pk[t.at]);
                }
            }
            if constexpr (F::code(K) == 1) {
                c.sc[t.out] = cand;
                c.rq[t.out] = rqc;
                c.rt[t.out] = rtc;
                if constexpr (live(t.out)) c.il[t.out] = ilc;
            } else {
                const int win = pk_lt_mask<1>(c.sc[t.out], cand, 0);
                c.rq[t.out] = bfi32(win, rqc, c.rq[t.out]);
                c.rt[t.out] = bfi32(win, rtc, c.rt[t.out]);
                if constexpr (live(t.out)) c.il[t.out] = bfi32(win, ilc, c.il[t.out]);
                c.sc[t.out] = pk_max<1>(c.sc[t.out], cand);
            }
        });
    }

    template <bool JINT, int PH>
    __device__ __forceinline__ void step(int s, int i0, bool last_strip, const int *bnd_in, int *bnd_out) {
        const int j = s - lane;
        int ms[R];
        static_for<P16::NP>([&](auto K_) __attribute__((always_inline)) { constexpr int K = K_;
            const int ea = nx_prof[K], eb = nx_prof[P16::NP + K];
            ms[2 * K] = (int)__builtin_amdgcn_perm((unsigned)eb, (unsigned)ea, 0x05040100u);
            if constexpr (2 * K + 1 < R) ms[2 * K + 1] = (int)__builtin_amdgcn_perm((unsigned)eb, (unsigned)ea, 0x07060302u);
        });
        int sp[4];
        static_for<4>([&](auto K_) __attribute__((always_inline)) { constexpr int K = K_; sp[K] = nx_sp4[K]; });
        for_exported([&](auto S_, int) __attribute__((always_inline)) { constexpr int S = S_;
            nbr[PH].sc[S] = dpp_shr1(nx_carry.sc[S], expo.sc[S]);
            nbr[PH].rq[S] = dpp_shr1(nx_carry.rq[S], expo.rq[S]);
            nbr[PH].rt[S] = dpp_shr1(nx_carry.rt[S], expo.rt[S]);
            if constexpr (live(S)) nbr[PH].il[S] = dpp_shr1(nx_carry.il[S], expo.il[S]);
        });
        prefetch_carry();
        prefetch_column();
        const int jpk = (j & 0xffff) | (j << 16);
        static_for<R>([&](auto RR_) __attribute__((always_inline)) { constexpr int RR = RR_;
            const int i = i0 + RR;
            eval_cell<RR, PH, JINT>(j, ms[RR], sp, i | (i << 16), jpk);
            if constexpr (RR == (R + 1) / 2 - 1) prefetch_profile();
        });
        if constexpr (!JINT) {
            if (s < DC + 64) {
                const bool early = (j >= 0) & (j < DC);
                const bool sd0 = early & seeded[0], sd1 = early & seeded[1];
                if (__builtin_amdgcn_ballot_w64(sd0 | sd1)) {
                    const int sdm = (sd0 ? 0x0000ffff : 0) | (sd1 ? (int)0xffff0000u : 0);
                    const int jc = j < 0 ? 0 : (j > DC - 1 ? DC - 1 : j);
                    static_for<R>([&](auto RR_) __attribute__((always_inline)) { constexpr int RR = RR_;
                        const int i = i0 + RR;
                        int w[2][SEEDW];
                        static_for<2>([&](auto H_) __attribute__((always_inline)) { constexpr int H = H_;
                            const int ic = i > seed_rows[H] - 1 ? seed_rows[H] - 1 : i;
                            const int *p = seed_rd[H] + ((long long)jc * seed_rows[H] + ic) * SEEDW;
                            static_for<SEEDW>([&](auto K_) __attribute__((always_inline)) { constexpr int K = K_; w[H][K] = p[K]; });
                        });
                        const int ident = 0x8000 | (i & 0x7fff);
                        const int ident_pk = ident | (ident << 16);
                        static_for<NS>([&](auto S_) __attribute__((always_inline)) { constexpr int S = S_;
                            if constexpr (inner(S)) {
                                constexpr int hs = D16::half_of_sc(S);
                                const int v = (int)__builtin_amdgcn_perm((unsigned)w[1][hs / 2], (unsigned)w[0][hs / 2],
                                                                         (hs & 1) ? 0x07060302u : 0x05040100u);
                                col[PH][RR].sc[S] = bfi32(sdm, v, col[PH][RR].sc[S]);
                                if constexpr (live(S)) {
                                    constexpr int hl = D16::half_of_il(S);
                                    const int vl = (int)__builtin_amdgcn_perm((unsigned)w[1][hl / 2], (unsigned)w[0][hl / 2],
                                                                              (hl & 1) ? 0x07060302u : 0x05040100u);
                                    col[PH][RR].il[S] = bfi32(sdm, pk_sub(vl, lim_pk), col[PH][RR].il[S]);
                                }
                                col[PH][RR].rq[S] = bfi32(sdm, ident_pk, col[PH][RR].rq[S]);
                                const int st = S * DC + jc;
                                col[PH][RR].rt[S] = bfi32(sdm, st | (st << 16), col[PH][RR].rt[S]);
                            }
                        });
                    });
                }
            }
        }
        for_exported([&](auto S_, int) __attribute__((always_inline)) { constexpr int S = S_;
            expo.sc[S] = col[PH][R - 1].sc[S];
            expo.rq[S] = col[PH][R - 1].rq[S];
            expo.rt[S] = col[PH][R - 1].rt[S];
            if constexpr (live(S)) expo.il[S] = col[PH][R - 1].il[S];
        });
        if (!last_strip && lane == 63 && j >= 0 && j <= Tm) {
            for_exported([&](auto S_, int slot) __attribute__((always_inline)) { constexpr int S = S_;
                int *p = bnd_out + (long long)j * BND + slot;
                p[0] = expo.sc[S];
                p[1] = expo.rq[S];
                p[2] = expo.rt[S];
                if constexpr (live(S)) p[3] = expo.il[S];
            });
        }
        static_for<2>([&](auto H_) __attribute__((always_inline)) { constexpr int H = H_;
            if (s >= T[H]) {
                const bool mine = (j == T[H]) & (Q[H] >= i0) & (Q[H] < i0 + R);
                if (__builtin_amdgcn_ballot_w64(mine)) {
                    static_for<R>([&](auto RR_) __attribute__((always_inline)) { constexpr int RR = RR_;
                        if (mine & (i0 + RR == Q[H])) {
                            static_for<NS>([&](auto S_) __attribute__((always_inline)) { constexpr int S = S_;
                                if constexpr (inner(S)) {
                                    if (final_state[H] == S) {
                                        corner_sc[H] = pk_half(col[PH][RR].sc[S], H);
                                        corner_rq[H] = (int)(((unsigned)col[PH][RR].rq[S] >> (16 * H)) & 0xffffu);
                                        corner_rt[H] = (int)(((unsigned)col[PH][RR].rt[S] >> (16 * H)) & 0xffffu);
                                        corner_set[H] = true;
                                    }
                                }
                            });
                        }
                    });
                }
            }
        });
    }

    template <int NW>
    __device__ __forceinline__ void run(const DevJob &ja, const DevJob &jb, const DevSeqs &seqs, int *bnd, int wid, int *prog, lds_int *stage) {
        const DevJob *jp[2] = {&ja, &jb};
        static_for<2>([&](auto H_) __attribute__((always_inline)) { constexpr int H = H_;
            const DevJob &jx = *jp[H];
            Q[H] = jx.Q; T[H] = jx.T; q0[H] = jx.q0; t0[H] = jx.t0;
            tlast[H] = seqs.tlen[jx.pair] > 0 ? seqs.tlen[jx.pair] - 1 : 0;
            qc[H] = seqs.qcode + seqs.qoff[jx.pair];
            tc[H] = reinterpret_cast<const uint8_t *>(seqs.sub_rows) + seqs.toff[jx.pair];
            ss16[H] = F::has_splice() ? seqs.ss16 + seqs.toff[jx.pair] : nullptr;
            seeded[H] = jx.seed_off >= 0;
            seed_rd[H] = seqs.seed + (seeded[H] ? jx.seed_off : 0);
            seed_rows[H] = jx.seed_rows > 0 ? jx.seed_rows : 1;
            final_state[H] = jx.final_state;
            corner_sc[H] = LOW; corner_rq[H] = 0; corner_rt[H] = 0; corner_set[H] = false;
        });
        Qm = Q[0] > Q[1] ? Q[0] : Q[1]; Tm = T[0] > T[1] ? T[0] : T[1];
        static_for<M::NC>([&](auto CI_) __attribute__((always_inline)) { constexpr int CI = CI_;
            const int v = clamp16(kp->calc_value[CI]);
            cv_pk[CI] = pk_pack(v, v);
        });
        static_for<4>([&](auto A_) __attribute__((always_inline)) { constexpr int A = A_; at_pk[A] = pk_pack(A, A); });
        {
            const int lim = clamp16(kp->min_intron - 4);
            lim_pk = pk_pack(lim, lim);
            open_il_pk = pk_pack(-lim, -lim);
            fifteen = 0x000f000f;
        }
        const int nstrips = (Qm + 1 + W - 1) / W;
        const int nsteps = Tm + 64;
        const int main_lo = 63 + (MAXAT > DC ? MAXAT : DC), main_hi = Tm;
        const int nsteps_r = (nsteps + NCOL - 1) / NCOL * NCOL;
        const int main_lo_r = (main_lo + NCOL - 1) / NCOL * NCOL;
        constexpr int CHK = (63 / NCOL) * NCOL;
        const int PS = nsteps_r + 1;
        stage_base = lds_addr(stage);
        carry_base = stage_base + ST::CARRY0 * ST::COLS * 4;
        for (int b = wid; b < nstrips; b += NW) {
            const int i0 = b * W + lane * R;
            stage_a = stage_base + ((0 - lane) & (ST::COLS - 1)) * 4;
            carry_a = carry_base;
            static_for<2>([&](auto H_) __attribute__((always_inline)) { constexpr int H = H_; build_profile<H>(i0); });
            static_for<NS>([&](auto S_) __attribute__((always_inline)) { constexpr int S = S_;
                expo.sc[S] = NEG16; expo.il[S] = 0; expo.rq[S] = 0; expo.rt[S] = 0;
                static_for<NCOL>([&](auto D_) __attribute__((always_inline)) { constexpr int D = D_;
                    nbr[D].sc[S] = NEG16; nbr[D].il[S] = 0; nbr[D].rq[S] = 0; nbr[D].rt[S] = 0;
                    static_for<R>([&](auto RR_) __attribute__((always_inline)) { constexpr int RR = RR_;
                        col[D][RR].sc[S] = NEG16; col[D][RR].il[S] = 0; col[D][RR].rq[S] = 0; col[D][RR].rt[S] = 0;
                    });
                });
            });
            __builtin_amdgcn_fence(__ATOMIC_ACQUIRE, "workgroup");
            const bool first = (b == 0), last = (b == nstrips - 1);
            carry_cols = !first;
            const int *bnd_in = first ? bnd : bnd + BND + (long long)((b + 1) & 1) * (Tm + 1) * BND;
            int *bnd_out = bnd + BND + (long long)(b & 1) * (Tm + 1) * BND;
            auto group = [&](auto JI_, int s0) __attribute__((always_inline)) {
                constexpr bool JI = decltype(JI_)::value != 0;
                static_for<NCOL>([&](auto P_) __attribute__((always_inline)) { constexpr int P = P_;
                    step<JI, P>(s0 + P, i0, last, bnd_in, bnd_out);
                });
            };
            {
                const int above = (wid + NW - 1) % NW, above_base = ((b - 1) / NW) * PS, my_base = (b / NW) * PS;
                auto wait_above = [&](int c1) __attribute__((always_inline)) {
                    if constexpr (NW == 1) return;
                    if (first) return;
                    const int need = above_base + (c1 + 64 < nsteps_r ? c1 + 64 : nsteps_r);
                    while (__hip_atomic_load(prog + above, __ATOMIC_RELAXED, __HIP_MEMORY_SCOPE_WORKGROUP) < need) __builtin_amdgcn_s_sleep(1);
                    __builtin_amdgcn_fence(__ATOMIC_ACQUIRE, "workgroup");
                };
                fill_stage(stage, -63);
                wait_above(CHK < nsteps_r ? CHK : nsteps_r);
                fill_carry(stage, -63, bnd_in);
                prefetch_column();
                prefetch_profile();
                prefetch_carry();
                for (int c0 = 0; c0 < nsteps_r; c0 += CHK) {
                    const int c1 = c0 + CHK < nsteps_r ? c0 + CHK : nsteps_r;
                    fill_stage(stage, c0 + 1);
                    if (c0) wait_above(c1);
                    fill_carry(stage, c0 + 1, bnd_in);
                    int s = c0;
                    for (; s < main_lo_r && s < c1; s += NCOL) group(IC<0>{}, s);
                    for (; s + NCOL - 1 <= main_hi && s < c1; s += NCOL) group(IC<1>{}, s);
                    for (; s < c1; s += NCOL) group(IC<0>{}, s);
                    if constexpr (NW > 1) {
                        if (!last) {
                            __builtin_amdgcn_fence(__ATOMIC_RELEASE, "workgroup");
                            if (lane == 0) __hip_atomic_store(prog + wid, my_base + c1, __ATOMIC_RELAXED, __HIP_MEMORY_SCOPE_WORKGROUP);
                        }
                    }
                }
            }
            __builtin_amdgcn_fence(__ATOMIC_RELEASE, "workgroup");
        }
    }
};

template <class M, int R, int ROOT, int NW>
__device__ __forceinline__ void win16_chains(const KParams *kp_lds, const DevSeqs &seqs, DevJob *job_lds, int *more, int ia, int ib,
                                             DevResult *results, int *bnd, int *prog, int (*corner_lds)[4], int *prof_mem,
                                             const uint8_t *tdense, int *stage_mem) {
    using DP = WaveWin16<M, R, ROOT>;
    int hop = 0, first_score = 0;
    bool active = threadIdx.x < 2 && more[threadIdx.x & 1];
    const int wid = __builtin_amdgcn_readfirstlane((int)(threadIdx.x >> 6));
    for (;;) {
        DP dp{};
        dp.kp = kp_lds;
        dp.lane = threadIdx.x & 63;
        dp.tdense = tdense;
        {
            typedef __attribute__((address_space(3))) int lds_int;
            for (int h = 0; h < 2; h++)
                dp.prof_a[h] = (int)(unsigned)(size_t)((lds_int *)prof_mem + (wid * 2 + h) * Prof16<R>::INTS) + dp.lane * Prof16<R>::EB;
        }
        if constexpr (NW > 1) {
            if (threadIdx.x < NW) prog[threadIdx.x] = 0;
            if (threadIdx.x < 2) corner_lds[threadIdx.x][3] = 0;
            __syncthreads();
        }
        dp.template run<NW>(job_lds[0], job_lds[1], seqs, bnd, wid, prog, (typename DP::lds_int *)stage_mem + wid * DP::ST::INTS);
        int sc[2], rq[2], rt[2];
        bool set[2];
        if constexpr (NW == 1) {
            for (int h = 0; h < 2; h++) {
                const unsigned long long owners = __ballot(dp.corner_set[h]);
                const int owner = owners ? __ffsll((long long)owners) - 1 : 0;
                sc[h] = __shfl(dp.corner_sc[h], owner); rq[h] = __shfl(dp.corner_rq[h], owner); rt[h] = __shfl(dp.corner_rt[h], owner);
                set[h] = owners != 0;
            }
            __syncthreads();
        } else {
            for (int h = 0; h < 2; h++)
                if (dp.corner_set[h]) {
                    corner_lds[h][0] = dp.corner_sc[h]; corner_lds[h][1] = dp.corner_rq[h]; corner_lds[h][2] = dp.corner_rt[h];
                    corner_lds[h][3] = 1;
                }
            __syncthreads();
            for (int h = 0; h < 2; h++) {
                sc[h] = corner_lds[h][0]; rq[h] = corner_lds[h][1]; rt[h] = corner_lds[h][2]; set[h] = corner_lds[h][3] != 0;
            }
        }
        if (active) {
            const int h = threadIdx.x;
            DevJob &job = job_lds[h];
            if (hop == 0) first_score = sc[h];
            const bool ident = (rq[h] & 0x8000) != 0;
            bool go_on = false;
            DevResult res;
            res.flags = set[h] ? 0 : FLAG_NO_END; res.n_ops = 0; res.last_srp = 0; res.ops_off = 0;
            res.cell_size = DP::CS;
            for (int l = 0; l < CELL_MAX; l++) res.final_cell[l] = 0;
            res.score = first_score; res.end_set = set[h]; res.qe = job.Q; res.te = job.T; res.qs = 0; res.ts = 0;
            res.n_vsa = hop + 1; res.pad = ident ? -1 : 0;
            if (set[h] && !ident) {
                res.qs = rq[h]; res.ts = rt[h] + job.win_t0w;
            } else if (set[h] && job.win_d >= 1 && hop + 1 < job.win_hops) {
                constexpr int DC = DP::DC;
                const int row = rq[h] & 0x7fff, jc = rt[h] % DC, state = rt[h] / DC;
                const int d2 = job.win_d - 1, t0w2 = d2 >= 1 ? (d2 << job.seed_kshift) - (DC - 1) : 0;
                const int endcol = job.win_t0w + jc;
                job.Q = row; job.final_state = state;
                job.T = endcol - t0w2; job.t0 = job.win_t0_base + t0w2;
                job.seed_off = d2 >= 1 ? job.seed_base + (long long)(d2 - 1) * DC * job.seed_rows * DP::SEEDW : -1;
                job.win_d = d2; job.win_t0w = t0w2;
                go_on = true;
            }
            if (!go_on) {
                results[h ? ib : ia] = res;
                more[h] = 0;
                active = false;
                job.Q = 0; job.T = DP::DC; job.seed_off = -1;
            }
        }
        hop++;
        __syncthreads();
        if (!(more[0] | more[1])) break;
        __syncthreads();
    }
}

template <class M, int R, int WPE, int NW = 1>
__global__ __launch_bounds__(64 * NW) __attribute__((amdgpu_waves_per_eu(WPE, 8)))
void win16_kernel(const KParams *kparams, DevSeqs seqs, const DevJob *jobs, const int *pairs, int n_pairs, DevResult *results,
                  DevScratch scratch, int *queue) {
    using RT = Roots<M>;
    constexpr int STAGE_BND = WaveWin16<M, R, RT::disjoint() ? RT::root(0) : -1>::BND;
    static_assert(!RT::disjoint() || STAGE_BND == WaveWin16<M, R, RT::root(RT::count() - 1)>::BND, "one stage layout for every root");
    __shared__ __attribute__((aligned(512))) int stage_mem[NW * Stage16<STAGE_BND>::INTS];
    __shared__ int next_job;
    __shared__ DevJob job_lds[2];
    __shared__ int more[2];
    __shared__ int prog[NW];
    __shared__ int corner_lds[2][4];
    __shared__ __attribute__((aligned(16))) int prof_mem[NW * 2 * Prof16<R>::INTS];
    __shared__ uint8_t tdense_lds[32];
    if (threadIdx.x < 32) tdense_lds[threadIdx.x] = reinterpret_cast<const uint8_t *>(seqs.sub_colptr)[threadIdx.x];
    __syncthreads();
    const KParams *kp_lds = kparams;
    int *bnd = scratch.bnd + (long long)blockIdx.x * scratch.bnd_stride;
    for (;;) {
        if (threadIdx.x == 0) next_job = atomicAdd(queue, 1);
        __syncthreads();
        const int pid = __builtin_amdgcn_readfirstlane(next_job);
        __syncthreads();
        if (pid >= n_pairs) break;
        const int ia = pairs[2 * pid], ib = pairs[2 * pid + 1];
        if (threadIdx.x < 2) {
            const int h = threadIdx.x;
            const bool real = h == 0 || ib >= 0;
            job_lds[h] = jobs[real ? (h ? ib : ia) : ia];
            more[h] = real ? 1 : 0;
            if (!real) { job_lds[h].Q = 0; job_lds[h].T = M::MAXAT; job_lds[h].seed_off = -1; }
        }
        __syncthreads();
        const int root = job_lds[0].root;
        bool ran = false;
        if constexpr (RT::disjoint()) {
            static_for<RT::count()>([&](auto X_) __attribute__((always_inline)) { constexpr int X = X_;
                constexpr int ROOT = RT::root(X);
                if (!ran && root == ROOT) {
                    if (threadIdx.x == 0) WaveWin16<M, R, ROOT>::write_empty_column(bnd);
                    __builtin_amdgcn_fence(__ATOMIC_RELEASE, "workgroup");
                    __syncthreads();
                    win16_chains<M, R, ROOT, NW>(kp_lds, seqs, job_lds, more, ia, ib, results, bnd, prog, corner_lds, prof_mem, tdense_lds, stage_mem);
                    ran = true;
                }
            });
        }
        if constexpr (!RT::disjoint()) {
            if (threadIdx.x == 0) WaveWin16<M, R, -1>::write_empty_column(bnd);
            __builtin_amdgcn_fence(__ATOMIC_RELEASE, "workgroup");
            __syncthreads();
            win16_chains<M, R, -1, NW>(kp_lds, seqs, job_lds, more, ia, ib, results, bnd, prog, corner_lds, prof_mem, tdense_lds, stage_mem);
        } else if (!ran) {
            if (threadIdx.x < 2 && more[threadIdx.x]) {
                DevResult res;
                res.flags = FLAG_NO_END; res.n_ops = 0; res.last_srp = 0; res.ops_off = 0; res.cell_size = 0; res.score = LOW;
                res.end_set = 0; res.qe = res.te = res.qs = res.ts = 0; res.n_vsa = 0; res.pad = -1;
                for (int l = 0; l < CELL_MAX; l++) res.final_cell[l] = 0;
                results[threadIdx.x ? ib : ia] = res;
            }
        }
        __syncthreads();
    }
}

}
```

exonerate_amd/csrc/kernels/kwin16_families.hip:

```cpp
#include "../c4_launch.h"
#include "../c4_win16_kernel.h"
namespace c4k {
#define WIN16_KERNEL(NAME, M, RV, WPEV, NWV)                                                                            \
    static hipError_t NAME##_launch(const LaunchArgs &a) {                                                            \
        hipLaunchKernelGGL((win16_kernel<M, RV, WPEV, NWV>), dim3(a.grid), dim3(64 * NWV), 0, a.stream, a.kp, a.seqs, a.jobs, \
                           a.aux, a.n_aux, a.results, a.scratch, a.queue);                                             \
        return hipGetLastError();                                                                                      \
    }                                                                                                                  \
    static const KernelInfo NAME = {NAME##_launch, (const void *)win16_kernel<M, RV, WPEV, NWV>, #NAME, RV, WaveWin16<M, RV, -1>::CS, \
                                    WaveWin16<M, RV, -1>::BND_ALL, M::NS, M::MAXAT, NWV, WaveWin16<M, RV, -1>::SEEDW, 0, 1, 0, 1};
WIN16_KERNEL(kwin16_est2genome_r4w2, Est2GenomeDesc, 4, 2, 1)
WIN16_KERNEL(kwin16_est2genome_r3w3, Est2GenomeDesc, 3, 3, 1)
WIN16_KERNEL(kwin16_est2genome_r2w4, Est2GenomeDesc, 2, 4, 1)
WIN16_KERNEL(kwin16_est2genome_r6w2, Est2GenomeDesc, 6, 2, 1)
WIN16_KERNEL(kwin16_est2genome_r4w2n4, Est2GenomeDesc, 4, 2, 4)
WIN16_KERNEL(kwin16_est2genome_r2w4n8, Est2GenomeDesc, 2, 4, 8)
WIN16_KERNEL(kwin16_est2genome_r2w4n4, Est2GenomeDesc, 2, 4, 4)
WIN16_KERNEL(kwin16_est2genome_r4w2n2, Est2GenomeDesc, 4, 2, 2)
WIN16_KERNEL(kwin16_est2genome_r4w3n2, Est2GenomeDesc, 4, 3, 2)
const KernelInfo *get_kernel_win16(int family, int variant) {
    if (family != FAM_EST2GENOME) return nullptr;
    switch (variant) {
        case 1: return &kwin16_est2genome_r3w3;
        case 2: return &kwin16_est2genome_r2w4;
        case 3: return &kwin16_est2genome_r6w2;
        case 4: return &kwin16_est2genome_r4w2n4;
        case 5: return &kwin16_est2genome_r2w4n8;
        case 6: return &kwin16_est2genome_r2w4n4;
        case 7: return &kwin16_est2genome_r4w2n2;
        case 9: return &kwin16_est2genome_r4w3n2;
        default: return &kwin16_est2genome_r4w2;
    }
}
}
```

Measured before the change: 1035 billion.

## Split checkpointed regions into pieces at windowed-pass crossing points

The windowed seed pass now records, for each hop, the crossing cell (row, state, column, score, intron length) into the checkpoint dump. The host uses these crossings to cut each reduced-space region into independent sub-regions that start from a seeded state and end in a fixed state. These pieces run as separate checkpoint jobs, which gives more parallel work and shorter target spans per job, and the stitch kernel checks that each piece's final cell matches the next piece's seed. In exchange it adds seed and final-state handling inside the DP kernel, extra dump traffic, and correctness risk at the piece boundaries.

Result: slower. 891.2 billion (-13.9%).

```diff
diff --git a/exonerate_amd/csrc/c4_ckpt16_kernel.h b/exonerate_amd/csrc/c4_ckpt16_kernel.h
--- a/exonerate_amd/csrc/c4_ckpt16_kernel.h
+++ b/exonerate_amd/csrc/c4_ckpt16_kernel.h
@@ -69,6 +69,8 @@
     bool carry_cols;
     int corner_sc[2], corner_srp[2];
     bool corner_set[2];
+    int fstate[2], lstate[2], seed_sc_pk[2], seed_il_pk[2];
+    bool seeded_any;
 
     template <class Fn>
     __device__ __forceinline__ static void for_exported(Fn &&fn) {
@@ -202,6 +204,23 @@
         });
     }
 
+    template <int PH>
+    __device__ __forceinline__ void seed_origin(bool origin) {
+        static_for<2>([&](auto H_) __attribute__((always_inline)) { constexpr int H = H_;
+            if (fstate[H] != M::START) {
+                const int hm = origin ? (H ? (int)0xffff0000u : 0x0000ffff) : 0;
+                static_for<NS>([&](auto S_) __attribute__((always_inline)) { constexpr int S = S_;
+                    if constexpr (inner(S)) {
+                        C16 &c = col[PH][0];
+                        c.sc[S] = bfi32(hm, fstate[H] == S ? seed_sc_pk[H] : NEG16, c.sc[S]);
+                        c.srp[S] = bfi32(hm, 0, c.srp[S]);
+                        if constexpr (live(S)) c.il[S] = bfi32(hm, seed_il_pk[H], c.il[S]);
+                    }
+                });
+            }
+        });
+    }
+
     template <bool JINT, int PH>
     __device__ __forceinline__ void step(int s, int i0, bool first_strip, bool last_strip, const int *bnd_in, int *bnd_out) {
         const int j = s - lane;
@@ -223,6 +242,9 @@
         const bool origin = first_strip & (lane == 0) & (s == 0);
         static_for<R>([&](auto RR_) __attribute__((always_inline)) { constexpr int RR = RR_;
             eval_cell<RR, PH, JINT>(j, origin, ms[RR], sp);
+            if constexpr (RR == 0 && !JINT) {
+                if (seeded_any && first_strip && s == 0) seed_origin<PH>(origin);
+            }
             if constexpr (RR == (R + 1) / 2 - 1) prefetch_profile();
         });
         for_exported([&](auto S_, int) __attribute__((always_inline)) { constexpr int S = S_;
@@ -259,6 +281,18 @@
                                     set = true;
                                 }
                             });
+                            if (lstate[H] != M::END) {
+                                set = false;
+                                static_for<NS>([&](auto S_) __attribute__((always_inline)) { constexpr int S = S_;
+                                    if constexpr (inner(S)) {
+                                        if (lstate[H] == S) {
+                                            e_sc = pk_half(col[PH][RR].sc[S], H);
+                                            e_srp = (int)(((unsigned)col[PH][RR].srp[S] >> (16 * H)) & 0xffffu);
+                                            set = true;
+                                        }
+                                    }
+                                });
+                            }
                             corner_sc[H] = e_sc; corner_srp[H] = e_srp; corner_set[H] = set;
                         }
                     });
@@ -346,7 +380,9 @@
             cp_count[H] = jx.cp_count;
             section[H] = jx.T / (jx.cp_count + 1);
             corner_sc[H] = LOW; corner_srp[H] = 0; corner_set[H] = false;
-        });
+            fstate[H] = jx.first_state; lstate[H] = jx.final_state;
+        });
+        seeded_any = (fstate[0] != M::START) | (fstate[1] != M::START);
         Qm = Q[0] > Q[1] ? Q[0] : Q[1]; Tm = T[0] > T[1] ? T[0] : T[1]; Tmin = T[0] < T[1] ? T[0] : T[1];
         static_for<M::NC>([&](auto CI_) __attribute__((always_inline)) { constexpr int CI = CI_;
             const int v = clamp16(kp->calc_value[CI]);
@@ -359,6 +395,17 @@
             open_il_pk = pk_pack(-lim, -lim);
             fifteen = 0x000f000f;
         }
+        static_for<2>([&](auto H_) __attribute__((always_inline)) { constexpr int H = H_;
+            const DevJob &jx = *jp[H];
+            const int sc = clamp16(jx.first_cell[0]);
+            seed_sc_pk[H] = pk_pack(sc, sc);
+            int len = 0;
+            if constexpr (M::NDES > 0) {
+                const long long l = (long long)jx.t0 - jx.first_cell[1] - 2;
+                len = l < 0 ? 0 : (l > 32767 ? 32767 : (int)l);
+            }
+            seed_il_pk[H] = pk_sub(pk_pack(len, len), lim_pk);
+        });
         const int nstrips = (Qm + 1 + W - 1) / W;
         const int nsteps = Tm + 64;
         const int main_lo = 63 + MAXAT, main_hi = Tm;
diff --git a/exonerate_amd/csrc/c4_config.h b/exonerate_amd/csrc/c4_config.h
--- a/exonerate_amd/csrc/c4_config.h
+++ b/exonerate_amd/csrc/c4_config.h
@@ -9,7 +9,7 @@
     X(SDP_ARENA_MB) X(REPAIR_REJOIN) X(PK16_R6) X(PK16_NW8) X(PK16_LONG) X(PK16_IO) X(PK16_C8) X(PIN_XFER) X(NESTED_REDO) X(MW) \
     X(LOOP_SHORTCUT) X(LOCAL_EXACT) X(LANES) X(FUSED) X(FREE_NOW) X(FORCE_CORNER_MISMATCH) X(DL_SYNC_FIRST) X(CONT_FREE) \
     X(CK16_TMAX) X(CK16_ROOT) X(CK16) X(CELL_STRICT) X(BYROOT) X(SS16_CHECK) X(SCORE_FIRST) X(HOST_THREADS) X(FORCE_SEQUENTIAL) \
-    X(FILL_ALLOC)
+    X(FILL_ALLOC) X(CKPT_PIECES)
 
 enum Key {
 #define X(name) name,
diff --git a/exonerate_amd/csrc/c4_engine_find_path.inc b/exonerate_amd/csrc/c4_engine_find_path.inc
--- a/exonerate_amd/csrc/c4_engine_find_path.inc
+++ b/exonerate_amd/csrc/c4_engine_find_path.inc
@@ -63,8 +63,13 @@
             }
             if (!win_pairs.empty()) {
                 std::vector<DevResult> wres;
-                if (windowed_region_pass(eng, seqs, win_pairs, plan, thr, kshift, wres)) return -1;
-                for (size_t x = 0; x < win_pairs.size(); x++) region_done.emplace_back(win_pairs[x], wres[x]);
+                std::vector<std::vector<int>> wcross;
+                const bool pieces = !c4cfg::is(c4cfg::CKPT_PIECES, 0);
+                if (windowed_region_pass(eng, seqs, win_pairs, plan, thr, kshift, wres, pieces ? &wcross : nullptr)) return -1;
+                for (size_t x = 0; x < win_pairs.size(); x++) {
+                    region_done.emplace_back(win_pairs[x], wres[x]);
+                    if (pieces) plan[win_pairs[x]].cross.swap(wcross[x]);
+                }
                 region_pairs.swap(rest);
             }
         }
diff --git a/exonerate_amd/csrc/c4_engine_launch.inc b/exonerate_amd/csrc/c4_engine_launch.inc
--- a/exonerate_amd/csrc/c4_engine_launch.inc
+++ b/exonerate_amd/csrc/c4_engine_launch.inc
@@ -42,6 +42,7 @@
     std::vector<long long> base;
     std::vector<int> d, t0w, t0_base;
     int hops = 0;
+    bool cross = false;
 };
 
 int window_waves(int family) {
@@ -74,7 +75,7 @@
     DevBuf<DevJob> d_fjobs, d_fsub_jobs;
     DevBuf<DevResult> d_fres, d_fsub_res;
     DevBuf<DevVsa> d_fvsa;
-    DevBuf<int> d_ffirst, d_fflags, d_fout;
+    DevBuf<int> d_ffirst, d_fflags, d_fout, d_fnext;
     DevBuf<unsigned long long> d_fstats;
     DevBuf<FusePair> d_fpairs;
     std::vector<DevJob> hf_jobs;
@@ -472,6 +473,7 @@
                     if (seed->hops) {
                         j.seed_base = seed->base[order[x]]; j.win_d = seed->d[order[x]]; j.win_t0w = seed->t0w[order[x]];
                         j.win_t0_base = seed->t0_base[order[x]]; j.win_hops = seed->hops;
+                        if (seed->cross && seed->fmt16 && ki->ckw > 0) { j.ckpt_off = dump_total; dump_total += (long long)seed->hops * ki->ckw; }
                     }
                 }
             }
@@ -628,6 +630,9 @@
                 if (mode == MODE_CKPT && jobs[x].ckpt_off >= 0) {
                     const long long ck = (long long)jobs[x].cp_count * ki->max_at * (jobs[x].Q + 1) * ki->n_states * ki->cs;
                     o.checkpoints.assign(dump.begin() + jobs[x].ckpt_off, dump.begin() + jobs[x].ckpt_off + ck);
+                } else if (seed && seed->mode == 2 && jobs[x].ckpt_off >= 0 && res[x].n_vsa > 1) {
+                    const long long cw = (long long)std::min(res[x].n_vsa - 1, seed->hops) * ki->ckw;
+                    o.checkpoints.assign(dump.begin() + jobs[x].ckpt_off, dump.begin() + jobs[x].ckpt_off + cw);
                 } else {
                     o.checkpoints.clear();
                 }
diff --git a/exonerate_amd/csrc/c4_engine_passes.inc b/exonerate_amd/csrc/c4_engine_passes.inc
--- a/exonerate_amd/csrc/c4_engine_passes.inc
+++ b/exonerate_amd/csrc/c4_engine_passes.inc
@@ -5,11 +5,14 @@
     bool needs_checkpoints;
 };
 
+constexpr int CROSS_W = 5;
+
 struct PairPlan {
     bool active = false, reduced = false;
     c4gpu_score region_score = 0;
     c4gpu_region ar;
     int end_from = 0;
+    std::vector<int> cross;
     std::vector<Segment> segs;
 };
 
@@ -88,9 +91,72 @@
     };
     const c4gpu_model *m = eng.model;
     c4gpu_ctx *ctx = eng.ctx;
-    const int n = (int)red.size();
-    if (!n || eng.pair_sub) return 0;
+    if (red.empty() || eng.pair_sub) return 0;
     if (c4cfg::is(c4cfg::FUSED, 0)) return 0;
+    const c4h::MemRule rule{m->max_query_advance, m->max_target_advance, m->n_states, m->total_shadow_designations};
+    struct Unit {
+        int pair;
+        c4gpu_region r;
+        int first_state, final_state, first_cell[2];
+        int cp, next;
+        int slot, of;
+    };
+    std::vector<Unit> units;
+    std::vector<int> unit_first(red.size() + 1, 0);
+    long long region_cells = 0, pairs_cut = 0;
+    const bool pieces_on = !c4cfg::is(c4cfg::CKPT_PIECES, 0);
+    {
+        const int piece_tmin = std::max(64, 8 * m->max_target_advance);
+        std::vector<int> keep;
+        for (size_t xi = 0; xi < red.size(); xi++) {
+            const PairPlan &p = plan[red[xi]];
+            const c4gpu_region &ar = p.ar;
+            const int cp_pair = c4h::checkpoint_rows(m, &ar, dpmemory_mb);
+            const int qe = ar.query_start + ar.query_length, te = ar.target_start + ar.target_length;
+            keep.clear();
+            bool sane = pieces_on && !p.cross.empty() && p.cross.size() % CROSS_W == 0;
+            if (sane) {
+                int q_prev = ar.query_start, t_prev = ar.target_start, t_kept = ar.target_start;
+                for (int k = (int)(p.cross.size() / CROSS_W) - 1; k >= 0; k--) {
+                    const int *c = &p.cross[(size_t)k * CROSS_W];
+                    if (c[0] < q_prev || c[0] > qe || c[2] <= t_prev || c[2] >= te ||
+                        c[1] == m->start_state || c[1] == m->end_state || c[1] < 0 || c[1] >= m->n_states) { sane = false; break; }
+                    q_prev = c[0]; t_prev = c[2];
+                    if (c[2] - t_kept < piece_tmin) continue;
+                    keep.push_back(k); t_kept = c[2];
+                }
+                while (sane && !keep.empty() && te - p.cross[(size_t)keep.back() * CROSS_W + 2] < piece_tmin) keep.pop_back();
+            }
+            if (!sane) keep.clear();
+            const int of = (int)keep.size() + 1;
+            const int section = std::max(piece_tmin, ar.target_length / (std::max(cp_pair, 0) + 1));
+            for (int a = 0; a < of; a++) {
+                Unit u;
+                memset(&u, 0, sizeof u);
+                u.pair = red[xi]; u.slot = a; u.of = of;
+                const int *c0 = a > 0 ? &p.cross[(size_t)keep[a - 1] * CROSS_W] : nullptr;
+                const int *c1 = a + 1 < of ? &p.cross[(size_t)keep[a] * CROSS_W] : nullptr;
+                const int q0 = c0 ? c0[0] : ar.query_start, t0 = c0 ? c0[2] : ar.target_start;
+                u.r = c4gpu_region{q0, t0, (c1 ? c1[0] : qe) - q0, (c1 ? c1[2] : te) - t0};
+                u.first_state = c0 ? c0[1] : m->start_state;
+                u.final_state = c1 ? c1[1] : m->end_state;
+                if (c0) { u.first_cell[0] = c0[3]; u.first_cell[1] = c0[4] >= 0 ? t0 - c0[4] - 2 : 0; }
+                if (of == 1) u.cp = cp_pair;
+                else {
+                    const int most = std::max(1, u.r.target_length / (2 * m->max_target_advance) - 2);
+                    const int by_rule = c4h::use_reduced_space(m, &u.r, dpmemory_mb) ? c4h::checkpoint_rows(m, &u.r, dpmemory_mb) : most;
+                    u.cp = std::max(1, std::min((u.r.target_length + section - 1) / section - 1, std::min(by_rule, most)));
+                }
+                u.next = a + 1 < of ? (int)units.size() + 1 : -1;
+                units.push_back(u);
+            }
+            unit_first[xi + 1] = (int)units.size();
+            region_cells += (long long)(ar.query_length + 1) * (ar.target_length + 1);
+            pairs_cut += of > 1;
+        }
+    }
+    const int n = (int)units.size();
+    const bool cut_any = pairs_cut > 0;
     const int wpe_env = c4cfg::num(c4cfg::WPE, 0);
     long long worst = 0;
     for (int i : red) worst = std::max(worst, (long long)plan[i].ar.query_length + plan[i].ar.target_length);
@@ -107,18 +173,18 @@
     const KernelInfo *kc16r = (ck16_on && ck_root_env) ? get_kernel_ck16(eng.family, ck_env == 8 ? 0 : ck_env - 1, true) : nullptr;
     const int ck16_tmax = c4cfg::num(c4cfg::CK16_TMAX, 0x7fffffff);
     hipStream_t s = ctx->stream;
-    const c4h::MemRule rule{m->max_query_advance, m->max_target_advance, m->n_states, m->total_shadow_designations};
     std::vector<int> order(n), cpn(n);
     std::vector<char> group(n, 0);
     std::iota(order.begin(), order.end(), 0);
-    auto cells = [&](int x) { const c4gpu_region &r = plan[red[x]].ar; return (long long)(r.query_length + 1) * (r.target_length + 1); };
-    auto root_of = [&](int x) { return plan[red[x]].end_from; };
+    auto cells = [&](int x) { const c4gpu_region &r = units[x].r; return (long long)(r.query_length + 1) * (r.target_length + 1); };
+    auto root_of = [&](int x) { return plan[units[x].pair].end_from; };
+    auto strips_of = [&](int x) { return (units[x].r.query_length + 1 + 255) / 256; };
     int count_g[3] = {0, 0, 0};
     for (int x = 0; x < n; x++) {
-        const c4gpu_region &r = plan[red[x]].ar;
-        cpn[x] = c4h::checkpoint_rows(m, &r, dpmemory_mb);
+        const c4gpu_region &r = units[x].r;
+        cpn[x] = units[x].cp;
         if (!kc16) continue;
-        const bool ok = eng.pk16_fits(r.query_length, r.target_length) && r.target_length <= ck16_tmax &&
+        const bool ok = eng.pk16_fits(r.query_length, r.target_length) && plan[units[x].pair].ar.target_length <= ck16_tmax &&
                         ((long long)r.query_length + 2) * kc16->n_states * kc16->max_at <= 65535 && cpn[x] >= 1 &&
                         r.target_length / (cpn[x] + 1) >= kc16->max_at;
         group[x] = !ok ? 0 : (kc16r && root_of(x) > 1) ? 2 : 1;
@@ -136,8 +202,8 @@
         int rows_max = 0;
         for (int x = 0; x < n; x++)
             if (group[x] == 2) {
-                strips += (plan[red[x]].ar.query_length + 1 + 255) / 256;
-                rows_max = std::max(rows_max, plan[red[x]].ar.query_length + 1);
+                strips += strips_of(x);
+                rows_max = std::max(rows_max, units[x].r.query_length + 1);
             }
         kc16r = get_kernel_ck16(eng.family, strips >= 3LL * n16r ? 8 : strips >= 2LL * n16r ? 5 : 0, true);
         if (rows_max > 1024 && rows_max <= 3 * 384 && strips >= 4LL * n16r && get_kernel_ck16(eng.family, 6, true))
@@ -147,6 +213,8 @@
     std::stable_sort(order.begin(), order.end(), [&](int a, int b) {
         if (group[a] != group[b]) return group[a] > group[b];
         if (group[a] == 2 && root_of(a) != root_of(b)) return root_of(a) < root_of(b);
+        if (cut_any && group[a] && strips_of(a) != strips_of(b)) return strips_of(a) > strips_of(b);
+        if (cut_any && group[a] && units[a].r.target_length != units[b].r.target_length) return units[a].r.target_length > units[b].r.target_length;
         return cells(a) > cells(b);
     });
     if (c4cfg::has(c4cfg::TRACE))
@@ -158,11 +226,13 @@
     bool carry = false, carry16 = false;
     int bnd16 = 0;
     for (int x = 0; x < n; x++) {
-        const c4gpu_region &r = plan[red[order[x]]].ar;
+        const Unit &u = units[order[x]];
+        const c4gpu_region &r = u.r;
         DevJob &j = jobs[x];
         memset(&j, 0, sizeof j);
-        j.pair = red[order[x]]; j.q0 = r.query_start; j.t0 = r.target_start; j.Q = r.query_length; j.T = r.target_length;
-        j.first_state = m->start_state; j.final_state = m->end_state;
+        j.pair = u.pair; j.q0 = r.query_start; j.t0 = r.target_start; j.Q = r.query_length; j.T = r.target_length;
+        j.first_state = u.first_state; j.final_state = u.final_state;
+        j.first_cell[0] = u.first_cell[0]; j.first_cell[1] = u.first_cell[1];
         j.cp_count = cpn[order[x]];
         j.root = x < n16r ? root_of(order[x]) : 0;
         int tb = 0;
@@ -322,9 +392,15 @@
     if (eng.d_fout.alloc(2 * (size_t)std::max<unsigned long long>(used, 1)) || eng.d_fpairs.alloc(n) ||
         eng.d_runs_used.upload(&zero64, 1, s))
         return -1;
+    std::vector<int> where(n), next_job(n, -1);
+    for (int x = 0; x < n; x++) where[order[x]] = x;
+    if (cut_any) {
+        for (int x = 0; x < n; x++) if (units[order[x]].next >= 0) next_job[x] = where[units[order[x]].next];
+        if (eng.d_fnext.upload(next_job.data(), n, s)) return -1;
+    }
     hipLaunchKernelGGL(fuse_stitch_kernel, dim3((n + 63) / 64), dim3(64), 0, s, eng.d_fjobs.p, eng.d_fvsa.p, eng.d_ffirst.p, n,
                        eng.d_fsub_res.p, eng.d_runs_out.p, 1 + m->total_shadow_designations, eng.d_fflags.p, eng.d_runs_used.p,
-                       eng.d_fout.p, eng.d_fpairs.p, n16, cell_strict() ? 1 : 0);
+                       eng.d_fout.p, eng.d_fpairs.p, n16, cell_strict() ? 1 : 0, cut_any ? eng.d_fnext.p : nullptr);
     HIP_OK(hipGetLastError());
     std::vector<FusePair> &fps = eng.hf_pairs;
     fps.resize(n);
@@ -338,36 +414,54 @@
         HIP_OK(c4_stream_sync(s));
     }
     lap("stitched + downloaded");
-    int n_done = 0;
-    for (int x = 0; x < n; x++) {
-        if (fps[x].status & 1) continue;
-        const int i = red[order[x]];
+    int n_done = 0, fell_back = 0, whole_left = 0;
+    for (size_t xi = 0; xi < red.size(); xi++) {
+        const int i = red[xi], u0 = unit_first[xi], u1 = unit_first[xi + 1];
+        bool ok = true;
+        long long ops = 0;
+        for (int u = u0; u < u1; u++) { ok = ok && !(fps[where[u]].status & 1); ops += fps[where[u]].count; }
+        if (ok && u1 - u0 > 1) ok = res[where[u1 - 1]].score == plan[i].region_score;
+        if (!ok) { (u1 - u0 > 1 ? fell_back : whole_left)++; continue; }
         c4gpu_alignment &a = alignments[i];
-        a.score = res[x].score;
+        a.score = res[where[u1 - 1]].score;
         a.region = plan[i].ar;
         a.valid = 1;
-        a.n_ops = fps[x].count;
-        if (a.n_ops) {
-            a.op_transition = (int32_t *)malloc(sizeof(int32_t) * a.n_ops);
-            a.op_length = (int32_t *)malloc(sizeof(int32_t) * a.n_ops);
-            const int *src = out.data() + 2 * fps[x].off;
-            for (int k = 0; k < a.n_ops; k++) { a.op_transition[k] = src[2 * k]; a.op_length[k] = src[2 * k + 1]; }
+        a.n_ops = 0;
+        if (ops) {
+            a.op_transition = (int32_t *)malloc(sizeof(int32_t) * ops);
+            a.op_length = (int32_t *)malloc(sizeof(int32_t) * ops);
+            int k = 0;
+            for (int u = u0; u < u1; u++) {
+                const int *src = out.data() + 2 * fps[where[u]].off;
+                for (int q = 0; q < fps[where[u]].count; q++) {
+                    if (k && a.op_transition[k - 1] == src[2 * q]) {
+                        a.op_length[k - 1] += src[2 * q + 1];
+                        if (a.op_length[k - 1] == 0) k--;
+                    } else {
+                        a.op_transition[k] = src[2 * q]; a.op_length[k] = src[2 * q + 1]; k++;
+                    }
+                }
+            }
+            a.n_ops = k;
         }
         done[i] = 1;
         n_done++;
     }
-    if (n_done < n) {
+    if (trace && pieces_on)
+        fprintf(stderr, "c4gpu trace:   fused: checkpoint pieces: %lld of %zu pairs cut, %d pieces, piece cells / region cells %.4f, "
+                "%d pairs fell back\n", pairs_cut, red.size(), n, region_cells ? (double)ckpt_cells / (double)region_cells : 0.0, fell_back);
+    if (whole_left) {
         std::vector<DevVsa> vsa((size_t)vsa_total);
         if (eng.d_fvsa.download(vsa.data(), vsa_total, s)) return -1;
         HIP_OK(c4_stream_sync(s));
         for (int x = 0; x < n; x++) {
-            if (!(fps[x].status & 1)) continue;
+            if (!(fps[x].status & 1) || units[order[x]].of > 1) continue;
             JobOut o;
             o.res = res[x];
             o.runs.n = 0;
             o.packed = x < n16;
             if (!(res[x].flags & FLAG_NO_END)) o.vsa.assign(vsa.begin() + jobs[x].vsa_off, vsa.begin() + jobs[x].vsa_off + res[x].n_vsa);
-            unfinished[red[order[x]]] = std::move(o);
+            unfinished[units[order[x]].pair] = std::move(o);
         }
     }
     if (c4cfg::has(c4cfg::TRACE))
@@ -375,7 +469,7 @@
         long long score_only = 0;
         for (int x = 0; x < n; x++) score_only += fps[x].status >> 8;
         fprintf(stderr, "c4gpu trace:   fused: %d of %d pairs finished on the device route, %lld sub-alignments, %lld final cells that "
-                "differ from their prediction in the score only\n", n_done, n, n_sub, score_only);
+                "differ from their prediction in the score only\n", n_done, (int)red.size(), n_sub, score_only);
     }
     lap("alignments built");
     return 0;
@@ -383,8 +477,10 @@
 
 template <class Thr>
 int windowed_region_pass(Engine &eng, const ResidentSeqs &seqs, const std::vector<int> &pairs,
-                         const std::vector<PairPlan> &plan, Thr thr, int kshift, std::vector<DevResult> &out) {
+                         const std::vector<PairPlan> &plan, Thr thr, int kshift, std::vector<DevResult> &out,
+                         std::vector<std::vector<int>> *cross_out = nullptr) {
     const int n = (int)pairs.size();
+    if (cross_out) cross_out->assign(n, std::vector<int>());
     auto nbits = [](int v) { int b = 0; while ((1LL << b) <= v) b++; return b; };
     std::vector<JobSpec> specs(n);
     std::vector<JobOut> outs;
@@ -425,6 +521,7 @@
         std::vector<JobSpec> hs(want.size());
         SeedPlan sp2;
         sp2.mode = 2; sp2.kshift = kshift; sp2.hops = std::max(1, max_hops); sp2.fmt16 = sp1.fmt16;
+        sp2.cross = cross_out != nullptr && sp1.fmt16;
         sp2.off.resize(want.size()); sp2.rows.resize(want.size()); sp2.base.resize(want.size());
         sp2.d.resize(want.size()); sp2.t0w.resize(want.size()); sp2.t0_base.resize(want.size());
         for (size_t h = 0; h < want.size(); h++) {
@@ -457,8 +554,15 @@
                 continue;
             }
             windows += r.n_vsa;
-            if (r.pad >= 0) { o.qs = r.qs; o.ts = r.ts; }
-            else open.push_back(want[h]);
+            if (r.pad >= 0) {
+                o.qs = r.qs; o.ts = r.ts;
+                if (sp2.cross && wouts[h].checkpoints.size() == (size_t)(r.n_vsa - 1) * CROSS_W) {
+                    std::vector<int> &c = (*cross_out)[want[h]];
+                    c = wouts[h].checkpoints;
+                    const c4gpu_region &ar = plan[pairs[want[h]]].ar;
+                    for (size_t k = 0; k < c.size(); k += CROSS_W) { c[k] += ar.query_start; c[k + 2] += ar.target_start; }
+                }
+            } else open.push_back(want[h]);
         }
     }
     if (!open.empty()) {
diff --git a/exonerate_amd/csrc/c4_engine_staging.inc b/exonerate_amd/csrc/c4_engine_staging.inc
--- a/exonerate_amd/csrc/c4_engine_staging.inc
+++ b/exonerate_amd/csrc/c4_engine_staging.inc
@@ -442,7 +442,8 @@
 
 __global__ void fuse_stitch_kernel(const DevJob *parents, const DevVsa *vsa, const int *first, int n_parents,
                                    const DevResult *sub, const uint32_t *runs, int path_cs, const int *flags,
-                                   unsigned long long *out_used, int *out, FusePair *pairs, int n_packed, int strict_score) {
+                                   unsigned long long *out_used, int *out, FusePair *pairs, int n_packed, int strict_score,
+                                   const int *next) {
     const int x = blockIdx.x * blockDim.x + threadIdx.x;
     if (x >= n_parents) return;
     FusePair fp; fp.off = 0; fp.count = 0; fp.status = 1;
@@ -461,6 +462,9 @@
             bad |= !final_cell_equiv(r.final_cell, dv.final_cell, path_cs, dv.ts + dv.tl, x < n_packed, strict_score != 0);
             if (bad) break;
             score_only += r.final_cell[0] != dv.final_cell[0];
+        } else if (next && next[x] >= 0) {
+            bad |= !final_cell_equiv(r.final_cell, parents[next[x]].first_cell, path_cs, pj.t0 + pj.T, true, strict_score != 0);
+            if (bad) break;
         }
     }
     if (bad) { pairs[x] = fp; return; }
diff --git a/exonerate_amd/csrc/c4_win16_kernel.h b/exonerate_amd/csrc/c4_win16_kernel.h
--- a/exonerate_amd/csrc/c4_win16_kernel.h
+++ b/exonerate_amd/csrc/c4_win16_kernel.h
@@ -2,6 +2,8 @@
 #include "c4_ckpt16_kernel.h"
 
 namespace c4k {
+
+constexpr int WIN16_CROSSW = 5;
 
 template <class M, int R, int ROOT>
 struct WaveWin16 {
@@ -388,7 +390,7 @@
 template <class M, int R, int ROOT, int NW>
 __device__ __forceinline__ void win16_chains(const KParams *kp_lds, const DevSeqs &seqs, DevJob *job_lds, int *more, int ia, int ib,
                                              DevResult *results, int *bnd, int *prog, int (*corner_lds)[4], int *prof_mem,
-                                             const uint8_t *tdense, int *stage_mem) {
+                                             const uint8_t *tdense, int *stage_mem, int *cross) {
     using DP = WaveWin16<M, R, ROOT>;
     int hop = 0, first_score = 0;
     bool active = threadIdx.x < 2 && more[threadIdx.x & 1];
@@ -449,6 +451,24 @@
                 const int row = rq[h] & 0x7fff, jc = rt[h] % DC, state = rt[h] / DC;
                 const int d2 = job.win_d - 1, t0w2 = d2 >= 1 ? (d2 << job.seed_kshift) - (DC - 1) : 0;
                 const int endcol = job.win_t0w + jc;
+                if (job.ckpt_off >= 0) {
+                    const int *dp16 = seqs.seed + job.seed_off + ((long long)jc * job.seed_rows + row) * DP::SEEDW;
+                    int dsc = 0, dil = -1;
+                    static_for<DP::NS>([&](auto S_) __attribute__((always_inline)) { constexpr int S = S_;
+                        if constexpr (DP::inner(S)) {
+                            if (state == S) {
+                                constexpr int hs = DP::D16::half_of_sc(S);
+                                dsc = (int)(short)(((unsigned)dp16[hs / 2] >> (16 * (hs & 1))) & 0xffffu);
+                                if constexpr (DP::live(S)) {
+                                    constexpr int hl = DP::D16::half_of_il(S);
+                                    dil = (int)(((unsigned)dp16[hl / 2] >> (16 * (hl & 1))) & 0xffffu);
+                                }
+                            }
+                        }
+                    });
+                    int *cw = cross + job.ckpt_off + (long long)hop * WIN16_CROSSW;
+                    cw[0] = row; cw[1] = state; cw[2] = endcol; cw[3] = dsc; cw[4] = dil;
+                }
                 job.Q = row; job.final_state = state;
                 job.T = endcol - t0w2; job.t0 = job.win_t0_base + t0w2;
                 job.seed_off = d2 >= 1 ? job.seed_base + (long long)(d2 - 1) * DC * job.seed_rows * DP::SEEDW : -1;
@@ -512,7 +532,7 @@
                     if (threadIdx.x == 0) WaveWin16<M, R, ROOT>::write_empty_column(bnd);
                     __builtin_amdgcn_fence(__ATOMIC_RELEASE, "workgroup");
                     __syncthreads();
-                    win16_chains<M, R, ROOT, NW>(kp_lds, seqs, job_lds, more, ia, ib, results, bnd, prog, corner_lds, prof_mem, tdense_lds, stage_mem);
+                    win16_chains<M, R, ROOT, NW>(kp_lds, seqs, job_lds, more, ia, ib, results, bnd, prog, corner_lds, prof_mem, tdense_lds, stage_mem, scratch.ckpt_dump);
                     ran = true;
                 }
             });
@@ -521,7 +541,7 @@
             if (threadIdx.x == 0) WaveWin16<M, R, -1>::write_empty_column(bnd);
             __builtin_amdgcn_fence(__ATOMIC_RELEASE, "workgroup");
             __syncthreads();
-            win16_chains<M, R, -1, NW>(kp_lds, seqs, job_lds, more, ia, ib, results, bnd, prog, corner_lds, prof_mem, tdense_lds, stage_mem);
+            win16_chains<M, R, -1, NW>(kp_lds, seqs, job_lds, more, ia, ib, results, bnd, prog, corner_lds, prof_mem, tdense_lds, stage_mem, scratch.ckpt_dump);
         } else if (!ran) {
             if (threadIdx.x < 2 && more[threadIdx.x]) {
                 DevResult res;
diff --git a/exonerate_amd/csrc/kernels/kwin16_families.hip b/exonerate_amd/csrc/kernels/kwin16_families.hip
--- a/exonerate_amd/csrc/kernels/kwin16_families.hip
+++ b/exonerate_amd/csrc/kernels/kwin16_families.hip
@@ -8,7 +8,7 @@
         return hipGetLastError();                                                                                      \
     }                                                                                                                  \
     static const KernelInfo NAME = {NAME##_launch, (const void *)win16_kernel<M, RV, WPEV, NWV>, #NAME, RV, WaveWin16<M, RV, -1>::CS, \
-                                    WaveWin16<M, RV, -1>::BND_ALL, M::NS, M::MAXAT, NWV, WaveWin16<M, RV, -1>::SEEDW, 0, 1, 0, 1};
+                                    WaveWin16<M, RV, -1>::BND_ALL, M::NS, M::MAXAT, NWV, WaveWin16<M, RV, -1>::SEEDW, WIN16_CROSSW, 1, 0, 1};
 WIN16_KERNEL(kwin16_est2genome_r4w2, Est2GenomeDesc, 4, 2, 1)
 WIN16_KERNEL(kwin16_est2genome_r3w3, Est2GenomeDesc, 3, 3, 1)
 WIN16_KERNEL(kwin16_est2genome_r2w4, Est2GenomeDesc, 2, 4, 1)
```
